# GiannisPikoulis/dsml-thesis

Hardware: AMD Instinct MI355X
Metric: DDIM denoise steps/sec (64×64×4 latent, 256² face) at 1/2/4/8 GPUs (higher is better)
Workload: dtype f32; 1 GPU; face_reenactment emotion-conditioned LDM (AffectNet config), DDIM-200 schedule, 16 samples/GPU, 64x64x4 latent, CFG off, eta 0, random-init weights; batch_per_gpu=16, global_batch=16, ddim_steps=200, hipgraph=True

## Files before the change

dsml_thesis_amd/csrc/igemm.hip:

```cpp
#include "ldmk_common.h"
#include "ldmk_split.h"
#include "ldmk_epilogue.h"
#include <stdlib.h>

#if defined(LDMK_IG_STAMPS) && (LDMK_IG_STAMPS == 1 || LDMK_IG_STAMPS == 3)
#define IG_T(i) do { const unsigned long long t_ = __builtin_amdgcn_s_memtime(); ig_acc[i] += t_ - ig_last; ig_last = t_; } while (0)
#elif defined(LDMK_IG_STAMPS)
#define IG_T(i) do { (void)ig_acc; (void)ig_last; } while (0)
#else
#define IG_T(i) do { } while (0)
#endif

namespace ldmk {

template <int TM, int TN, int LEAN>
__device__ __forceinline__ void ig_lean_epilogue(const ldmk_igemm_args& p, f32x16 (&acc)[TM][TN], const int rowbase, const int colbase, const int bz,
                                                 const int l31, const int half) {
  float* __restrict__ outp = p.out + (long long)bz * p.out_bstride;
  const float* __restrict__ resp = (LEAN == 2 || LEAN == 4) ? p.residual + (long long)bz * p.out_bstride : nullptr;
  const float alpha = p.alpha;
#pragma unroll
  for (int j = 0; j < TN; ++j) {
    const int col = colbase + j * 32 + l31;
    const float bv = p.bias ? p.bias[col] : 0.f;
// ... 1058 lines not shown
      const long long w = blocks * sk;
      const long long rounds = (w + 511) / 512;
      const float occ = (float)w / (float)(rounds * 512);
      const float kpen = (float)(iters / sk) / (float)(iters / sk + 2);
      const float score = kCfg[c].eff * col_use * row_use * occ * kpen * (sk > 1 ? 0.93f : 1.f);
      if (score > best) { best = score; best_cfg = c; best_sk = sk; }
    }
  }
  *cfg_out = best_cfg + 1;
  *splitk_out = best_sk;
}

template <int TM, int TN, int WM, int WN, int KS, bool BT, int BF, bool ASP, bool FG_RT>
static int launch_wk1(const ldmk_igemm_args& a, int splitk, float* ws, hipStream_t st) {
  if constexpr (FG_RT) return launch_cfg<TM, TN, WM, WN, 1, KS, false, BT, BF>(a, splitk, ws, st);
  else return launch_cfg_g<TM, TN, WM, WN, 1, KS, false, BT, BF, true, ASP>(a, splitk, ws, st);
}
template <bool BT, int BF, bool ASP, bool FG_RT>
static int dispatch_wk1(const ldmk_igemm_args& a, int cfg, int splitk, float* ws, hipStream_t st) {
  const bool geglu = a.epi == LDMK_EPI_GEGLU;
  if (cfg == 3) cfg = 4;
  if (cfg == 6) cfg = geglu ? 2 : 5;
  if (geglu && !kCfg[cfg - 1].even_tn) cfg = 1;
  switch (cfg) {
    case 1: return launch_wk1<2, 2, 2, 2, 1, BT, BF, ASP, FG_RT>(a, splitk, ws, st);
    case 2: return launch_wk1<1, 2, 2, 2, 2, BT, BF, ASP, FG_RT>(a, splitk, ws, st);
    case 4: return launch_wk1<1, 1, 2, 2, 2, BT, BF, ASP, FG_RT>(a, splitk, ws, st);
    default: return launch_wk1<1, 5, 4, 1, 1, BT, BF, ASP, FG_RT>(a, splitk, ws, st);
  }
}

template <bool BT>
static int dispatch(const ldmk_igemm_args& a, int cfg, int splitk, float* ws, hipStream_t st) {
  if (a.compute == LDMK_COMPUTE_BF16 && a.w_split && !BT && igemm_fast_gather_ok(a)) return dispatch_wk1<false, 2, false, false>(a, cfg, splitk, ws, st);
  if (a.compute == LDMK_COMPUTE_BF16) return dispatch_wk1<BT, 1, false, true>(a, cfg, splitk, ws, st);
  if (a.compute == LDMK_COMPUTE_BF16X3)
    return a.a_split ? dispatch_wk1<false, 3, true, false>(a, cfg, splitk, ws, st) : dispatch_wk1<false, 3, false, false>(a, cfg, splitk, ws, st);
  if (a.compute == LDMK_COMPUTE_F16X2) return dispatch_wk1<false, 4, false, false>(a, cfg, splitk, ws, st);
  if (a.epi == LDMK_EPI_GEGLU && !kCfg[cfg - 1].even_tn) cfg = 3;
  switch (cfg) {
    case 1: return launch_cfg<2, 2, 2, 2, 1, 1, false, BT>(a, splitk, ws, st);
    case 2: return launch_cfg<1, 2, 2, 2, 1, 2, false, BT>(a, splitk, ws, st);
    case 3: return launch_cfg<2, 2, 1, 1, 4, 1, false, BT>(a, splitk, ws, st);
    case 4: return launch_cfg<1, 1, 2, 2, 1, 2, false, BT>(a, splitk, ws, st);
    case 5: return launch_cfg<1, 5, 4, 1, 1, 1, false, BT>(a, splitk, ws, st);
    default: return launch_cfg<1, 5, 2, 1, 2, 1, false, BT>(a, splitk, ws, st);
  }
}

template <bool BT, bool FG>
static void set_all_attrs() {
  cfg_set_attr<2, 2, 2, 2, 1, 1, false, BT, false, FG>();
  cfg_set_attr<1, 2, 2, 2, 1, 2, false, BT, false, FG>();
  cfg_set_attr<2, 2, 1, 1, 4, 1, false, BT, false, FG>();
  cfg_set_attr<1, 1, 2, 2, 1, 2, false, BT, false, FG>();
  cfg_set_attr<1, 5, 4, 1, 1, 1, false, BT, false, FG>();
  cfg_set_attr<1, 5, 2, 1, 2, 1, false, BT, false, FG>();
}
void igemm_init_attributes() {
  set_all_attrs<false, true>();
  set_all_attrs<true, true>();
  set_all_attrs<false, false>();
  set_all_attrs<true, false>();
}

const char* rgemm_unsupported(const ldmk_igemm_args& a, int rcfg);
int rgemm_dispatch(const ldmk_igemm_args& a, int rcfg, hipStream_t st);
constexpr int kNumRCfg = 6;
const char* sgemm_unsupported(const ldmk_igemm_args& a, int scfg, int splitk);
int sgemm_dispatch(const ldmk_igemm_args& a, int scfg, int splitk, float* ws, hipStream_t st);
constexpr int kNumSCfg = 8;
const char* igemm_ws_unsupported(const ldmk_igemm_args& a, int wcfg, int splitk);
int igemm_ws_dispatch(const ldmk_igemm_args& a, int wcfg, int splitk, float* ws, hipStream_t st);
constexpr int kNumWCfg = 2;
const char* igemm_ps_unsupported(const ldmk_igemm_args& a, int pcfg, int splitk);
int igemm_ps_dispatch(const ldmk_igemm_args& a, int pcfg, int splitk, float* ws, hipStream_t st);
constexpr int kNumPCfg = 11;

}

extern "C" int ldmk_pack_wsplit(const float* w, int K, int N, int ldb, int batch, long long w_bstride, void* out, int ld_out,
                                void* stream) {
  LDMK_ENTER();
  LDMK_REQUIRE(w && out && K > 0 && N > 0 && ldb >= N && batch >= 1, "ldmk_pack_wsplit: bad args");
  LDMK_REQUIRE(ld_out >= K && ld_out % 8 == 0, "ldmk_pack_wsplit: ld_out=%d must be >= K=%d and a multiple of 8", ld_out, K);
  hipLaunchKernelGGL(ldmk::pack_wsplit_kernel<3>, dim3((ld_out + 31) / 32, (N + 31) / 32, batch), dim3(256), 0, (hipStream_t)stream, w, K,
                     N, ldb, w_bstride, reinterpret_cast<__bf16*>(out), ld_out);
  return ldmk::check_launch("ldmk_pack_wsplit");
}

extern "C" int ldmk_pack_wsplit_h2(const float* w, int K, int N, int ldb, int batch, long long w_bstride, int scale_exp, void* out, int ld_out,
                                   void* stream) {
  LDMK_ENTER();
  LDMK_REQUIRE(w && out && K > 0 && N > 0 && ldb >= N && batch >= 1, "ldmk_pack_wsplit_h2: bad args");
  LDMK_REQUIRE(ld_out >= K && ld_out % 8 == 0, "ldmk_pack_wsplit_h2: ld_out=%d must be >= K=%d and a multiple of 8", ld_out, K);
  LDMK_REQUIRE(scale_exp >= -60 && scale_exp <= 60, "ldmk_pack_wsplit_h2: scale_exp=%d outside [-60, 60]", scale_exp);
  hipLaunchKernelGGL(ldmk::pack_wsplit_h2_kernel, dim3((ld_out + 31) / 32, (N + 31) / 32, batch), dim3(256), 0, (hipStream_t)stream, w, K, N, ldb,
                     w_bstride, ldexpf(1.f, scale_exp), reinterpret_cast<_Float16*>(out), ld_out);
  return ldmk::check_launch("ldmk_pack_wsplit_h2");
}

extern "C" int ldmk_pack_wbf16t(const float* w, int K, int N, int ldb, void* out, int ld_out, void* stream) {
  LDMK_ENTER();
  LDMK_REQUIRE(w && out && K > 0 && N > 0 && ldb >= N, "ldmk_pack_wbf16t: bad args");
  LDMK_REQUIRE(ld_out >= K && ld_out % 8 == 0, "ldmk_pack_wbf16t: ld_out=%d must be >= K=%d and a multiple of 8", ld_out, K);
  hipLaunchKernelGGL(ldmk::pack_wsplit_kernel<1>, dim3((ld_out + 31) / 32, (N + 31) / 32, 1), dim3(256), 0, (hipStream_t)stream, w, K, N,
                     ldb, 0LL, reinterpret_cast<__bf16*>(out), ld_out);
  return ldmk::check_launch("ldmk_pack_wbf16t");
}

static int g_force_cfg = 0;
extern "C" void ldmk_igemm_force_config(int cfg) { g_force_cfg = cfg; }

extern "C" int ldmk_igemm_plan(const ldmk_igemm_args* args, int* tile_cfg, int* splitk) {
  if (!args || !tile_cfg || !splitk) return LDMK_EINVAL;
  ldmk::plan(*args, tile_cfg, splitk, args->splitk_ws ? args->splitk_ws_elems : 0);
  return LDMK_OK;
}

extern "C" long long ldmk_igemm_workspace_elems(const ldmk_igemm_args* args) {
  using namespace ldmk;
  LDMK_REQUIRE(args != nullptr, "ldmk_igemm_workspace_elems: null args");
  const ldmk_igemm_args& a = *args;
  LDMK_REQUIRE(a.M > 0 && a.N > 0 && a.K > 0, "ldmk_igemm_workspace_elems: empty problem M=%d N=%d K=%d", a.M, a.N, a.K);
  LDMK_REQUIRE(a.splitk >= 0 && a.splitk <= 64, "ldmk_igemm_workspace_elems: splitk=%d outside [0,64]", a.splitk);
  int cfg = a.tile_cfg, sk = a.splitk;
  if (sk == 0) {
    int c2 = 0;
    plan(a, &c2, &sk, 1LL << 50);
    if (cfg == 0) cfg = c2;
  }
  if (cfg > kNumCfg + kNumRCfg + kNumSCfg)
    return sk <= 1 || a.epi == LDMK_EPI_GEGLU ? 0 : (long long)(a.batch > 1 ? a.batch : 1) * sk * (long long)a.M * a.N;
  if (cfg > kNumCfg + kNumRCfg) {
    if (sk <= 1 || (a.epi == LDMK_EPI_GEGLU && !a.raw_slabs)) return 0;
    return (long long)sk * (long long)a.M * a.N;
  }
  if (cfg > kNumCfg || a.epi == LDMK_EPI_GEGLU || sk <= 1) return 0;
  return (long long)(a.batch > 1 ? a.batch : 1) * sk * (long long)a.M * a.N;
}

static int igemm_entry(const ldmk_igemm_args* args, void* stream, bool launch);
extern "C" int ldmk_igemm(const ldmk_igemm_args* args, void* stream) { return igemm_entry(args, stream, true); }
extern "C" int ldmk_igemm_check(const ldmk_igemm_args* args) { return igemm_entry(args, nullptr, false); }

static int igemm_entry(const ldmk_igemm_args* args, void* stream, bool launch) {
  LDMK_ENTER();
  using namespace ldmk;
  LDMK_REQUIRE(args != nullptr, "ldmk_igemm: null args");
  ldmk_igemm_args a = *args;
  LDMK_REQUIRE(a.M > 0 && a.N > 0 && a.K > 0, "ldmk_igemm: empty problem M=%d N=%d K=%d", a.M, a.N, a.K);
  LDMK_REQUIRE(a.c0 > 0 && a.c0 % 32 == 0 && a.c1 % 32 == 0, "ldmk_igemm: channel counts must be multiples of 32 (c0=%d c1=%d)", a.c0, a.c1);
  LDMK_REQUIRE((a.c1 == 0) == (a.a1 == nullptr), "ldmk_igemm: a1/c1 mismatch");
  const int taps = a.a_mode == LDMK_A_CONV3X3 ? 9 : 1;
  const int skip_k = a.skip_a0 ? a.skip_c0 + a.skip_c1 : 0;
  LDMK_REQUIRE(a.K == taps * (a.c0 + a.c1) + skip_k, "ldmk_igemm: K=%d != taps*(c0+c1)+skip=%d", a.K, taps * (a.c0 + a.c1) + skip_k);
  LDMK_REQUIRE(!a.skip_a0 || (a.a_mode == LDMK_A_CONV3X3 && a.skip_c0 > 0 && a.skip_c0 % 8 == 0 && a.skip_c1 % 8 == 0 &&
                              (a.skip_c1 == 0) == (a.skip_a1 == nullptr) && (a.tile_cfg > kNumCfg + kNumRCfg || a.tile_cfg == 0)),
               "ldmk_igemm: the fused skip connection needs a 3x3 convolution on a slab-GEMM tile, skip channels in multiples of 8");
  LDMK_REQUIRE(a.N % 4 == 0 && a.ldb % 4 == 0, "ldmk_igemm: N and ldb must be multiples of 4");
  LDMK_REQUIRE(a.rows_per_sample > 0, "ldmk_igemm: rows_per_sample");
  LDMK_REQUIRE((long long)a.M * a.ldc < (1LL << 31) && a.ldc > 0, "ldmk_igemm: output exceeds 2^31 elements per batch item (32-bit epilogue offsets)");
  const long long samples = ((long long)a.M + a.rows_per_sample - 1) / a.rows_per_sample;
  if (a.a_mode == LDMK_A_CONV3X3) {
    LDMK_REQUIRE(a.in_h > 0 && a.in_w > 0 && a.out_h > 0 && a.out_w > 0 && a.stride >= 1, "ldmk_igemm: conv geometry");
    LDMK_REQUIRE(a.rows_per_sample == a.out_h * a.out_w, "ldmk_igemm: rows_per_sample != out_h*out_w");
    LDMK_REQUIRE(a.batch <= 1, "ldmk_igemm: batched conv unsupported");
    LDMK_REQUIRE(samples * a.in_h * a.in_w * (a.c0 > a.c1 ? a.c0 : a.c1) < (1LL << 31),
                 "ldmk_igemm: conv input exceeds 2^31 elements (32-bit gather indices)");
  } else {
    LDMK_REQUIRE((long long)a.M * (a.c0 > a.c1 ? a.c0 : a.c1) < (1LL << 31), "ldmk_igemm: A exceeds 2^31 elements per batch item");
  }
  if (a.a_tf == LDMK_TF_AFFINE || a.a_tf == LDMK_TF_AFFINE_SILU) LDMK_REQUIRE(a.tf_coef, "ldmk_igemm: tf_coef missing");
  if (a.a_tf == LDMK_TF_LAYERNORM) {
    LDMK_REQUIRE(a.row_stats && a.ln_gamma && a.ln_beta && a.a_mode == LDMK_A_ROWS, "ldmk_igemm: layernorm prologue args");
  }
  if (a.a_tf == LDMK_TF_LAYERNORM_FOLDED)
    LDMK_REQUIRE(a.row_stats && a.ln_colsum && a.a_mode == LDMK_A_ROWS && !a.stats_out && a.batch <= 1,
                 "ldmk_igemm: folded layernorm needs row_stats, ln_colsum (ldmk_fold_layernorm), rows mode, no stats_out, no batching");
  LDMK_REQUIRE(a.a_tf >= LDMK_TF_NONE && a.a_tf <= LDMK_TF_LAYERNORM_FOLDED, "ldmk_igemm: a_tf=%d", a.a_tf);
  if (a.epi == LDMK_EPI_GEGLU) LDMK_REQUIRE(a.N % 64 == 0 && !a.residual && !a.batch_vec, "ldmk_igemm: GEGLU needs N%%64==0 and no residual");
  if (a.stats_out)
    LDMK_REQUIRE(a.M % 32 == 0 && a.rows_per_sample % 32 == 0 && a.epi == LDMK_EPI_NONE && a.batch <= 1,
                 "ldmk_igemm: stats_out needs M%%32==0, rows_per_sample%%32==0, no GEGLU, no batching");
  LDMK_REQUIRE(a.tile_cfg >= 0 && a.tile_cfg <= kNumCfg + kNumRCfg + kNumSCfg + kNumWCfg + kNumPCfg, "ldmk_igemm: tile_cfg=%d outside [0,%d]",
               a.tile_cfg, kNumCfg + kNumRCfg + kNumSCfg + kNumWCfg + kNumPCfg);
  LDMK_REQUIRE(a.splitk >= 0 && a.splitk <= 64, "ldmk_igemm: splitk=%d outside [0,64]", a.splitk);
  LDMK_REQUIRE(a.compute == LDMK_COMPUTE_F32 || a.compute == LDMK_COMPUTE_BF16 || a.compute == LDMK_COMPUTE_BF16X3 || a.compute == LDMK_COMPUTE_F16X2,
               "ldmk_igemm: compute=%d", a.compute);
  const bool ps_tile = a.tile_cfg > kNumCfg + kNumRCfg + kNumSCfg + kNumWCfg;
  LDMK_REQUIRE(!a.a_ps1 || (ps_tile && a.a_ps), "ldmk_igemm: a_ps1 (second A source) is read by the pre-split tiles only, next to a_ps");
  if (a.compute == LDMK_COMPUTE_BF16X3 && !ps_tile) {
    LDMK_REQUIRE(a.w_split && !a.b_trans && a.w_split_ld >= a.K && a.w_split_ld % 8 == 0,
                 "ldmk_igemm: LDMK_COMPUTE_BF16X3 needs w_split (ldmk_pack_wsplit), b_trans = 0, w_split_ld >= K and a multiple of 8");
    LDMK_REQUIRE(3LL * a.N * a.w_split_ld * 2 < (1LL << 32), "ldmk_igemm: w_split exceeds 4 GB per batch entry");
    LDMK_REQUIRE(igemm_fast_gather_ok(a), "ldmk_igemm: LDMK_COMPUTE_BF16X3 needs the fast gather (no zero-insertion, two-source "
                 "upsampling or operands beyond 4 GB)");
  }
  if (a.compute == LDMK_COMPUTE_F16X2) {
    LDMK_REQUIRE(a.tile_cfg <= kNumCfg || ps_tile, "ldmk_igemm: LDMK_COMPUTE_F16X2 runs on the LDS-tiled shapes (tile_cfg 0..6) and the pre-split "
                 "tiles (23..28, 31..33), not tile_cfg=%d", a.tile_cfg);
    LDMK_REQUIRE(!a.a_split && a.w_scale_exp >= -60 && a.w_scale_exp <= 60, "ldmk_igemm: LDMK_COMPUTE_F16X2: a_split is not taken; w_scale_exp=%d", a.w_scale_exp);
    if (!ps_tile) {
      LDMK_REQUIRE(a.w_split && !a.b_trans && a.w_split_ld >= a.K && a.w_split_ld % 8 == 0 && 2LL * a.N * a.w_split_ld * 2 < (1LL << 32),
                   "ldmk_igemm: LDMK_COMPUTE_F16X2 needs w_split (ldmk_pack_wsplit_h2), b_trans = 0, w_split_ld >= K and a multiple of 8, below 4 GB");
      LDMK_REQUIRE(a.range_flag != nullptr, "ldmk_igemm: LDMK_COMPUTE_F16X2 needs range_flag");
      LDMK_REQUIRE(igemm_fast_gather_ok(a), "ldmk_igemm: LDMK_COMPUTE_F16X2 needs the fast gather (no zero-insertion, two-source upsampling or "
                   "operands beyond 4 GB)");
    }
  }
  if (a.compute == LDMK_COMPUTE_BF16 && a.w_split)
    LDMK_REQUIRE(!a.b_trans && a.w_split_ld >= a.K && a.w_split_ld % 8 == 0 && (long long)a.N * a.w_split_ld * 2 < (1LL << 32) && a.batch <= 1,
                 "ldmk_igemm: LDMK_COMPUTE_BF16 with w_split (ldmk_pack_wbf16t) needs b_trans = 0, w_split_ld >= K and a multiple of 8, "
                 "no batching");
  if (a.a_split) {
    LDMK_REQUIRE(a.compute == LDMK_COMPUTE_BF16X3 && a.a_mode == LDMK_A_ROWS && a.c1 == 0 && a.batch <= 1 &&
                 (a.a_tf == LDMK_TF_NONE || a.a_tf == LDMK_TF_LAYERNORM_FOLDED) && a.tile_cfg <= kNumCfg,
                 "ldmk_igemm: a_split (pre-split A) needs LDMK_COMPUTE_BF16X3 on an LDS-tiled shape (tile_cfg 0..6), rows mode, one "
                 "source, no staging prologue, no batching");
    LDMK_REQUIRE(a.a_split_ld >= a.K && a.a_split_ld % 8 == 0 && 3LL * a.M * a.a_split_ld * 2 < (1LL << 32),
                 "ldmk_igemm: a_split_ld=%d must be >= K, a multiple of 8, and the three images below 4 GB", a.a_split_ld);
  }
  LDMK_REQUIRE(a.compute == LDMK_COMPUTE_F32 || a.tile_cfg <= kNumCfg || a.tile_cfg > kNumCfg + kNumRCfg + kNumSCfg,
               "ldmk_igemm: the row / slab GEMM tiles are fp32 only");
  if (a.alpha == 0.f) a.alpha = 1.f;
  if (a.compute == LDMK_COMPUTE_F16X2) a.alpha *= ldexpf(1.f, -(LDMK_F16X2_A_EXP + a.w_scale_exp));
  int cfg = 0, sk = 1;
  plan(a, &cfg, &sk, a.splitk_ws ? a.splitk_ws_elems : 0);
  if (a.tile_cfg > 0) cfg = a.tile_cfg;
  if (g_force_cfg > 0 && (g_force_cfg <= kNumCfg || !rgemm_unsupported(a, g_force_cfg - kNumCfg - 1))) cfg = g_force_cfg;
  LDMK_REQUIRE(!a.skip_a0 || cfg > kNumCfg + kNumRCfg, "ldmk_igemm: the fused skip connection runs on the slab GEMM only (tile_cfg 13..20)");
  if (cfg > kNumCfg + kNumRCfg + kNumSCfg + kNumWCfg) {
    const int pcfg = cfg - kNumCfg - kNumRCfg - kNumSCfg - kNumWCfg - 1;
    int psk = a.splitk > 0 ? a.splitk : 1;
    const char* why = igemm_ps_unsupported(a, pcfg, psk);
    LDMK_REQUIRE(why == nullptr, "ldmk_igemm: tile_cfg=%d splitk=%d (pre-split bf16x3 tile) cannot run this problem: %s", cfg, psk, why ? why : "");
    LDMK_REQUIRE(!a.raw_slabs || psk >= 2, "ldmk_igemm: raw_slabs needs a split-K plan");
    if (psk > 1) {
      const long long b = a.batch > 1 ? a.batch : 1;
      LDMK_REQUIRE_MEM(a.splitk_ws && b * psk * (long long)a.M * a.N <= a.splitk_ws_elems,
                       "ldmk_igemm: splitk=%d needs a workspace of %lld floats (ldmk_igemm_workspace_elems), %lld given", psk,
                       b * psk * (long long)a.M * a.N, a.splitk_ws ? a.splitk_ws_elems : 0LL);
    }
    if (!launch) return LDMK_OK;
    return igemm_ps_dispatch(a, pcfg, psk, a.splitk_ws, (hipStream_t)stream);
  }
  if (cfg > kNumCfg + kNumRCfg + kNumSCfg) {
    const int wcfg = cfg - kNumCfg - kNumRCfg - kNumSCfg - 1;
    int wsk = a.splitk > 0 ? a.splitk : 1;
    const char* why = igemm_ws_unsupported(a, wcfg, wsk);
    LDMK_REQUIRE(why == nullptr, "ldmk_igemm: tile_cfg=%d splitk=%d (warp-specialised bf16x3 tile) cannot run this problem: %s", cfg, wsk,
                 why ? why : "");
    LDMK_REQUIRE(!a.raw_slabs || wsk >= 2, "ldmk_igemm: raw_slabs needs a split-K plan");
    if (wsk > 1) {
      const long long b = a.batch > 1 ? a.batch : 1;
      LDMK_REQUIRE_MEM(a.splitk_ws && b * wsk * (long long)a.M * a.N <= a.splitk_ws_elems,
                       "ldmk_igemm: splitk=%d needs a workspace of %lld floats (ldmk_igemm_workspace_elems), %lld given", wsk,
                       b * wsk * (long long)a.M * a.N, a.splitk_ws ? a.splitk_ws_elems : 0LL);
    }
    if (!launch) return LDMK_OK;
    return igemm_ws_dispatch(a, wcfg, wsk, a.splitk_ws, (hipStream_t)stream);
  }
  if (cfg > kNumCfg + kNumRCfg) {
    const int scfg = cfg - kNumCfg - kNumRCfg - 1;
    int ssk = a.splitk > 0 ? a.splitk : 1;
    const char* why = sgemm_unsupported(a, scfg, ssk);
    LDMK_REQUIRE(why == nullptr, "ldmk_igemm: tile_cfg=%d splitk=%d (slab GEMM) cannot run this problem: %s", cfg, ssk, why ? why : "");
    if (ssk > 1)
      LDMK_REQUIRE_MEM(a.splitk_ws && ssk * (long long)a.M * a.N <= a.splitk_ws_elems,
                       "ldmk_igemm: splitk=%d needs a workspace of %lld floats (ldmk_igemm_workspace_elems), %lld given", ssk,
                       ssk * (long long)a.M * a.N, a.splitk_ws ? a.splitk_ws_elems : 0LL);
    if (!launch) return LDMK_OK;
    return sgemm_dispatch(a, scfg, ssk, a.splitk_ws, (hipStream_t)stream);
  }
  if (cfg > kNumCfg) {
    const char* why = rgemm_unsupported(a, cfg - kNumCfg - 1);
    LDMK_REQUIRE(why == nullptr, "ldmk_igemm: tile_cfg=%d (row GEMM) cannot run this problem: %s", cfg, why ? why : "");
    if (!launch) return LDMK_OK;
    return rgemm_dispatch(a, cfg - kNumCfg - 1, (hipStream_t)stream);
  }
  if (a.splitk > 0) sk = a.splitk;
  if (a.epi == LDMK_EPI_GEGLU && !a.raw_slabs) sk = 1;
  LDMK_REQUIRE(!a.raw_slabs || (sk >= 2 && a.batch <= 1 && !a.splitk_counters && !a.stats_out),
               "ldmk_igemm: raw_slabs needs a split-K plan (splitk >= 2), no batching / in-launch combine / stats_out");
  if (sk > 1 && a.splitk_counters) {
    const long long tiles = (long long)(a.batch > 1 ? a.batch : 1) * ((a.M + 63) / 64) * ((a.N + 63) / 64);
    LDMK_REQUIRE_MEM(tiles <= a.splitk_counters_len, "ldmk_igemm: in-launch split-K combine needs %lld zeroed counters, %d given",
                     tiles, a.splitk_counters_len);
    LDMK_REQUIRE((long long)sk * a.M * a.N * 4 < (1LL << 31), "ldmk_igemm: in-launch split-K combine addresses the %d slabs of one "
                 "batch entry with 32-bit offsets (%lld bytes)", sk, (long long)sk * a.M * a.N * 4);
  }
  if (sk > 1) {
    const long long b = a.batch > 1 ? a.batch : 1;
    LDMK_REQUIRE_MEM(a.splitk_ws && b * sk * (long long)a.M * a.N <= a.splitk_ws_elems,
                     "ldmk_igemm: splitk=%d needs a workspace of %lld floats (ldmk_igemm_workspace_elems), %lld given", sk,
                     b * sk * (long long)a.M * a.N, a.splitk_ws ? a.splitk_ws_elems : 0LL);
  }
  if (!launch) return LDMK_OK;
  hipStream_t st = (hipStream_t)stream;
  return a.b_trans ? dispatch<true>(a, cfg, sk, a.splitk_ws, st) : dispatch<false>(a, cfg, sk, a.splitk_ws, st);
}
```

dsml_thesis_amd/csrc/igemm_ps.hip:

```cpp
#include "ldmk_common.h"
#include "ldmk_split.h"
#include "ldmk_epilogue.h"
#include <stdlib.h>

namespace ldmk {

#ifdef LDMK_PS_PROBES
constexpr bool PS_PROBES = true;
#else
constexpr bool PS_PROBES = false;
#endif
static int ps_probe_bits() {
  if (!PS_PROBES) return 0;
  static const int dbg = [] {
    const char* d = getenv("LDMK_PS_DEBUG");
    const char* s = getenv("LDMK_PS_STAGGER");
    return (d ? atoi(d) : 0) | ((s ? atoi(s) : 0) << 8);
  }();
  return dbg;
}

constexpr unsigned PS_OOB = 0x80000000u;

__device__ __forceinline__ void ps_dma3(unsigned voff, const u32x4& rs, unsigned lds_dst) {
// ... 781 lines not shown
  const u32x4 rs_a = buffer_rsrc(p.a_ps, Mb_in * (unsigned)Kb_in * (unsigned)UB);
  const u32x4 rs_b = buffer_rsrc(p.w_ps, (unsigned)Nb * (unsigned)Kb_w * (unsigned)UB);

  unsigned toff[AI][9];
#pragma unroll
  for (int i = 0; i < AI; ++i) {
    const int u = wave + NW * i;
    const int row = m0 + 32 * u + l31;
    const bool rok = u < FA && row < p.M;
    const int rr = rok ? row : 0;
    const int n = rr / p.rows_per_sample, rem = rr - n * p.rows_per_sample;
    const int oy = rem / p.out_w, ox = rem - oy * p.out_w;
#pragma unroll
    for (int t = 0; t < 9; ++t) {
      const int iy = oy * p.stride + t / 3 - p.pad_lo, ix = ox * p.stride + t % 3 - p.pad_lo;
      const bool ok = rok && iy >= 0 && iy < p.in_h && ix >= 0 && ix < p.in_w;
      const unsigned q = (unsigned)((n * p.in_h + iy) * p.in_w + ix);
      toff[i][t] = ok ? (q >> 5) * (unsigned)Kb_in * (unsigned)UB + ((unsigned)half * 32u + (q & 31u)) * 16u : PS_OOB;
    }
  }
  unsigned ubase[UHI];
#pragma unroll
  for (int i = 0; i < UHI; ++i) {
    const int u = wave + NW * i;
    const int blk = n0 / 32 + (u - FA);
    ubase[i] = (u >= FA && u < U && blk < Nb) ? (unsigned)blk * (unsigned)Kb_w * (unsigned)UB + (unsigned)(18 * c_begin) * (unsigned)UB : PS_OOB;
  }
  const unsigned lane16 = lane * 16;
  const unsigned lds0 = (unsigned)(size_t)smem_ps;
  const bool hi_wave = wave + NW * (UHI - 1) < U;

  f32x16 acc[TM][TN];
#pragma unroll
  for (int i = 0; i < TM; ++i)
#pragma unroll
    for (int j = 0; j < TN; ++j)
#pragma unroll
      for (int r = 0; r < 16; ++r) acc[i][j][r] = 0.f;

  auto issue = [&](const int c, const int j, const int buf, const unsigned sB) {
    const bool live = c < c_end;
    const unsigned cs = (unsigned)(2 * c + (j & 1)) * (unsigned)UB;
    const unsigned bdst = lds0 + (unsigned)buf * STAGE;
#pragma unroll
    for (int i = 0; i < UHI; ++i) {
      const int u = wave + NW * i;
      if (u < U) {
        if (i < AI && u < FA) {
          const unsigned t = toff[i < AI ? i : 0][j >> 1];
          ps_dma<PL>((live && t != PS_OOB) ? t + cs : PS_OOB, rs_a, bdst + (unsigned)u * (unsigned)UB);
        } else {
          ps_dma<PL>((live && ubase[i] != PS_OOB) ? lane16 + ubase[i] + sB * (unsigned)UB : PS_OOB, rs_b, bdst + (unsigned)u * (unsigned)UB);
        }
      }
    }
  };

  unsigned sB = 0;
  issue(c_begin, 0, 0, 0);
  issue(c_begin, 1, 1, 1);
  for (int c = c_begin; c < c_end; ++c) {
#pragma unroll
    for (int j = 0; j < 18; ++j) {
      if (hi_wave) wait_vm<PL * UHI * (NS - 2)>(); else wait_vm<PL * ULO * (NS - 2)>();
      asm volatile("s_barrier" ::: "memory");
      issue(j + 2 < 18 ? c : c + 1, (j + 2) % 18, (j + 2) % NS, sB + 2);
      ++sB;
      const unsigned char* sb = smem_ps + (j % NS) * STAGE + lane16;
      f16x8 a8[PL][TM];
#pragma unroll
      for (int g = 0; g < PL; ++g)
#pragma unroll
        for (int i = 0; i < TM; ++i) a8[g][i] = *reinterpret_cast<const f16x8*>(sb + ((wm * TM + i) * PL + g) * 1024);
#pragma unroll
      for (int jn = 0; jn < TN; ++jn) {
        f16x8 b8[PL];
#pragma unroll
        for (int g = 0; g < PL; ++g) b8[g] = *reinterpret_cast<const f16x8*>(sb + ((FA + wn * TN + jn) * PL + g) * 1024);
#pragma unroll
        for (int i = 0; i < TM; ++i) {
          if constexpr (TR) {
            acc[i][jn] = __builtin_amdgcn_mfma_f32_32x32x16_f16(b8[0], a8[1][i], acc[i][jn], 0, 0, 0);
            acc[i][jn] = __builtin_amdgcn_mfma_f32_32x32x16_f16(b8[1], a8[0][i], acc[i][jn], 0, 0, 0);
            acc[i][jn] = __builtin_amdgcn_mfma_f32_32x32x16_f16(b8[0], a8[0][i], acc[i][jn], 0, 0, 0);
          } else {
            acc[i][jn] = __builtin_amdgcn_mfma_f32_32x32x16_f16(a8[1][i], b8[0], acc[i][jn], 0, 0, 0);
            acc[i][jn] = __builtin_amdgcn_mfma_f32_32x32x16_f16(a8[0][i], b8[1], acc[i][jn], 0, 0, 0);
            acc[i][jn] = __builtin_amdgcn_mfma_f32_32x32x16_f16(a8[0][i], b8[0], acc[i][jn], 0, 0, 0);
          }
        }
      }
    }
  }
  wait_vm<0>();
  const int lean = ps_lean_form<TR>(p, splitk, (nfast & 2) != 0, m0 + (wm + 1) * 32 * TM, n0 + (wn + 1) * 32 * TN);
  if (lean == 1) ps_epilogue<TM, TN, TR, PL, false, 1>(p, acc, m0 + wm * 32 * TM, n0 + wn * 32 * TN, splitk, ks, 0, ws, lane);
  else if (lean == 2) ps_epilogue<TM, TN, TR, PL, false, 2>(p, acc, m0 + wm * 32 * TM, n0 + wn * 32 * TN, splitk, ks, 0, ws, lane);
  else if (lean == 3) ps_epilogue<TM, TN, TR, PL, false, 3>(p, acc, m0 + wm * 32 * TM, n0 + wn * 32 * TN, splitk, ks, 0, ws, lane);
  else if (lean == 4) ps_epilogue<TM, TN, TR, PL, false, 4>(p, acc, m0 + wm * 32 * TM, n0 + wn * 32 * TN, splitk, ks, 0, ws, lane);
  else ps_epilogue<TM, TN, TR, PL>(p, acc, m0 + wm * 32 * TM, n0 + wn * 32 * TN, splitk, ks, 0, ws, lane);
}

__global__ __launch_bounds__(256) void gn_apply_ps_h2_kernel(const float* __restrict__ x0, int c0, const float* __restrict__ x1, int c1,
                                                             const float* __restrict__ coef, unsigned char* __restrict__ dst, long long rows,
                                                             int hw, int silu, int* __restrict__ range_flag) {
  const int rb = blockIdx.x, kc = blockIdx.y;
  const int r = threadIdx.x >> 3, o = threadIdx.x & 7;
  const long long row = (long long)rb * 32 + r;
  const int C = c0 + c1;
  const int k0 = kc * 64 + o * 8;
  if (k0 >= C) return;
  float4 v0 = make_float4(0.f, 0.f, 0.f, 0.f), v1 = v0;
  if (row < rows) {
    const float* src = k0 < c0 ? x0 + row * c0 + k0 : x1 + row * c1 + (k0 - c0);
    const float4 a = *reinterpret_cast<const float4*>(src), b = *reinterpret_cast<const float4*>(src + 4);
    const float* cf = coef + ((row / hw) * 2) * C + k0;
    const float4 s0 = *reinterpret_cast<const float4*>(cf), s1 = *reinterpret_cast<const float4*>(cf + 4);
    const float4 h0 = *reinterpret_cast<const float4*>(cf + C), h1 = *reinterpret_cast<const float4*>(cf + C + 4);
    v0 = make_float4(fmaf(a.x, s0.x, h0.x), fmaf(a.y, s0.y, h0.y), fmaf(a.z, s0.z, h0.z), fmaf(a.w, s0.w, h0.w));
    v1 = make_float4(fmaf(b.x, s1.x, h1.x), fmaf(b.y, s1.y, h1.y), fmaf(b.z, s1.z, h1.z), fmaf(b.w, s1.w, h1.w));
    if (silu) {
      v0 = make_float4(silu_f(v0.x), silu_f(v0.y), silu_f(v0.z), silu_f(v0.w));
      v1 = make_float4(silu_f(v1.x), silu_f(v1.y), silu_f(v1.z), silu_f(v1.w));
    }
    if (h2_out_of_range(v0) || h2_out_of_range(v1)) *range_flag = 1;
  }
  unsigned char* d = dst + ((long long)rb * (C / 16) + (k0 >> 4)) * 2048 + ((o & 1) * 32 + r) * 16;
  f16x4 a0, l0, a1, l1;
  split2h(scaled_sat(v0), a0, l0);
  split2h(scaled_sat(v1), a1, l1);
  *reinterpret_cast<f16x8*>(d) = f16x8{a0[0], a0[1], a0[2], a0[3], a1[0], a1[1], a1[2], a1[3]};
  *reinterpret_cast<f16x8*>(d + 1024) = f16x8{l0[0], l0[1], l0[2], l0[3], l1[0], l1[1], l1[2], l1[3]};
}

template <int NWM, int NWN, int TM, int TN, bool TR>
static int psc_launch(const ldmk_igemm_args& a, int splitk, float* ws, hipStream_t st) {
  constexpr int BM = 32 * TM * NWM, BN = 32 * TN * NWN;
  constexpr size_t lds = (size_t)3 * (BM / 32 + BN / 32) * 2048;
  static_assert(lds <= 160 * 1024, "LDS ring exceeds 160 KiB");
  static bool attr = false;
  if (!attr) {
    (void)hipFuncSetAttribute(reinterpret_cast<const void*>(igemm_psc_kernel<NWM, NWN, TM, TN, TR>), hipFuncAttributeMaxDynamicSharedMemorySize, (int)lds);
    attr = true;
  }
  const int tiles = ((a.M + BM - 1) / BM) * ((a.N + BN - 1) / BN);
  const int nfast_env = switch_value(SW_PS_NFAST);
  const int lean_env = switch_value(SW_PS_LEAN);
  const int nfast = (nfast_env && (a.N + BN - 1) / BN > 1 && (a.M + BM - 1) / BM >= 8 ? 1 : 0) | (lean_env ? 0 : 2);
  hipLaunchKernelGGL((igemm_psc_kernel<NWM, NWN, TM, TN, TR>), dim3(tiles, splitk, 1), dim3(64 * NWM * NWN), lds, st, a, splitk, ws, nfast);
  if (splitk > 1 && !a.raw_slabs) return launch_splitk_reduce(a, splitk, ws, st);
  return check_launch("ldmk_igemm(ps, conv)");
}

const char* igemm_ps_unsupported(const ldmk_igemm_args& a, int pcfg, int splitk) {
  if (a.compute != LDMK_COMPUTE_BF16X3 && a.compute != LDMK_COMPUTE_F16X2) return "the pre-split tiles run the bf16x3 and the f16x2 arithmetic (compute)";
  const int pl = a.compute == LDMK_COMPUTE_F16X2 ? 2 : 3;
  if (pl == 2 && (pcfg == 6 || pcfg == 7)) return "the warp-specialised pre-split tiles (29 / 30) exist in the bf16x3 arithmetic only";
  if (pl == 2 && a.out_ps && !a.range_flag) return "out_ps in the f16x2 arithmetic needs range_flag";
  if (!a.a_ps || !a.w_ps) return "a_ps / w_ps (operands in the PS layout: ldmk_pack_ps, ldmk_ln_stats_ps, out_ps of a producer GEMM)";
  if (a.a_mode == LDMK_A_CONV3X3) {
    if (pl != 2) return "the conv-mode pre-split tile runs the f16x2 arithmetic only";
    if (pcfg != 0 && pcfg != 1 && pcfg != 3 && pcfg != 4) return "conv mode: tile_cfg 23 / 24 / 26 / 27";
    if (a.c1 || a.a1 || a.upsample || a.a_tf != LDMK_TF_NONE || a.out_ps || a.batch > 1 || a.epi != LDMK_EPI_NONE || a.attn_kv_out)
      return "conv mode: one pre-normalised source (ldmk_gn_apply_ps_h2), no upsampling / prologue / out_ps / batching / GEGLU";
    if (a.c0 % 32) return "conv mode: C_in must be a multiple of 32";
    if ((a.c0 / 32) % splitk) return "conv mode: splitk must divide C_in / 32 (K is split on 32-channel chunk boundaries)";
    const long long smp = ((long long)a.M + a.rows_per_sample - 1) / a.rows_per_sample;
    if (((smp * a.in_h * a.in_w + 31) / 32) * (a.c0 / 16) * 2048 >= (1LL << 31)) return "conv mode: input of 2 GiB or more";
  } else if (a.a_mode != LDMK_A_ROWS) {
    return "rows mode or 3x3 convolution";
  }
  if (a.b_trans || a.upsample || a.skip_a0 || (a.splitk_counters && !(ps_probe_bits() & 8))) return "b_trans / upsample / fused skip / in-launch combine";
  if (a.a_tf != LDMK_TF_NONE && a.a_tf != LDMK_TF_LAYERNORM_FOLDED) return "no staging prologue: a_ps is what gets multiplied";
  if (a.K % 32 || a.N % 32) return "K and N must be multiples of 32";
  if (a.a_ps1) {
    if (a.a_mode != LDMK_A_ROWS || pcfg == 6 || pcfg == 7) return "a_ps1: rows mode on tile_cfg 23..28 / 31..33 (not the conv-mode or warp-specialised tiles)";
    if (a.batch > 1 || a.attn_kv_out || a.a_tf != LDMK_TF_NONE || a.epi == LDMK_EPI_GEGLU)
      return "a_ps1: no batching, no fused QKV tiles, no folded LayerNorm, no GEGLU";
    if (a.a_ps_k0 <= 0 || a.a_ps_k0 >= a.K || a.a_ps_k0 % 32) return "a_ps1: a_ps_k0 and K - a_ps_k0 must be positive multiples of 32";
  }
  const long long kb = a.K / 16;
  if ((a.a_mode == LDMK_A_ROWS && (long long)((a.M + 31) / 32) * kb * pl * 1024 >= (1LL << 31)) || (long long)(a.N / 32) * kb * pl * 1024 >= (1LL << 31))
    return "an operand of 2 GiB or more";
  if (a.epi == LDMK_EPI_GEGLU && (!kPsCfg[pcfg].even_tn || splitk > 1)) return "GEGLU needs a tile of (value, gate) pairs (256x256, 128x256) and no split-K";
  if (splitk > a.K / 32) return "more K slices than 32-deep chunks";
  if (a.out_ps) {
    if (splitk > 1 || a.batch > 1 || a.stats_out) return "out_ps: no split-K, no batching, no GroupNorm records (transposed epilogue)";
    if (a.ldc % 16) return "out_ps: ldc (the PS output's column count) must be a multiple of 16";
  } else if (!a.out && splitk <= 1) {
    return "no output";
  }
  if (a.stats_out && !a.out) return "stats_out needs out";
  if (a.attn_kv_out) {
    if (pl != 2 || (pcfg != 0 && pcfg != 4)) return "attn_kv_out: the F16X2 arithmetic on tile_cfg 23 / 27";
    if (a.stats_out || splitk > 1 || a.batch > 1 || a.epi != LDMK_EPI_NONE || a.out_ps || !a.out || !a.range_flag)
      return "attn_kv_out: the fused QKV projection (no split-K / batching / GEGLU / records / out_ps; out and range_flag required)";
    if (a.attn_heads <= 0 || a.N != 3 * 32 * a.attn_heads) return "attn_kv_out: N must be 3 x 32 x attn_heads ([q | k | v] of d_head 32)";
    if (a.attn_tokens <= 0 || a.attn_tokens % 64 || a.M % a.attn_tokens) return "attn_kv_out: attn_tokens a multiple of 64 that divides M";
  }
  return nullptr;
}

int igemm_ps_dispatch(const ldmk_igemm_args& a, int pcfg, int splitk, float* ws, hipStream_t st) {
  const bool tr = !a.stats_out;
  if (a.a_mode == LDMK_A_CONV3X3) {
    switch (pcfg) {
      case 0: return tr ? psc_launch<8, 1, 1, 5, true>(a, splitk, ws, st) : psc_launch<8, 1, 1, 5, false>(a, splitk, ws, st);
      case 1: return tr ? psc_launch<4, 2, 2, 5, true>(a, splitk, ws, st) : psc_launch<4, 2, 2, 5, false>(a, splitk, ws, st);
      case 3: return tr ? psc_launch<4, 2, 1, 5, true>(a, splitk, ws, st) : psc_launch<4, 2, 1, 5, false>(a, splitk, ws, st);
      default: return tr ? psc_launch<4, 1, 1, 5, true>(a, splitk, ws, st) : psc_launch<4, 1, 1, 5, false>(a, splitk, ws, st);
    }
  }
  if (a.compute == LDMK_COMPUTE_F16X2 && a.attn_kv_out)
    return pcfg == 0 ? ps_launch<8, 1, 1, 5, 3, true, 2, true>(a, splitk, ws, st) : ps_launch<4, 1, 1, 5, 3, true, 2, true>(a, splitk, ws, st);
  if (a.compute == LDMK_COMPUTE_F16X2) {
    switch (pcfg) {
      case 0: return tr ? ps_launch<8, 1, 1, 5, 3, true, 2>(a, splitk, ws, st) : ps_launch<8, 1, 1, 5, 3, false, 2>(a, splitk, ws, st);
      case 1: return tr ? ps_launch<4, 2, 2, 5, 3, true, 2>(a, splitk, ws, st) : ps_launch<4, 2, 2, 5, 3, false, 2>(a, splitk, ws, st);
      case 2: return tr ? ps_launch<4, 2, 2, 4, 3, true, 2>(a, splitk, ws, st) : ps_launch<4, 2, 2, 4, 3, false, 2>(a, splitk, ws, st);
      case 3: return tr ? ps_launch<4, 2, 1, 5, 3, true, 2>(a, splitk, ws, st) : ps_launch<4, 2, 1, 5, 3, false, 2>(a, splitk, ws, st);
      case 4: return tr ? ps_launch<4, 1, 1, 5, 3, true, 2>(a, splitk, ws, st) : ps_launch<4, 1, 1, 5, 3, false, 2>(a, splitk, ws, st);
      case 8: return tr ? ps_launch<4, 1, 2, 5, 3, true, 2>(a, splitk, ws, st) : ps_launch<4, 1, 2, 5, 3, false, 2>(a, splitk, ws, st);
      case 9: return tr ? ps_launch<4, 1, 2, 4, 3, true, 2>(a, splitk, ws, st) : ps_launch<4, 1, 2, 4, 3, false, 2>(a, splitk, ws, st);
      case 10: return tr ? ps_launch<2, 2, 2, 4, 3, true, 2>(a, splitk, ws, st) : ps_launch<2, 2, 2, 4, 3, false, 2>(a, splitk, ws, st);
      default: return tr ? ps_launch<4, 2, 1, 4, 3, true, 2>(a, splitk, ws, st) : ps_launch<4, 2, 1, 4, 3, false, 2>(a, splitk, ws, st);
    }
  }
  switch (pcfg) {
    case 0: return tr ? ps_launch<8, 1, 1, 5, 3, true>(a, splitk, ws, st) : ps_launch<8, 1, 1, 5, 3, false>(a, splitk, ws, st);
    case 1: return tr ? ps_launch<4, 2, 2, 5, 2, true>(a, splitk, ws, st) : ps_launch<4, 2, 2, 5, 2, false>(a, splitk, ws, st);
    case 2: return tr ? ps_launch<4, 2, 2, 4, 3, true>(a, splitk, ws, st) : ps_launch<4, 2, 2, 4, 3, false>(a, splitk, ws, st);
    case 3: return tr ? ps_launch<4, 2, 1, 5, 3, true>(a, splitk, ws, st) : ps_launch<4, 2, 1, 5, 3, false>(a, splitk, ws, st);
    case 4: return tr ? ps_launch<4, 1, 1, 5, 2, true>(a, splitk, ws, st) : ps_launch<4, 1, 1, 5, 2, false>(a, splitk, ws, st);
    case 6: return tr ? pw_launch<2, 5, 4, true>(a, splitk, ws, st) : pw_launch<2, 5, 4, false>(a, splitk, ws, st);
    case 7: return tr ? pw_launch<2, 4, 4, true>(a, splitk, ws, st) : pw_launch<2, 4, 4, false>(a, splitk, ws, st);
    case 8: return tr ? ps_launch<4, 1, 2, 5, 2, true>(a, splitk, ws, st) : ps_launch<4, 1, 2, 5, 2, false>(a, splitk, ws, st);
    case 9: return tr ? ps_launch<4, 1, 2, 4, 2, true>(a, splitk, ws, st) : ps_launch<4, 1, 2, 4, 2, false>(a, splitk, ws, st);
    case 10: return tr ? ps_launch<2, 2, 2, 4, 2, true>(a, splitk, ws, st) : ps_launch<2, 2, 2, 4, 2, false>(a, splitk, ws, st);
    default: return tr ? ps_launch<4, 2, 1, 4, 3, true>(a, splitk, ws, st) : ps_launch<4, 2, 1, 4, 3, false>(a, splitk, ws, st);
  }
}

}

extern "C" long long ldmk_ps_bytes(int rows, int k) {
  if (rows <= 0 || k <= 0 || k % 16) return -1;
  return (long long)((rows + 31) / 32) * (k / 16) * 3072;
}

extern "C" long long ldmk_ps_bytes_h2(int rows, int k) {
  if (rows <= 0 || k <= 0 || k % 16) return -1;
  return (long long)((rows + 31) / 32) * (k / 16) * 2048;
}

extern "C" int ldmk_pack_ps(const float* src, int rows, int k, long long row_stride, long long k_stride, int batch, long long src_bstride,
                            void* dst, void* stream) {
  LDMK_ENTER();
  using namespace ldmk;
  LDMK_REQUIRE(src && dst && rows > 0 && k > 0 && batch >= 1, "ldmk_pack_ps: bad args");
  LDMK_REQUIRE(k % 16 == 0, "ldmk_pack_ps: k=%d must be a multiple of 16", k);
  LDMK_REQUIRE(k_stride != 1 || (row_stride % 4 == 0 && (reinterpret_cast<uintptr_t>(src) & 15) == 0 && src_bstride % 4 == 0),
               "ldmk_pack_ps: row-major sources are read as float4 (16-byte aligned rows)");
  const long long bytes = ldmk_ps_bytes(rows, k);
  hipLaunchKernelGGL(pack_ps_kernel<3>, dim3((rows + 31) / 32, (k + 63) / 64, batch), dim3(256), 0, (hipStream_t)stream, src, rows, k, row_stride,
                     k_stride, src_bstride, reinterpret_cast<unsigned char*>(dst), bytes, 1.0f, (int*)nullptr);
  return check_launch("ldmk_pack_ps");
}

extern "C" int ldmk_pack_ps_h2(const float* src, int rows, int k, long long row_stride, long long k_stride, int batch, long long src_bstride,
                               int scale_exp, int* range_flag, void* dst, void* stream) {
  LDMK_ENTER();
  using namespace ldmk;
  LDMK_REQUIRE(src && dst && rows > 0 && k > 0 && batch >= 1, "ldmk_pack_ps_h2: bad args");
  LDMK_REQUIRE(k % 16 == 0, "ldmk_pack_ps_h2: k=%d must be a multiple of 16", k);
  LDMK_REQUIRE(k_stride != 1 || (row_stride % 4 == 0 && (reinterpret_cast<uintptr_t>(src) & 15) == 0 && src_bstride % 4 == 0),
               "ldmk_pack_ps_h2: row-major sources are read as float4 (16-byte aligned rows)");
  LDMK_REQUIRE(scale_exp >= -60 && scale_exp <= 60, "ldmk_pack_ps_h2: scale_exp=%d outside [-60, 60]", scale_exp);
  LDMK_REQUIRE(!range_flag || scale_exp == LDMK_F16X2_A_EXP, "ldmk_pack_ps_h2: range_flag is the activations' check: scale_exp must be %d", LDMK_F16X2_A_EXP);
  const long long bytes = ldmk_ps_bytes_h2(rows, k);
  hipLaunchKernelGGL(pack_ps_kernel<2>, dim3((rows + 31) / 32, (k + 63) / 64, batch), dim3(256), 0, (hipStream_t)stream, src, rows, k, row_stride,
                     k_stride, src_bstride, reinterpret_cast<unsigned char*>(dst), bytes, ldexpf(1.f, scale_exp), range_flag);
  return check_launch("ldmk_pack_ps_h2");
}

extern "C" int ldmk_ln_stats_ps(const float* x, int rows, int c, float eps, float* stats, void* dst, float guard, int* flag, void* stream) {
  LDMK_ENTER();
  using namespace ldmk;
  LDMK_REQUIRE(x && stats && dst && rows > 0 && c > 0, "ldmk_ln_stats_ps: bad args");
  LDMK_REQUIRE(c % 16 == 0 && c <= 1280, "ldmk_ln_stats_ps: C=%d must be a multiple of 16, at most 1280", c);
  LDMK_REQUIRE(!flag || guard > 0.f, "ldmk_ln_stats_ps: guard=%g must be positive", (double)guard);
  const dim3 grid((rows + 31) / 32);
  unsigned char* d = reinterpret_cast<unsigned char*>(dst);
  hipStream_t st = (hipStream_t)stream;
  int* nf = nullptr;
  if (c <= 192) hipLaunchKernelGGL(ln_stats_ps_kernel<3>, grid, dim3(256), 0, st, x, rows, c, eps, stats, d, guard, flag, nf);
  else if (c <= 320) hipLaunchKernelGGL(ln_stats_ps_kernel<5>, grid, dim3(256), 0, st, x, rows, c, eps, stats, d, guard, flag, nf);
  else if (c <= 640) hipLaunchKernelGGL(ln_stats_ps_kernel<10>, grid, dim3(256), 0, st, x, rows, c, eps, stats, d, guard, flag, nf);
  else hipLaunchKernelGGL(ln_stats_ps_kernel<20>, grid, dim3(256), 0, st, x, rows, c, eps, stats, d, guard, flag, nf);
  return check_launch("ldmk_ln_stats_ps");
}

extern "C" int ldmk_ln_stats_ps_h2(const float* x, int rows, int c, float eps, float* stats, void* dst, float guard, int* flag, int* range_flag,
                                   void* stream) {
  LDMK_ENTER();
  using namespace ldmk;
  LDMK_REQUIRE(x && stats && dst && range_flag && rows > 0 && c > 0, "ldmk_ln_stats_ps_h2: bad args");
  LDMK_REQUIRE(c % 16 == 0 && c <= 1280, "ldmk_ln_stats_ps_h2: C=%d must be a multiple of 16, at most 1280", c);
  LDMK_REQUIRE(!flag || guard > 0.f, "ldmk_ln_stats_ps_h2: guard=%g must be positive", (double)guard);
  const dim3 grid((rows + 31) / 32);
  unsigned char* d = reinterpret_cast<unsigned char*>(dst);
  hipStream_t st = (hipStream_t)stream;
  if (c <= 192) hipLaunchKernelGGL((ln_stats_ps_kernel<3, 2>), grid, dim3(256), 0, st, x, rows, c, eps, stats, d, guard, flag, range_flag);
  else if (c <= 320) hipLaunchKernelGGL((ln_stats_ps_kernel<5, 2>), grid, dim3(256), 0, st, x, rows, c, eps, stats, d, guard, flag, range_flag);
  else if (c <= 640) hipLaunchKernelGGL((ln_stats_ps_kernel<10, 2>), grid, dim3(256), 0, st, x, rows, c, eps, stats, d, guard, flag, range_flag);
  else hipLaunchKernelGGL((ln_stats_ps_kernel<20, 2>), grid, dim3(256), 0, st, x, rows, c, eps, stats, d, guard, flag, range_flag);
  return check_launch("ldmk_ln_stats_ps_h2");
}

extern "C" int ldmk_gn_apply_ps_h2(const float* x0, int c0, const float* x1, int c1, const float* coef, void* y_ps, int n, int hw, int silu,
                                   int* range_flag, void* stream) {
  LDMK_ENTER();
  using namespace ldmk;
  LDMK_REQUIRE(x0 && coef && y_ps && range_flag && n > 0 && hw > 0 && c0 > 0, "ldmk_gn_apply_ps_h2: bad args");
  LDMK_REQUIRE((c1 == 0) == (x1 == nullptr), "ldmk_gn_apply_ps_h2: x1/c1 mismatch");
  LDMK_REQUIRE(c0 % 8 == 0 && c1 % 8 == 0 && (c0 + c1) % 16 == 0, "ldmk_gn_apply_ps_h2: c0 = %d, c1 = %d must be multiples of 8, their sum of 16", c0, c1);
  const long long rows = (long long)n * hw;
  LDMK_REQUIRE(ldmk_ps_bytes_h2((int)rows, c0 + c1) < (1LL << 31) && rows < (1LL << 31), "ldmk_gn_apply_ps_h2: output of 2 GiB or more");
  hipLaunchKernelGGL(gn_apply_ps_h2_kernel, dim3((unsigned)((rows + 31) / 32), (c0 + c1 + 63) / 64), dim3(256), 0, (hipStream_t)stream, x0, c0, x1, c1,
                     coef, reinterpret_cast<unsigned char*>(y_ps), rows, hw, silu, range_flag);
  return check_launch("ldmk_gn_apply_ps_h2");
}
```

dsml_thesis_amd/csrc/ldmk_epilogue.h:

```cpp
#pragma once
#include "ldmk_common.h"

namespace ldmk {

__device__ __forceinline__ float lnf_bias(float acc, float mean, float cs, float rstd, float bias) {
#pragma clang fp contract(off)
  const float t = __builtin_fmaf(-mean, cs, acc) * rstd;
  return t + bias;
}
__device__ __forceinline__ float bias_res(float acc_alpha, float bias, float vec, float res) {
#pragma clang fp contract(off)
  float t = acc_alpha + bias;
  t = t + vec;
  return t + res;
}
__device__ __forceinline__ float col_finish(float acc_alpha, float bias) {
#pragma clang fp contract(off)
  return acc_alpha + bias;
}
__device__ __forceinline__ float col_finish(float acc_alpha, float bias, float extra) {
#pragma clang fp contract(off)
  const float t = acc_alpha + bias;
  return t + extra;
}
// ... 21 lines not shown
  sm += __shfl_xor(sm, 32, 64);
  sq += __shfl_xor(sq, 32, 64);
  if (half == 0) {
    float* d = stats_out + ((long long)tile_row * N + col) * 3;
    d[0] = shift; d[1] = sm; d[2] = sq;
  }
}

template <int TM, int TN>
__device__ __forceinline__ void col_slab_store(const ldmk_igemm_args& p, const f32x16 (&acc)[TM][TN], const int rowbase, const int colbase,
                                               const int bz, const int l31, const int half, const int splitk, const int ks,
                                               float* __restrict__ ws) {
  float* slab = ws + ((long long)bz * splitk + ks) * p.M * p.N;
#pragma unroll
  for (int j = 0; j < TN; ++j) {
    const int col = colbase + j * 32 + l31;
    if (col >= p.N) continue;
#pragma unroll
    for (int i = 0; i < TM; ++i)
#pragma unroll
      for (int r = 0; r < 16; ++r) {
        const int row = rowbase + i * 32 + (r & 3) + 8 * (r >> 2) + 4 * half;
        if (row < p.M) slab[(long long)row * p.N + col] = acc[i][j][r];
      }
  }
}

template <int TM, int TN>
__device__ __forceinline__ void col_geglu(const ldmk_igemm_args& p, const f32x16 (&acc)[TM][TN], const int rowbase, const int colbase,
                                          const int bz, const int l31, const int half, const bool lnf) {
  float* __restrict__ outp = p.out + (long long)bz * p.out_bstride;
  const float alpha = p.alpha;
  const float2* __restrict__ stats2 = reinterpret_cast<const float2*>(p.row_stats);
  if constexpr (TN % 2 == 0) {
#pragma unroll
    for (int j = 0; j < TN; j += 2) {
      const int cv = colbase + j * 32 + l31;
      const int cg = cv + 32;
      if (cv >= p.N) continue;
      const int oc = ((colbase + j * 32) >> 1) + l31;
      const float bv = p.bias ? p.bias[cv] : 0.f, bg = p.bias ? p.bias[cg] : 0.f;
      const float csv = lnf ? p.ln_colsum[cv] : 0.f, csg = lnf ? p.ln_colsum[cg] : 0.f;
#pragma unroll
      for (int i = 0; i < TM; ++i) {
        float2 st[16];
        if (lnf) {
#pragma unroll
          for (int r = 0; r < 16; ++r) st[r] = stats2[min(rowbase + i * 32 + (r & 3) + 8 * (r >> 2) + 4 * half, p.M - 1)];
        }
#pragma unroll
        for (int r = 0; r < 16; ++r) {
          const int row = rowbase + i * 32 + (r & 3) + 8 * (r >> 2) + 4 * half;
          if (row < p.M) {
            float v = acc[i][j][r] * alpha, g = acc[i][j + 1][r] * alpha;
            if (lnf) {
              v = fmaf(-st[r].x, csv, v) * st[r].y;
              g = fmaf(-st[r].x, csg, g) * st[r].y;
            }
            v += bv;
            g += bg;
            const float ge = gelu_erf_f(g);
            outp[(long long)row * p.ldc + oc] = v * ge;
          }
        }
      }
    }
  }
}

template <int TM, int TN>
__device__ __forceinline__ void col_general(const ldmk_igemm_args& p, f32x16 (&acc)[TM][TN], const int rowbase, const int colbase,
                                            const int bz, const int l31, const int half, const bool lnf) {
  float* __restrict__ outp = p.out + (long long)bz * p.out_bstride;
  const float* resp = p.residual ? p.residual + (long long)bz * p.out_bstride : nullptr;
  const float alpha = p.alpha;
  const float2* __restrict__ stats2 = reinterpret_cast<const float2*>(p.row_stats);
  const bool tile_in_sample = p.rows_per_sample % 32 == 0;
  int smp[TM];
#pragma unroll
  for (int i = 0; i < TM; ++i) smp[i] = p.batch_vec ? min(rowbase + i * 32, p.M - 1) / p.rows_per_sample : 0;
#pragma unroll
  for (int j = 0; j < TN; ++j) {
    const int col = colbase + j * 32 + l31;
    if (col >= p.N) continue;
    const float bv = p.bias ? p.bias[col] : 0.f;
    const float cs = lnf ? p.ln_colsum[col] : 0.f;
#pragma unroll
    for (int i = 0; i < TM; ++i) {
      float vals[16];
      const int r0 = rowbase + i * 32 + 4 * half;
      if (lnf) {
        float2 st[16];
#pragma unroll
        for (int r = 0; r < 16; ++r) st[r] = stats2[min(r0 + (r & 3) + 8 * (r >> 2), p.M - 1)];
#pragma unroll
        for (int r = 0; r < 16; ++r) acc[i][j][r] = fmaf(-st[r].x, cs, acc[i][j][r] * alpha) * st[r].y;
      }
      const unsigned obase = (unsigned)r0 * (unsigned)p.ldc + (unsigned)col;
      const float vec = (p.batch_vec && tile_in_sample) ? p.batch_vec[(long long)smp[i] * p.batch_vec_ld + col] : 0.f;
#pragma unroll
      for (int r = 0; r < 16; ++r) {
        const int dr = (r & 3) + 8 * (r >> 2);
        float v = 0.f;
        if (r0 + dr < p.M) {
          v = (lnf ? acc[i][j][r] : acc[i][j][r] * alpha) + bv;
          if (p.batch_vec) v += tile_in_sample ? vec : p.batch_vec[(long long)((r0 + dr) / p.rows_per_sample) * p.batch_vec_ld + col];
          const unsigned o = obase + (unsigned)(dr * p.ldc);
          if (resp) v += resp[o];
          outp[o] = v;
        }
        vals[r] = v;
      }
      if (p.stats_out && rowbase + i * 32 < p.M) gn_tile_record(vals, p.stats_out, (rowbase + i * 32) >> 5, p.N, col, l31, half);
    }
  }
}

template <int TM, int TN, int LEAN>
__device__ __forceinline__ void col_lean(const ldmk_igemm_args& p, const f32x16 (&acc)[TM][TN], const int rowbase, const int colbase,
                                         const int bz, const int l31, const int half) {
  static_assert(LEAN >= 1 && LEAN <= 4, "operand set 1..4");
  float* __restrict__ outp = p.out + (long long)bz * p.out_bstride;
  const float* __restrict__ resp = (LEAN == 2 || LEAN == 4) ? p.residual + (long long)bz * p.out_bstride : nullptr;
  const float alpha = p.alpha;
#pragma unroll
  for (int j = 0; j < TN; ++j) {
    const int col = colbase + j * 32 + l31;
    const float bv = p.bias ? p.bias[col] : 0.f;
#pragma unroll
    for (int i = 0; i < TM; ++i) {
      const int r0 = rowbase + i * 32 + 4 * half;
      const unsigned obase = (unsigned)r0 * (unsigned)p.ldc + (unsigned)col;
      float extra[16], vec = 0.f;
      if constexpr (LEAN == 1 || LEAN == 4) vec = p.batch_vec[(long long)((rowbase + i * 32) / p.rows_per_sample) * p.batch_vec_ld + col];
      if constexpr (LEAN == 2 || LEAN == 4) {
#pragma unroll
        for (int r = 0; r < 16; ++r) extra[r] = resp[obase + (unsigned)(((r & 3) + 8 * (r >> 2)) * p.ldc)];
      }
      float vals[16];
#pragma unroll
      for (int r = 0; r < 16; ++r) {
        const float t = acc[i][j][r] * alpha;
        if constexpr (LEAN == 3) vals[r] = col_finish(t, bv);
        else if constexpr (LEAN == 1) vals[r] = col_finish(t, bv, vec);
        else if constexpr (LEAN == 2) vals[r] = col_finish(t, bv, extra[r]);
        else vals[r] = col_finish(t, bv, vec, extra[r]);
        outp[obase + (unsigned)(((r & 3) + 8 * (r >> 2)) * p.ldc)] = vals[r];
      }
      if (p.stats_out) gn_tile_record(vals, p.stats_out, (rowbase + i * 32) >> 5, p.N, col, l31, half);
    }
  }
}

__device__ __forceinline__ int col_lean_form(const ldmk_igemm_args& p, const int splitk, const bool off, const int row_end, const int col_end) {
  if (off || splitk != 1 || row_end > p.M || col_end > p.N) return 0;
  if (p.batch_vec && p.rows_per_sample % 32 != 0) return 0;
  if (p.a_tf == LDMK_TF_LAYERNORM_FOLDED || p.epi == LDMK_EPI_GEGLU) return 0;
  return p.batch_vec ? (p.residual ? 4 : 1) : (p.residual ? 2 : 3);
}

}
```

dsml_thesis_amd/engine.py:

```python
import ctypes as C
import math
import os
from collections import namedtuple

import torch

from . import lib as L
from . import ops as _ops
from . import switches


def plan_key(a, m):
    key = f"{m},{a.N},{a.K},{a.a_mode},{a.a_tf},{a.epi},{max(1, a.batch)}"
    if a.b_trans:
        key += ",bt"
    if a.a_mode == L.A_CONV3X3 and (a.stride != 1 or a.upsample):
        key += f",s{a.stride}u{a.upsample}"
    return key


_SECTIONS = {"f32": "LDMK_PLAN_TABLE", "bf16x3": "LDMK_X3_TABLE", "f16x2": "LDMK_H2_TABLE", "ps_bf16x3": "LDMK_PS_TABLE",
             "ps_f16x2": "LDMK_PS_H2_TABLE"}
_TABLES = {}
_PLAN_FILE = os.path.join(os.path.dirname(os.path.abspath(__file__)), "igemm_plans.json")
# ... 322 lines not shown
            args.raw_slabs = 1
            args.splitk_ws, args.splitk_ws_elems = slabs.data_ptr(), args.splitk * args.M * args.N
        else:
            args.raw_slabs = 0
            args.out = slabs.data_ptr()
        args._own_slabs = slabs
        self.calls.append((self.lib.ldmk_igemm, (C.byref(args),), args, "ldmk_igemm"))

    def post(self, pargs, keep=None):
        need = self.lib.ldmk_post_scratch_elems(C.byref(pargs))
        if need > 0:
            if self._gnws is None or self._gnws.numel() < need:
                self._gnws = torch.empty(int(need), device=self.device, dtype=torch.float32)
                self._all.append(self._gnws)
                for _, _, k, name in self.calls:
                    if name == "ldmk_post" and k[0].gn_scratch:
                        k[0].gn_scratch, k[0].gn_scratch_elems = self._gnws.data_ptr(), self._gnws.numel()
            pargs.gn_scratch, pargs.gn_scratch_elems = self._gnws.data_ptr(), self._gnws.numel()
        self.calls.append((self.lib.ldmk_post, (C.byref(pargs),), (pargs, keep), "ldmk_post"))

    def run(self, stream=None):
        st = torch.cuda.current_stream().cuda_stream if stream is None else stream
        for fn, args, _, name in self.calls:
            rc = fn(*args, st)
            if rc != 0:
                L.check(rc, name)


class NetBuilder:

    def __init__(self, pg, n, pin=None, sites=None):
        self.pg, self.n, self.pin, self.ops = pg, n, pin, _ops
        self._stats = {}
        self.sites = sites
        self.h2_flag = pg.h2_flag

    def site(self, name):
        import contextlib

        @contextlib.contextmanager
        def ctx():
            if self.sites is None:
                yield self.h2_flag
                return
            old = (self.h2_flag, self.pg.h2_flag)
            self.h2_flag = self.pg.h2_flag = self.sites.flag(name)
            try:
                yield self.h2_flag
            finally:
                self.h2_flag, self.pg.h2_flag = old
        return ctx()

    @staticmethod
    def ptr(t):
        return 0 if t is None else (t if isinstance(t, int) else t.data_ptr())

    def stats_buffer(self, rows, c):
        return self.pg.alloc(rows // 32, c, 3)

    def release(self, *tensors):
        for t in tensors:
            if t is not None:
                self.drop_stats(t)
        self.pg.release(*tensors)

    def attach_stats(self, t, partial):
        self._stats[t.data_ptr()] = partial

    def drop_stats(self, t):
        p = self._stats.pop(t.data_ptr(), None)
        if p is not None:
            self.pg.release(p)

    def _partial(self, x, hw):
        p = self._stats.get(x.data_ptr())
        if p is None:
            c = x.shape[-1]
            p = self.pg.alloc(self.n * self.pg.lib.ldmk_gn_chunks(hw), c, 3)
            self.pg.add("ldmk_gn_partial", self.ptr(x), c, self.n, hw, self.ptr(p))
            self._stats[x.data_ptr()] = p
        return p

    def gn(self, x0, x1, hw, gamma, beta, eps, film=None):
        pg, p_ = self.pg, self.ptr
        c0 = x0.shape[-1]
        c1 = 0 if x1 is None else x1.shape[-1]
        pa = self._partial(x0, hw)
        pb = None if x1 is None else self._partial(x1, hw)
        coef = pg.alloc(self.n, 2, c0 + c1)
        pg.add("ldmk_gn_finalize", p_(pa), c0, p_(pb), c1, self.n, hw, 32, eps, p_(gamma), p_(beta), p_(coef))
        if film is not None:
            pg.add("ldmk_gn_coef_film", p_(coef), film[0], film[1], self.n, c0 + c1)
        return coef

    def gn_act(self, x0, x1, hw, gamma, beta, eps, silu=True, film=None):
        pg, p_ = self.pg, self.ptr
        c0 = x0.shape[-1]
        c1 = 0 if x1 is None else x1.shape[-1]
        coef = self.gn(x0, x1, hw, gamma, beta, eps, film)
        y = pg.alloc(self.n * hw, c0 + c1)
        pg.add("ldmk_gn_apply", p_(x0), c0, p_(x1), c1, p_(coef), p_(y), self.n, hw, 1 if silu else 0)
        self.release(coef)
        return y

    def conv(self, x0, x1, wp, bias, h, w, coef=None, stride=1, pad_lo=1, upsample=False, batch_vec=None, bv_ld=0,
             residual=None, out=None, stats=False, wf=None):
        pg, n, ops = self.pg, self.n, self.ops
        c0 = x0.shape[-1]
        c1 = 0 if x1 is None else x1.shape[-1]
        cout = wp.shape[1]
        if upsample:
            oh, ow = 2 * h, 2 * w
        elif pad_lo == 1:
            oh, ow = (h - 1) // stride + 1, (w - 1) // stride + 1
        else:
            oh, ow = (h + 1 - 3) // stride + 1, (w + 1 - 3) // stride + 1
        if out is None:
            out = pg.alloc(n, oh, ow, cout)
        a = ops.make_igemm_args(n * oh * ow, cout, 9 * (c0 + c1), x0, c0, wp, out, cout, oh * ow, a1=x1, c1=c1,
                                conv=(h, w, oh, ow, stride, pad_lo, 1 if upsample else 0),
                                tf=L.TF_NONE if coef is None else L.TF_AFFINE_SILU, tf_coef=coef, bias=bias,
                                residual=residual, w_frag=wf)
        if batch_vec is not None:
            a.batch_vec, a.batch_vec_ld = self.ptr(batch_vec), bv_ld
        self._maybe_stats(a, out.view(-1, cout), oh * ow, stats)
        pg.igemm(a, self.pin)
        return out

    WINO_MIN_TILES = int(switches.get("LDMK_WINO_MIN_TILES", "256"))
    UP_MIN_PIXELS = 1024
    WINO_MIN_CIN = int(switches.get("LDMK_WINO_MIN_CIN", "320"))

    def winograd_ok(self, cin, h, w):
        if switches.get("LDMK_NO_WINOGRAD"):
            return False
        pol_n = self.pin[0] if self.pin else self.n
        return (cin >= self.WINO_MIN_CIN and pol_n * (h // 2) * (w // 2) >= self.WINO_MIN_TILES and h % 2 == 0
                and w in (8, 16, 32, 64, 128) and (h * w) % 32 == 0 and (w >= 16 or (h // 2) % 2 == 0))

    def ps_query_conv(self, M, N, K, stride=1):
        if not ps_enabled() or self.h2_flag is None or switches.get("LDMK_PSC", "1") == "0":
            return None
        forced = switches.get("LDMK_PSC_FORCE")
        if forced:
            cfg, sk = (int(v) for v in forced.split(","))
            cin32 = K // (9 * 32)
            while cin32 % sk:
                sk -= 1
            return cfg, sk
        m = M
        if self.pin is not None and self.pin[0] != self.pin[1]:
            m = max(1, M * self.pin[0] // self.pin[1])
        return ps_plan(f"{N},{K},{L.A_CONV3X3},0,0,1" + ("" if stride == 1 else f",s{stride}u0"), m, h2=True, max_ratio=2.0)

    def gn_conv(self, x0, x1, h, w, gamma, beta, eps, wp, u, bias, batch_vec=None, bv_ld=0, residual=None, out=None,
                stats=False, wf=None, u_ps=None, wp_ps=None, film=None):
        pg, n, ops, p_ = self.pg, self.n, self.ops, self.ptr
        c0 = x0.shape[-1]
        c1 = 0 if x1 is None else x1.shape[-1]
        cin = c0 + c1
        cout_ = wp.shape[1]
        plan_c = (self.ps_query_conv(n * h * w, cout_, 9 * cin)
                  if (wp_ps is not None and cin % 32 == 0 and cout_ % 32 == 0 and c0 % 8 == 0 and c1 % 8 == 0) else None)
        if plan_c is not None:
            hf = self.h2_flag
            coef = self.gn(x0, x1, h * w, gamma, beta, eps, film)
            y_ps = pg.alloc_ps(n * h * w, cin)
            pg.add("ldmk_gn_apply_ps_h2", p_(x0), c0, p_(x1), c1, p_(coef), p_(y_ps), n, h * w, 1, p_(hf))
            self.release(coef)
            if out is None:
                out = pg.alloc(n, h, w, cout_)
            a = ops.make_igemm_args(n * h * w, cout_, 9 * cin, None, cin, wp, out, cout_, h * w, conv=(h, w, h, w, 1, 1, 0), bias=bias,
                                    residual=residual, a_ps=y_ps, w_ps=wp_ps, range_flag=hf)
            if batch_vec is not None:
                a.batch_vec, a.batch_vec_ld = self.ptr(batch_vec), bv_ld
            a._algo_flops = 2.0 * (n * h * w) * cout_ * (9 * cin)
            self._maybe_stats(a, out.view(-1, cout_), h * w, stats)
            pg.igemm_ps(a, *plan_c)
            pg.release(y_ps)
            return out
        if u is None or not self.winograd_ok(cin, h, w):
            y = self.gn_act(x0, x1, h * w, gamma, beta, eps, film=film)
            res = self.conv(y.view(n, h, w, cin), None, wp, bias, h, w, batch_vec=batch_vec, bv_ld=bv_ld, residual=residual,
                            out=out, stats=stats, wf=wf)
            self.release(y)
            return res
        cout = u.shape[2]
        tiles = n * (h // 2) * (w // 2)
        coef = self.gn(x0, x1, h * w, gamma, beta, eps, film)
        Mb = pg.alloc(16, tiles, cout)
        if out is None:
            out = pg.alloc(n, h, w, cout)
        plan = self.ps_query(tiles, cout, cin, batch=16) if (u_ps is not None and c0 % 16 == 0 and c1 % 16 == 0) else None
        if plan is not None:
            V = pg.alloc_ps(tiles, cin, batch=16)
            hf = pg.h2_flag
            if hf is not None:
                pg.add("ldmk_winograd_input_ps_h2", p_(x0), c0, p_(x1), c1, p_(coef), 1, n, h, w, p_(V), p_(hf))
            else:
                pg.add("ldmk_winograd_input_ps", p_(x0), c0, p_(x1), c1, p_(coef), 1, n, h, w, p_(V))
            a = ops.make_igemm_args(tiles, cout, cin, None, cin, u, Mb, cout, tiles, batch=16, w_bstride=cin * cout,
                                    out_bstride=tiles * cout, a_ps=V.view(16, -1), w_ps=u_ps, range_flag=hf)
        else:
            V = pg.alloc(16, tiles, cin)
            pg.add("ldmk_winograd_input", p_(x0), c0, p_(x1), c1, p_(coef), 1, n, h, w, p_(V))
            a = ops.make_igemm_args(tiles, cout, cin, V, cin, u, Mb, cout, tiles, batch=16, a_bstride=tiles * cin,
                                    w_bstride=cin * cout, out_bstride=tiles * cout)
        a._winograd = True
        a._algo_flops = 2.0 * (4 * tiles) * cout * (9 * cin)
        if plan is not None:
            pg.igemm_ps(a, *plan)
        else:
            pg.igemm(a, self.pin, batch_is_samples=False)
        part = None
        out2d = out.view(-1, cout)
        if stats:
            self.drop_stats(out2d)
            part = self.stats_buffer(n * h * w, cout)
        pg.add("ldmk_winograd_output", p_(Mb), p_(bias), p_(batch_vec), bv_ld, p_(residual), p_(out), p_(part), n, h, w, cout)
        if stats:
            self.attach_stats(out2d, part)
        self.release(coef)
        pg.release(V, Mb)
        return out

    def up_conv(self, x, h, w, wp, w4, bias, stats=False, w4_ps=None):
        pg, n, ops, p_ = self.pg, self.n, self.ops, self.ptr
        c = x.shape[-1]
        pol_n = self.pin[0] if self.pin else n
        if (w4 is None or switches.get("LDMK_NO_WINOGRAD") or c < self.WINO_MIN_CIN or pol_n * h * w < self.UP_MIN_PIXELS
                or w not in (8, 16, 32, 64)):
            return self.conv(x, None, wp, bias, h, w, upsample=True, stats=stats)
        cout = w4.shape[2]
        pix = n * h * w
        Pm = pg.alloc(4, pix, cout)
        out = pg.alloc(n, 2 * h, 2 * w, cout)
        plan = self.ps_query(pix, cout, 4 * c, batch=4) if (w4_ps is not None and c % 16 == 0) else None
        if plan is not None:
            A = pg.alloc_ps(pix, 4 * c, batch=4)
            hf = pg.h2_flag
            if hf is not None:
                pg.add("ldmk_upconv_gather_ps_h2", p_(x), c, n, h, w, p_(A), p_(hf))
            else:
                pg.add("ldmk_upconv_gather_ps", p_(x), c, n, h, w, p_(A))
            a = ops.make_igemm_args(pix, cout, 4 * c, None, 4 * c, w4, Pm, cout, pix, batch=4, w_bstride=4 * c * cout,
                                    out_bstride=pix * cout, a_ps=A.view(4, -1), w_ps=w4_ps, range_flag=hf)
        else:
            A = pg.alloc(4, pix, 4 * c)
            pg.add("ldmk_upconv_gather", p_(x), c, n, h, w, p_(A))
            a = ops.make_igemm_args(pix, cout, 4 * c, A, 4 * c, w4, Pm, cout, pix, batch=4, a_bstride=pix * 4 * c,
                                    w_bstride=4 * c * cout, out_bstride=pix * cout)
        a._winograd = True
        a._algo_flops = 2.0 * (4 * pix) * cout * (9 * c)
        if plan is not None:
            pg.igemm_ps(a, *plan)
        else:
            pg.igemm(a, self.pin, batch_is_samples=False)
        part = None
        out2d = out.view(-1, cout)
        if stats:
            self.drop_stats(out2d)
            part = self.stats_buffer(4 * pix, cout)
        pg.add("ldmk_upconv_scatter", p_(Pm), p_(bias), p_(out), p_(part), n, h, w, cout)
        if stats:
            self.attach_stats(out2d, part)
        pg.release(A, Pm)
        return out

    def _maybe_stats(self, a, out2d, rows_per_sample, stats):
        if stats and a.M % 32 == 0 and rows_per_sample % 32 == 0:
            self.drop_stats(out2d)
            part = self.stats_buffer(a.M, a.N)
            a.stats_out = part.data_ptr()
            self.attach_stats(out2d, part)

    def ps_query(self, M, N, K, tf=L.TF_NONE, epi=L.EPI_NONE, batch=1, per_sample=True):
        if not ps_enabled():
            return None
        m = M
        if self.pin is not None and self.pin[0] != self.pin[1] and per_sample:
            m = max(1, M * self.pin[0] // self.pin[1])
        return ps_plan(f"{N},{K},{L.A_ROWS},{tf},{epi},{max(1, batch)}", m, h2=self.pg.h2_flag is not None,
                       far=self.pg.far_plans)

    def lin_ps(self, plan, M, K, a_ps, wp, w_ps, bias, rows_per_sample, out=None, out_ps=None, geglu=False, stats=False, **kw):
        pg, ops = self.pg, self.ops
        N = wp.shape[1]
        ncol = N // 2 if geglu else N
        if out is None and out_ps is None:
            out = pg.alloc(M, ncol)
        a = ops.make_igemm_args(M, N, K, None, K, wp, out, ncol, rows_per_sample, bias=bias,
                                epi=L.EPI_GEGLU if geglu else L.EPI_NONE, a_ps=a_ps, w_ps=w_ps, out_ps=out_ps,
                                range_flag=pg.h2_flag, **kw)
        if out is not None:
            self._maybe_stats(a, out, rows_per_sample, stats)
        pg.igemm_ps(a, *plan)
        return out

    def lin(self, x0, wp, bias, rows_per_sample, x1=None, out=None, geglu=False, stats=False, wf=None, **kw):
        pg, ops = self.pg, self.ops
        M, c0 = x0.shape[0], x0.shape[-1]
        c1 = 0 if x1 is None else x1.shape[-1]
        N = wp.shape[1]
        ncol = N // 2 if geglu else N
        if out is None:
            out = pg.alloc(M, ncol)
        a = ops.make_igemm_args(M, N, c0 + c1, x0, c0, wp, out, ncol, rows_per_sample, a1=x1, c1=c1, bias=bias,
                                epi=L.EPI_GEGLU if geglu else L.EPI_NONE, w_frag=wf, **kw)
        self._maybe_stats(a, out, rows_per_sample, stats)
        pg.igemm(a, self.pin)
        return out


class GraphedProgram:

    def __init__(self, fn, warmup=2):
        self.fn = fn
        rng = torch.cuda.get_rng_state()
        side = torch.cuda.Stream()
        side.wait_stream(torch.cuda.current_stream())
        with torch.cuda.stream(side):
            for _ in range(warmup):
                fn()
        torch.cuda.current_stream().wait_stream(side)
        torch.cuda.synchronize()
        self.graph = torch.cuda.CUDAGraph()
        with torch.cuda.graph(self.graph):
            fn()
        torch.cuda.set_rng_state(rng)

    def replay(self):
        self.graph.replay()
```

dsml_thesis_amd/lib.py:

```python
import ctypes as C
import os

from . import switches

_HERE = os.path.dirname(os.path.abspath(__file__))
LIB_PATH = switches.get("LDMK_LIBRARY") or os.path.join(_HERE, "libldmk.so")

A_ROWS, A_CONV3X3 = 0, 1
TF_NONE, TF_AFFINE, TF_AFFINE_SILU, TF_LAYERNORM, TF_LAYERNORM_FOLDED = 0, 1, 2, 3, 4
EPI_NONE, EPI_GEGLU = 0, 1
COMPUTE_F32, COMPUTE_BF16, COMPUTE_BF16X3, COMPUTE_F16X2 = 0, 1, 2, 3
POST_NONE, POST_GROUPNORM, POST_LAYERNORM = 0, 1, 2
PLMS_MULTISTEP, PLMS_PREDICTOR, PLMS_CORRECTOR = 0, 1, 2

_fp = C.c_void_p


class IgemmArgs(C.Structure):
    _fields_ = [
        ("M", C.c_int), ("N", C.c_int), ("K", C.c_int),
        ("a0", _fp), ("a1", _fp), ("c0", C.c_int), ("c1", C.c_int),
        ("a_mode", C.c_int), ("in_h", C.c_int), ("in_w", C.c_int), ("out_h", C.c_int), ("out_w", C.c_int),
        ("stride", C.c_int), ("pad_lo", C.c_int), ("upsample", C.c_int),
        ("a_tf", C.c_int), ("tf_coef", _fp), ("row_stats", _fp), ("ln_gamma", _fp), ("ln_beta", _fp),
        ("rows_per_sample", C.c_int),
        ("w", _fp), ("b_trans", C.c_int), ("ldb", C.c_int),
        ("bias", _fp), ("batch_vec", _fp), ("batch_vec_ld", C.c_int),
        ("residual", _fp), ("epi", C.c_int),
        ("out", _fp), ("ldc", C.c_int), ("batch", C.c_int),
        ("a_bstride", C.c_longlong), ("w_bstride", C.c_longlong), ("out_bstride", C.c_longlong),
        ("alpha", C.c_float), ("tile_cfg", C.c_int), ("splitk", C.c_int),
        ("splitk_ws", _fp), ("splitk_ws_elems", C.c_longlong), ("stats_out", _fp), ("compute", C.c_int), ("splitk_counters", _fp), ("splitk_counters_len", C.c_int),
        ("w_frag", _fp),
        ("ln_colsum", _fp),
        ("raw_slabs", C.c_int),
        ("skip_a0", _fp), ("skip_a1", _fp), ("skip_c0", C.c_int), ("skip_c1", C.c_int),
        ("w_split", _fp), ("w_split_ld", C.c_int), ("w_split_bstride", C.c_longlong),
        ("a_split", _fp), ("a_split_ld", C.c_int),
        ("a_ps", _fp), ("a_ps_bstride", C.c_longlong), ("w_ps", _fp), ("w_ps_bstride", C.c_longlong), ("out_ps", _fp),
        ("w_scale_exp", C.c_int), ("range_flag", _fp),
        ("attn_kv_out", _fp), ("attn_tokens", C.c_int), ("attn_heads", C.c_int),
        ("a_ps1", _fp), ("a_ps_k0", C.c_int),
    ]


class PostArgs(C.Structure):
    _fields_ = [
        ("src", _fp), ("nslab", C.c_int), ("slab_stride", C.c_longlong), ("M", C.c_int), ("N", C.c_int),
        ("rows_per_sample", C.c_int), ("alpha", C.c_float), ("bias", _fp), ("batch_vec", _fp), ("batch_vec_ld", C.c_int),
        ("residual", _fp), ("ldr", C.c_int), ("geglu", C.c_int), ("raw_out", _fp), ("ld_raw", C.c_int), ("norm", C.c_int),
        ("x1", _fp), ("c1", C.c_int), ("groups", C.c_int), ("eps", C.c_float), ("gamma", _fp), ("beta", _fp),
        ("silu", C.c_int), ("norm_out", _fp), ("ld_norm", C.c_int), ("gn_cache_floats", C.c_int),
        ("gn_scratch", _fp), ("gn_scratch_elems", C.c_longlong),
    ]


class WgradArgs(C.Structure):
    _fields_ = [
        ("R", C.c_int), ("Kw", C.c_int), ("N", C.c_int), ("a", _fp), ("c", C.c_int), ("lda", C.c_int),
        ("a_mode", C.c_int), ("in_h", C.c_int), ("in_w", C.c_int), ("out_h", C.c_int), ("out_w", C.c_int),
        ("stride", C.c_int), ("pad_lo", C.c_int), ("upsample", C.c_int),
        ("dy", _fp), ("ldy", C.c_int), ("dw", _fp), ("ldw", C.c_int), ("accumulate", C.c_int), ("alpha", C.c_float),
        ("batch", C.c_int), ("a_bstride", C.c_longlong), ("dy_bstride", C.c_longlong), ("dw_bstride", C.c_longlong),
        ("splitr", C.c_int), ("ws", _fp), ("ws_elems", C.c_longlong), ("dbias", _fp), ("compute", C.c_int),
    ]


_SIGS = {
    "ldmk_version": (C.c_int, []),
    "ldmk_last_error": (C.c_char_p, []),
    "ldmk_init": (C.c_int, [C.c_int]),
    "ldmk_switch_value": (C.c_int, [C.c_char_p]),
    "ldmk_switch_override": (C.c_int, [C.c_char_p, C.c_int]),
    "ldmk_igemm": (C.c_int, [C.POINTER(IgemmArgs), _fp]),
    "ldmk_igemm_workspace_elems": (C.c_longlong, [C.POINTER(IgemmArgs)]),
    "ldmk_igemm_check": (C.c_int, [C.POINTER(IgemmArgs)]),
    "ldmk_igemm_plan": (C.c_int, [C.POINTER(IgemmArgs), C.POINTER(C.c_int), C.POINTER(C.c_int)]),
    "ldmk_igemm_force_config": (None, [C.c_int]),
    "ldmk_wfrag_elems": (C.c_longlong, [C.c_int, C.c_int]),
    "ldmk_pack_wfrag": (C.c_int, [_fp, C.c_int, C.c_int, C.c_int, _fp, _fp]),
    "ldmk_pack_wsplit": (C.c_int, [_fp, C.c_int, C.c_int, C.c_int, C.c_int, C.c_longlong, _fp, C.c_int, _fp]),
    "ldmk_pack_wsplit_h2": (C.c_int, [_fp, C.c_int, C.c_int, C.c_int, C.c_int, C.c_longlong, C.c_int, _fp, C.c_int, _fp]),
    "ldmk_pack_wbf16t": (C.c_int, [_fp, C.c_int, C.c_int, C.c_int, _fp, C.c_int, _fp]),
    "ldmk_winograd_tiles": (C.c_longlong, [C.c_int, C.c_int, C.c_int]),
    "ldmk_winograd_input": (C.c_int, [_fp, C.c_int, _fp, C.c_int, _fp, C.c_int, C.c_int, C.c_int, C.c_int, _fp, _fp]),
    "ldmk_winograd_input_ps": (C.c_int, [_fp, C.c_int, _fp, C.c_int, _fp, C.c_int, C.c_int, C.c_int, C.c_int, _fp, _fp]),
    "ldmk_winograd_output": (C.c_int, [_fp, _fp, _fp, C.c_int, _fp, _fp, _fp, C.c_int, C.c_int, C.c_int, C.c_int, _fp]),
    "ldmk_upconv_gather": (C.c_int, [_fp, C.c_int, C.c_int, C.c_int, C.c_int, _fp, _fp]),
    "ldmk_upconv_gather_ps": (C.c_int, [_fp, C.c_int, C.c_int, C.c_int, C.c_int, _fp, _fp]),
    "ldmk_upconv_gather_ps_h2": (C.c_int, [_fp, C.c_int, C.c_int, C.c_int, C.c_int, _fp, _fp, _fp]),
    "ldmk_winograd_input_ps_h2": (C.c_int, [_fp, C.c_int, _fp, C.c_int, _fp, C.c_int, C.c_int, C.c_int, C.c_int, _fp, _fp, _fp]),
    "ldmk_winograd_input_ps_v1": (C.c_int, [_fp, C.c_int, _fp, C.c_int, _fp, C.c_int, C.c_int, C.c_int, C.c_int, _fp, _fp]),
    "ldmk_winograd_input_ps_h2_v1": (C.c_int, [_fp, C.c_int, _fp, C.c_int, _fp, C.c_int, C.c_int, C.c_int, C.c_int, _fp, _fp, _fp]),
    "ldmk_winograd_output_v1": (C.c_int, [_fp, _fp, _fp, C.c_int, _fp, _fp, _fp, C.c_int, C.c_int, C.c_int, C.c_int, _fp]),
    "ldmk_winograd_input_ps_route": (C.c_int, [C.c_int, C.c_int, C.c_int, C.c_int, C.c_int]),
    "ldmk_winograd_output_route": (C.c_int, [C.c_int, C.c_int, C.c_int, C.c_int, C.c_int]),
    "ldmk_upconv_scatter": (C.c_int, [_fp, _fp, _fp, _fp, C.c_int, C.c_int, C.c_int, C.c_int, _fp]),
    "ldmk_fold_layernorm": (C.c_int, [_fp, C.c_int, C.c_int, C.c_int, _fp, _fp, _fp, _fp, _fp, _fp, _fp]),
    "ldmk_attn_force_qt": (None, [C.c_int]),
    "ldmk_gn_chunks": (C.c_int, [C.c_int]),
    "ldmk_gn_partial": (C.c_int, [_fp, C.c_int, C.c_int, C.c_int, _fp, _fp]),
    "ldmk_gn_finalize": (C.c_int, [_fp, C.c_int, _fp, C.c_int, C.c_int, C.c_int, C.c_int, C.c_float, _fp, _fp, _fp, _fp]),
    "ldmk_gn_coef": (C.c_int, [_fp, C.c_int, _fp, C.c_int, C.c_int, C.c_int, C.c_int, C.c_float, _fp, _fp, _fp, _fp, _fp]),
    "ldmk_ln_stats": (C.c_int, [_fp, C.c_int, C.c_int, C.c_float, _fp, _fp]),
    "ldmk_ln_stats_guard": (C.c_int, [_fp, C.c_int, C.c_int, C.c_float, _fp, C.c_float, _fp, _fp]),
    "ldmk_ps_bytes": (C.c_longlong, [C.c_int, C.c_int]),
    "ldmk_pack_ps": (C.c_int, [_fp, C.c_int, C.c_int, C.c_longlong, C.c_longlong, C.c_int, C.c_longlong, _fp, _fp]),
    "ldmk_ps_bytes_h2": (C.c_longlong, [C.c_int, C.c_int]),
    "ldmk_pack_ps_h2": (C.c_int, [_fp, C.c_int, C.c_int, C.c_longlong, C.c_longlong, C.c_int, C.c_longlong, C.c_int, _fp, _fp, _fp]),
    "ldmk_ln_stats_ps_h2": (C.c_int, [_fp, C.c_int, C.c_int, C.c_float, _fp, _fp, C.c_float, _fp, _fp, _fp]),
    "ldmk_ln_stats_ps": (C.c_int, [_fp, C.c_int, C.c_int, C.c_float, _fp, _fp, C.c_float, _fp, _fp]),
    "ldmk_ln_stats_split": (C.c_int, [_fp, C.c_int, C.c_int, C.c_float, _fp, _fp, C.c_int, _fp]),
    "ldmk_gn_apply": (C.c_int, [_fp, C.c_int, _fp, C.c_int, _fp, _fp, C.c_int, C.c_int, C.c_int, _fp]),
    "ldmk_gn_coef_film": (C.c_int, [_fp, _fp, C.c_int, C.c_int, C.c_int, _fp]),
    "ldmk_gn_apply_ps_h2": (C.c_int, [_fp, C.c_int, _fp, C.c_int, _fp, _fp, C.c_int, C.c_int, C.c_int, _fp, _fp]),
    "ldmk_post": (C.c_int, [C.POINTER(PostArgs), _fp]),
    "ldmk_post_scratch_elems": (C.c_longlong, [C.POINTER(PostArgs)]),
    "ldmk_attn_self": (C.c_int, [_fp, _fp, C.c_int, C.c_int, C.c_int, C.c_float, _fp]),
    "ldmk_attn_self_x3": (C.c_int, [_fp, _fp, C.c_int, C.c_int, C.c_int, C.c_float, _fp]),
    "ldmk_attn_kv_split_bytes": (C.c_longlong, [C.c_int, C.c_int, C.c_int]),
    "ldmk_attn_self_x3p": (C.c_int, [_fp, _fp, _fp, C.c_int, C.c_int, C.c_int, C.c_float, _fp]),
    "ldmk_attn_self_x3p_ps": (C.c_int, [_fp, _fp, _fp, _fp, C.c_int, C.c_int, C.c_int, C.c_float, _fp]),
    "ldmk_attn_kv_split_h2_bytes": (C.c_longlong, [C.c_int, C.c_int, C.c_int]),
    "ldmk_attn_self_h2": (C.c_int, [_fp, _fp, _fp, _fp, C.c_int, C.c_int, C.c_int, C.c_float, _fp]),
    "ldmk_attn_self_h2_ps": (C.c_int, [_fp, _fp, _fp, _fp, _fp, C.c_int, C.c_int, C.c_int, C.c_float, _fp]),
    "ldmk_attn_self_h2_tiles": (C.c_int, [_fp, _fp, _fp, _fp, _fp, C.c_int, C.c_int, C.c_int, C.c_float, _fp]),
    "ldmk_attn_self_small": (C.c_int, [_fp, C.c_int, C.c_longlong, _fp, C.c_int, C.c_int, C.c_int, C.c_float, _fp]),
    "ldmk_attn_cross": (C.c_int, [_fp, C.c_int, _fp, _fp, C.c_int, _fp, C.c_int, C.c_int, C.c_int, C.c_int, C.c_int,
                                  C.c_float, _fp]),
    "ldmk_attn_cross_d": (C.c_int, [_fp, C.c_int, _fp, _fp, C.c_int, _fp, C.c_int, C.c_int, C.c_int, C.c_int, C.c_int, C.c_int, C.c_float, _fp]),
    "ldmk_heads_gather": (C.c_int, [_fp, C.c_int, C.c_int, _fp, C.c_int, C.c_int, C.c_int, C.c_int, C.c_int, _fp]),
    "ldmk_heads_scatter": (C.c_int, [_fp, _fp, C.c_int, C.c_int, C.c_int, C.c_int, C.c_int, C.c_int, _fp]),
    "ldmk_softmax_rows": (C.c_int, [_fp, C.c_longlong, C.c_int, C.c_float, _fp]),
    "ldmk_dense_small": (C.c_int, [_fp, C.c_int, _fp, _fp, _fp, C.c_int, C.c_int, C.c_int, C.c_int, C.c_int, _fp]),
    "ldmk_timestep_embedding": (C.c_int, [_fp, _fp, _fp, C.c_int, C.c_int, _fp]),
    "ldmk_timestep_embedding_f32": (C.c_int, [_fp, _fp, _fp, C.c_int, C.c_int, _fp]),
    "ldmk_conv3x3_in": (C.c_int, [_fp, C.c_int, _fp, C.c_int, _fp, _fp, _fp, C.c_int, C.c_int, C.c_int, C.c_int, _fp]),
    "ldmk_conv3x3_out": (C.c_int, [_fp, _fp, _fp, _fp, _fp, C.c_int, C.c_int, C.c_int, C.c_int, C.c_int, _fp]),
    "ldmk_conv3x3_out_small": (C.c_int, [_fp, _fp, _fp, _fp, _fp, C.c_int, C.c_int, C.c_int, C.c_int, C.c_int, _fp]),
    "ldmk_conv1x1_nchw": (C.c_int, [_fp, _fp, _fp, _fp, C.c_int, C.c_int, C.c_int, C.c_int, _fp]),
    "ldmk_ddim_step": (C.c_int, [_fp, _fp, _fp, _fp, _fp, C.c_float, C.c_int, _fp, _fp, C.c_longlong, C.c_int, _fp, _fp,
                                 C.c_int, C.c_int, C.c_int, _fp]),
    "ldmk_plms_step": (C.c_int, [_fp, _fp, _fp, _fp, _fp, C.c_float, C.c_int, C.c_int, _fp, _fp, _fp, _fp, C.c_longlong, C.c_int,
                                 _fp, _fp, C.c_int, C.c_int, C.c_int, _fp]),
    "ldmk_dpm_step": (C.c_int, [_fp, _fp, _fp, _fp, C.c_float, C.c_int, _fp, _fp, _fp, C.c_longlong, C.c_int, _fp, C.c_int, C.c_int,
                                C.c_int, C.c_int, _fp]),
    "ldmk_advance_timestep": (C.c_int, [_fp, _fp, _fp, C.c_int, C.c_int, C.c_int, _fp]),
    "ldmk_ddpm_step": (C.c_int, [_fp, _fp, _fp, _fp, _fp, _fp, _fp, C.c_longlong, C.c_int, _fp]),
    "ldmk_patch_unfold": (C.c_int, [_fp, _fp] + [C.c_int] * 10 + [_fp]),
    "ldmk_patch_fold": (C.c_int, [_fp, _fp, _fp, _fp] + [C.c_int] * 10 + [_fp]),
    "ldmk_conv3x3_moments": (C.c_int, [_fp] * 7 + [C.c_int] * 6 + [_fp]),
    "ldmk_gauss_posterior": (C.c_int, [_fp, _fp, C.c_float, _fp, _fp, _fp, _fp, C.c_int, C.c_int, C.c_int, _fp]),
    "ldmk_vq_nearest": (C.c_int, [_fp, _fp, _fp, _fp, C.c_int, C.c_int, C.c_int, C.c_int, _fp]),
    "ldmk_permute3": (C.c_int, [_fp, _fp, C.c_int, C.c_int, C.c_int, C.c_int, C.c_int, C.c_int, _fp]),
    "ldmk_audio_attention": (C.c_int, [_fp, C.c_int, C.c_int, C.c_int, _fp, _fp, _fp, _fp, _fp, _fp]),
    "ldmk_mask_rows": (C.c_int, [_fp, _fp, C.c_int, C.c_int, C.c_int, C.c_int, C.c_float, _fp]),
    "ldmk_pack_conv3x3": (C.c_int, [_fp, _fp, C.c_int, C.c_int, _fp]),
    "ldmk_postprocess_frames": (C.c_int, [_fp, _fp, C.c_int, C.c_int, C.c_int, _fp]),
    "ldmk_add_rowvec": (C.c_int, [_fp, _fp, C.c_int, C.c_longlong, C.c_int, C.c_int, _fp]),
    "ldmk_wgrad": (C.c_int, [C.POINTER(WgradArgs), _fp]),
    "ldmk_wgrad_workspace_elems": (C.c_longlong, [C.POINTER(WgradArgs)]),
# ... 109 lines not shown
```

dsml_thesis_amd/ops.py:

```python
import ctypes as C
import math
import weakref
from typing import NamedTuple

import torch

from . import lib as L


def _ptr(t):
    return 0 if t is None else (t if isinstance(t, int) else t.data_ptr())


def stream():
    return torch.cuda.current_stream().cuda_stream


def _chk(t, name):
    if t is None:
        return
    if not (t.is_cuda and t.dtype == torch.float32 and t.is_contiguous()):
        raise L.LdmkError(f"{name}: expected a contiguous float32 CUDA tensor, got {t.dtype} {t.device} "
                          f"contiguous={t.is_contiguous()}")


def pack_conv3x3(w):
    _chk(w, "pack_conv3x3")
    o, i, kh, kw = w.shape
    assert kh == 3 and kw == 3
    out = torch.empty(9 * i, o, device=w.device, dtype=torch.float32)
    L.call("ldmk_pack_conv3x3", _ptr(w), _ptr(out), o, i, stream())
    return out


def pack_conv3x3_narrow(w):
    _chk(w, "pack_conv3x3")
    o, i, kh, kw = w.shape
    assert kh == 3 and kw == 3
    out = torch.empty(9 * i, o, device=w.device, dtype=torch.float32)
    L.call("ldmk_permute3", _ptr(w), _ptr(out), o, i, 9, 2, 1, 0, stream())
    return out


def pack_linear(w):
    _chk(w, "pack_linear")
    n, k = w.shape[0], w.shape[1]
    out = torch.empty(k, n, device=w.device, dtype=torch.float32)
    L.call("ldmk_permute3", _ptr(w), _ptr(out), n, k, 1, 1, 0, 2, stream())
    return out


def permute3(x, perm):
    _chk(x, "permute3")
    d0, d1, d2 = x.shape
    out = torch.empty(x.shape[perm[0]], x.shape[perm[1]], x.shape[perm[2]], device=x.device, dtype=torch.float32)
    L.call("ldmk_permute3", _ptr(x), _ptr(out), d0, d1, d2, perm[0], perm[1], perm[2], stream())
    return out


def pack_wfrag(wp):
    _chk(wp, "pack_wfrag")
    k, n = wp.shape
    if L.load().ldmk_wfrag_elems(k, n) < 0:
        return None
    out = torch.empty(k * n, device=wp.device, dtype=torch.float32)
    L.call("ldmk_pack_wfrag", _ptr(wp), n, k, n, _ptr(out), stream())
    return out


def pack_geglu(w, b):
    two_inner, k = w.shape
    inner = two_inner // 2
    assert inner % 32 == 0
    wt = pack_linear(w)
    val = wt[:, :inner].reshape(k, inner // 32, 1, 32)
    gate = wt[:, inner:].reshape(k, inner // 32, 1, 32)
    wp = torch.cat([val, gate], dim=2).reshape(k, two_inner).contiguous()
    bp = torch.cat([b[:inner].reshape(-1, 1, 32), b[inner:].reshape(-1, 1, 32)], dim=1).reshape(-1).contiguous()
    return wp, bp


def gn_coef(x0, x1, n, hw, gamma, beta, eps, groups=32, partial=None, coef=None):
    c0 = x0.shape[-1]
    c1 = 0 if x1 is None else x1.shape[-1]
    C_ = c0 + c1
    chunks = L.load().ldmk_gn_chunks(hw)
    if partial is None:
        partial = torch.empty(n * chunks * C_ * 3, device=x0.device, dtype=torch.float32)
    if coef is None:
        coef = torch.empty(n, 2, C_, device=x0.device, dtype=torch.float32)
    L.call("ldmk_gn_coef", _ptr(x0), c0, _ptr(x1), c1, n, hw, groups, float(eps), _ptr(gamma), _ptr(beta),
           _ptr(partial), _ptr(coef), stream())
    return coef


def gn_apply(x0, x1, coef, n, hw, silu=True, out=None):
    c0 = x0.shape[-1]
    c1 = 0 if x1 is None else x1.shape[-1]
    if out is None:
        out = torch.empty(n * hw, c0 + c1, device=x0.device, dtype=torch.float32)
    L.call("ldmk_gn_apply", _ptr(x0), c0, _ptr(x1), c1, _ptr(coef), _ptr(out), n, hw, 1 if silu else 0, stream())
    return out


def gn_apply_ps(x0, x1, coef, n, hw, h2_flag, silu=True, out=None):
    c0 = x0.shape[-1]
    c1 = 0 if x1 is None else x1.shape[-1]
    if out is None:
        out = ps_empty(n * hw, c0 + c1, 1, x0.device, h2=True)
    L.call("ldmk_gn_apply_ps_h2", _ptr(x0), c0, _ptr(x1), c1, _ptr(coef), _ptr(out), n, hw, 1 if silu else 0, _ptr(h2_flag), stream())
    return out


def conv3x3_ps(y_ps, n, h, w_, cin, wp, wps, range_flag, bias=None, stride=1, pad_lo=1, batch_vec=None, residual=None, out=None,
               tile_cfg=27, splitk=1, splitk_ws=None, stats_out=None):
    cout = wp.shape[1]
    oh = (h + 2 * pad_lo - 3) // stride + 1 if pad_lo == 1 else (h + 1 - 3) // stride + 1
    ow = (w_ + 2 * pad_lo - 3) // stride + 1 if pad_lo == 1 else (w_ + 1 - 3) // stride + 1
    if out is None:
        out = torch.empty(n, oh, ow, cout, device=wp.device, dtype=torch.float32)
    a = make_igemm_args(n * oh * ow, cout, 9 * cin, None, cin, wp, out, cout, oh * ow, conv=(h, w_, oh, ow, stride, pad_lo, 0), bias=bias,
                        batch_vec=batch_vec, batch_vec_ld=0 if batch_vec is None else batch_vec.stride(0), residual=residual,
                        tile_cfg=tile_cfg, splitk=splitk, splitk_ws=splitk_ws, a_ps=y_ps, w_ps=wps, range_flag=range_flag)
    if stats_out is not None:
        a.stats_out = stats_out.data_ptr()
        a._keep = a._keep + (stats_out,)
    igemm(a)
    return out


def ln_stats(x2d, eps=1e-5, out=None, split=None):
    rows, c = x2d.shape
    if out is None:
        out = torch.empty(rows, 2, device=x2d.device, dtype=torch.float32)
    if split is not None:
        L.call("ldmk_ln_stats_split", _ptr(x2d), rows, c, float(eps), _ptr(out), _ptr(split), split.shape[-1], stream())
    else:
        L.call("ldmk_ln_stats", _ptr(x2d), rows, c, float(eps), _ptr(out), stream())
    return out


PS_TILE0 = 23


def ps_empty(rows, k, batch=1, device="cuda", h2=False):
    nb = (L.load().ldmk_ps_bytes_h2 if h2 else L.load().ldmk_ps_bytes)(int(rows), int(k))
    assert nb > 0, (rows, k)
    return torch.empty(batch, nb, device=device, dtype=torch.uint8)


F16X2_A_EXP = 6


def pack_ps(x, out=None, h2_flag=None):
    batch = x.shape[0] if x.dim() == 3 else 1
    rows, k = x.shape[-2], x.shape[-1]
    assert x.is_contiguous()
    if out is None:
        out = ps_empty(rows, k, batch, x.device, h2=h2_flag is not None)
    if h2_flag is not None:
        L.call("ldmk_pack_ps_h2", _ptr(x), rows, k, k, 1, batch, rows * k, F16X2_A_EXP, _ptr(h2_flag), _ptr(out), stream())
    else:
        L.call("ldmk_pack_ps", _ptr(x), rows, k, k, 1, batch, rows * k, _ptr(out), stream())
    return out


_WPS_H2_EXP = {}


def h2_scale_exp(w):
    mx = float(w.abs().max().item())
    e = 13 - math.floor(math.log2(mx)) if mx > 0.0 and math.isfinite(mx) else 0
    return max(-60, min(60, e))


def pack_wps(w, batch=1, h2=False):
    assert w.is_contiguous() and ((w.dim() == 3 and w.shape[0] == batch) if batch > 1 else w.dim() == 2)
    K, N = w.shape[-2:]
    out = ps_empty(N, K, batch, w.device, h2=h2)
    if h2:
        e = h2_scale_exp(w)
        L.call("ldmk_pack_ps_h2", _ptr(w), N, K, 1, N, batch, K * N, e, 0, _ptr(out), stream())
        ptr = out.data_ptr()
        _WPS_H2_EXP[ptr] = (weakref.ref(out), e)
        weakref.finalize(out, _WPS_H2_EXP.pop, ptr, None)
    else:
        L.call("ldmk_pack_ps", _ptr(w), N, K, 1, N, batch, K * N, _ptr(out), stream())
    return out


def fold_pout(w2, b2, wpo, bpo, dtype=torch.float32):
    w2d, wpod = w2.double(), wpo.reshape(wpo.shape[0], wpo.shape[1]).double()
    w = torch.cat([w2d.t() @ wpod.t(), wpod.t()], 0)
    b = b2.double() @ wpod.t() + bpo.double()
    return w.to(dtype).contiguous(), b.to(dtype).contiguous()


FOLD_POUT_H2_MIN_RATIO = 2.0 ** -16


def fold_pout_h2_ok(w, k0):
    top, bot = float(w[:k0].abs().max().item()), float(w[k0:].abs().max().item())
    return min(top, bot) >= FOLD_POUT_H2_MIN_RATIO * max(top, bot) > 0.0


def ln_stats_ps(x2d, eps=1e-5, out=None, ps=None, guard=0.0, flag=None, h2_flag=None):
    rows, c = x2d.shape
    if out is None:
        out = torch.empty(rows, 2, device=x2d.device, dtype=torch.float32)
    if ps is None:
        ps = ps_empty(rows, c, 1, x2d.device, h2=h2_flag is not None)
    if h2_flag is not None:
        L.call("ldmk_ln_stats_ps_h2", _ptr(x2d), rows, c, float(eps), _ptr(out), _ptr(ps), float(guard), _ptr(flag), _ptr(h2_flag), stream())
    else:
        L.call("ldmk_ln_stats_ps", _ptr(x2d), rows, c, float(eps), _ptr(out), _ptr(ps), float(guard), _ptr(flag), stream())
    return out, ps


def unpack_ps_h2(ps, rows, k):
    nb = (rows + 31) // 32
    t = ps.reshape(-1).view(torch.float16).reshape(nb, k // 16, 2, 2, 32, 8)
    t = t.permute(2, 0, 4, 1, 3, 5).reshape(2, nb * 32, k)[:, :rows]
    return t[0].float(), t[1].float()


def unpack_ps(ps, rows, k):
    nb = (rows + 31) // 32
    t = ps.reshape(-1).view(torch.bfloat16).reshape(nb, k // 16, 3, 2, 32, 8)
    t = t.permute(2, 0, 4, 1, 3, 5).reshape(3, nb * 32, k)[:, :rows]
    return t[0].float(), t[1].float(), t[2].float()


def make_post_args(src, M, N, rows_per_sample, nslab=1, slab_stride=None, bias=None, batch_vec=None, batch_vec_ld=0,
                   residual=None, ldr=None, geglu=False, raw_out=None, ld_raw=None, norm=L.POST_NONE, x1=None, c1=0,
                   gamma=None, beta=None, eps=1e-5, silu=False, norm_out=None, ld_norm=None, groups=32, alpha=1.0):
    a = L.PostArgs()
    a.src, a.nslab, a.slab_stride = _ptr(src), nslab, (M * N if slab_stride is None else slab_stride)
    a.M, a.N, a.rows_per_sample, a.alpha = M, N, rows_per_sample, alpha
    a.bias, a.batch_vec, a.batch_vec_ld = _ptr(bias), _ptr(batch_vec), batch_vec_ld
    a.residual, a.ldr = _ptr(residual), (N if ldr is None else ldr)
    a.geglu = 1 if geglu else 0
    a.raw_out, a.ld_raw = _ptr(raw_out), ((N // 2 if geglu else N) if ld_raw is None else ld_raw)
    a.norm, a.x1, a.c1, a.groups, a.eps = norm, _ptr(x1), c1, groups, float(eps)
    a.gamma, a.beta, a.silu = _ptr(gamma), _ptr(beta), 1 if silu else 0
    a.norm_out, a.ld_norm = _ptr(norm_out), ((N + c1) if ld_norm is None else ld_norm)
    return a


def post(args, device=None):
    need = L.load().ldmk_post_scratch_elems(C.byref(args))
    if need > 0 and not args.gn_scratch:
        scratch = torch.empty(need, device=device if device is not None else torch.device("cuda", torch.cuda.current_device()),
                              dtype=torch.float32)
        args.gn_scratch, args.gn_scratch_elems = scratch.data_ptr(), need
        args._scratch = scratch
    L.call("ldmk_post", C.byref(args), stream())


def make_igemm_args(M, N, K, a0, c0, w, out, ldc, rows_per_sample, a1=None, c1=0, conv=None, tf=L.TF_NONE,
                    tf_coef=None, row_stats=None, ln_gamma=None, ln_beta=None, b_trans=False, ldb=None, bias=None,
                    batch_vec=None, batch_vec_ld=0, residual=None, epi=L.EPI_NONE, batch=1, a_bstride=0, w_bstride=0,
                    out_bstride=0, alpha=1.0, splitk=0, splitk_ws=None, w_frag=None, tile_cfg=0, compute=0, ln_colsum=None,
                    splitk_counters=None, raw_slabs=False, a_split=None, w_bf16t=None, a_ps=None, w_ps=None, out_ps=None,
                    range_flag=None, attn_kv=None, a_ps1=None, a_ps_k0=0):
    a = L.IgemmArgs()
    a._keep = (a0, a1, w, out, tf_coef, row_stats, ln_gamma, ln_beta, bias, batch_vec, residual, splitk_ws, w_frag, ln_colsum,
               splitk_counters, a_split, w_bf16t, a_ps, w_ps, out_ps)
    a.M, a.N, a.K = M, N, K
    a.a0, a.a1, a.c0, a.c1 = _ptr(a0), _ptr(a1), c0, c1
    if conv is not None:
        a.a_mode = L.A_CONV3X3
        a.in_h, a.in_w, a.out_h, a.out_w, a.stride, a.pad_lo, a.upsample = conv
    else:
        a.a_mode = L.A_ROWS
    a.a_tf = tf
    a.tf_coef, a.row_stats, a.ln_gamma, a.ln_beta = _ptr(tf_coef), _ptr(row_stats), _ptr(ln_gamma), _ptr(ln_beta)
    a.rows_per_sample = rows_per_sample
    a.w, a.b_trans = _ptr(w), 1 if b_trans else 0
    a.ldb = ldb if ldb is not None else (K if b_trans else N)
# ... 454 lines not shown
```

dsml_thesis_amd/switches.py:

```python
import os

SWITCHES = {
    "LDMK_SPLIT_BF16": ("1", "arithmetic", "0: every GEMM and the attention on the f32 matrix-core form (v_mfma_f32_32x32x2_f32); the "
                        "f32_mfma_form leg of bench.py", "tolerance"),
    "LDMK_F16X2": ("1", "arithmetic", "0: split products from the exact bf16x3 split (six bf16 MFMAs, operands bit-exact) instead of "
                   "F16X2 (three fp16 MFMAs, range-checked per site); the bf16x3_form leg of bench.py", "tolerance"),
    "LDMK_LN_UNFOLDED": (None, "arithmetic", "set: LayerNorm applied in the GEMM prologue instead of folded through the product (what "
                         "the folded-LayerNorm guard switches a model to by itself)", "tolerance"),
    "LDMK_LN_GUARD_RATIO": ("4.0", "arithmetic", "|mean| / std of a token row above which the folded LayerNorm raises its guard", None),
    "LDMK_ATTN_H2_MIN_TOKENS": ("512", "arithmetic", "self attention runs in F16X2 from this many tokens per sample, bf16x3 below", None),
    "LDMK_H2_CONV_RULE": ("1", "arithmetic", "0: untabled long-K convolutions (K >= 1440) do not take the F16X2 rule (they stay on the f32 matrix-core form of their plan: other bits, same tolerance)", "tolerance"),
    "LDMK_PS": ("1", "route", "0: no pre-split (PS layout, LDS-DMA) GEMM tiles: every GEMM back on the LDS-tiled plan of its shape (that plan's "
                "tile and K split), no conv-mode tile, no folded proj_out -- other bits, same tolerance (tile for tile, at equal split-K, "
                "a pre-split kernel gives the LDS-tiled kernel's bits: tests/test_ps_gpu.py)", "tolerance"),
    "LDMK_PSC": ("1", "route", "0: no conv-mode pre-split tile for 3x3 convolutions: the listed shapes return to their other route (Winograd for "
                 "the wide ones, the in-register split on that route's plan) -- other bits, same tolerance (at equal split-K the tile gives "
                 "the LDS-tiled F16X2 convolution's bits: tests/test_ps_conv_gpu.py)", "tolerance"),
    "LDMK_PSC_FORCE": (None, "route", "'cfg,splitk': force the conv-mode pre-split tile for every eligible convolution (A/B runs)", None),
    "LDMK_POUT_PS": ("0", "route", "1: SpatialTransformer.proj_out on a pre-split tile instead of the row GEMM (measured slower; another arithmetic: other bits, same tolerance)", "tolerance"),
    "LDMK_FOLD_POUT": ("1", "route", "0: the last block's ff.net.2 and proj_out stay two GEMMs instead of one pre-split GEMM on two A "
                       "sources with the composed weight (other bits, same tolerance)", "tolerance"),
    "LDMK_ATTN_PS": ("1", "route", "0: attn1.to_out does not read the attention result in the PS layout (its GEMM leaves the pre-split tile: other bits, same tolerance)", "tolerance"),
    "LDMK_ATTN_PRESPLIT": ("1", "route", "0: K / V are split inside the attention kernel instead of once by their producer; same bits", "bits"),
    "LDMK_ATTN_PRESPLIT_MIN_TOKENS": ("2048", "route", "tokens per sample from which K / V are pre-split", None),
    "LDMK_QKV_TILES": ("1", "route", "0: the fused QKV projection does not write the attention's K / V tiles from its epilogue (the attention's own pre-pass splits them; same bits)", "bits"),
    "LDMK_NO_WINOGRAD": (None, "route", "set: no Winograd F(2x2,3x3) convolutions and no phase-split upsampling convolutions (direct "
                         "implicit GEMM everywhere; other bits, same tolerance)", "tolerance"),
    "LDMK_WINO_MIN_TILES": ("256", "route", "Winograd from this many 2x2 output tiles at the plan-policy batch", None),
    "LDMK_WINO_MIN_CIN": ("320", "route", "Winograd / phase-split upsampling from this many input channels", None),
    "LDMK_NO_SMALL_ROUTE": (None, "route", "set: batch 1-2 jobs run the batched launch program instead of the small-batch route (other kernels: other bits, same tolerance)", "tolerance"),
    "LDMK_SMALL_ROWS": ("4096", "route", "rows (batch x pixels at the policy batch) up to which the small-batch route is taken", None),
    "LDMK_SPLITK_IN_LAUNCH": (None, "route", "set: split-K slabs combined by each tile's last workgroup instead of a reduce launch "
                              "(measured slower; the same output bits per GEMM, but its GroupNorm records are summed in another order: other bits, same tolerance)", "tolerance"),
    "LDMK_TRAIN_NO_PACKED_W": (None, "route", "set: the training step's bf16 GEMMs read fp32 weights instead of the packed bf16 copies (rounded to bf16 in the kernel as the packing does; same bits)", "bits"),
    "LDMK_ATTN_QT": (None, "route", "1 | 2: query tiles per wave of the staged f32 attention kernel (A/B hook; other bits, same tolerance)", "tolerance"),
    "LDMK_NO_PLAN_TABLE": (None, "plan", "set: ignore igemm_plans.json (the library's built-in tile heuristic plans every GEMM)", None),
    "LDMK_PLAN_MAX_RATIO": ("0", "plan", "> 0: a tuned plan is used only within this ratio of its tuned row count (0: nearest at any "
                            "distance)", None),
    "LDMK_PLAN_TABLE": (None, "plan", "a file that replaces the `f32` section of igemm_plans.json (a flat {key: [cfg, splitk]} file as "
                        "the tuning tools write it, or another merged file whose section is taken)", None),
    "LDMK_X3_TABLE": (None, "plan", "the same for the `bf16x3` section", None),
    "LDMK_H2_TABLE": (None, "plan", "the same for the `f16x2` section", None),
    "LDMK_PS_TABLE": (None, "plan", "the same for the `ps_bf16x3` section (pre-split tiles)", None),
    "LDMK_PS_H2_TABLE": (None, "plan", "the same for the `ps_f16x2` section (pre-split tiles, F16X2)", None),
    "LDMK_LIBRARY": (None, "runtime", "path of the libldmk.so to load instead of the in-tree one", None),
    "LDMK_FORCE_COLLECTIVE": (None, "runtime", "set: parallel.all_gather_items issues the real all-gather at world size 1 too (RCCL "
                              "rehearsal; bench.py sets it under LDMK_BENCH_FORCE_DIST)", None),
    "LDMK_LIB_OUT": (None, "build", "output path of the build (an A/B build next to the shipped library)", None),
    "LDMK_HIPCC_FLAGS": ("", "build", "extra hipcc flags, part of the build digest (-DLDMK_PS_PROBES, -DLDMK_IG_STAMPS: probe builds "
                         "for tools/; the shipped library carries neither)", None),
    "LDMK_ATTN_QB": (None, "library", "1 | 2: 32-query blocks per wave of the pre-split attention kernels (default by token count); "
                     "same bits -- but two blocks per wave at a multiple of 256 tokens bring the F16X2 kernel's pipelined loop with them: "
                     "the same bits under LDMK_ATTN_PIPE=1 | 0, other bits within the same tolerance under its default 2", "bits"),
    "LDMK_ATTN_XCD": ("1", "library", "0: F16X2 attention workgroups in launch order instead of re-dealt over the XCDs; same bits", "bits"),
    "LDMK_ATTN_PIPE": ("2", "library", "F16X2 attention key loop: 2 pipelined + lazy running maximum, 1 pipelined with the exact "
                       "maximum, 0 phase-separated (1 and 0: same bits)", "bits"),
    "LDMK_IG_NFAST": ("1", "library", "0: LDS-tiled igemm workgroups in row-major tile order instead of column tiles adjacent; same bits", "bits"),
    "LDMK_IG_LEAN": ("1", "library", "0: the general igemm epilogue everywhere instead of the operand-set specialised copies; same bits", "bits"),
    "LDMK_PS_NFAST": ("1", "library", "as LDMK_IG_NFAST, pre-split tiles; same bits", "bits"),
    "LDMK_PS_LEAN": ("1", "library", "as LDMK_IG_LEAN, pre-split tiles; same bits", "bits"),
    "LDMK_WINO_STAGED": ("1", "library", "0: the Winograd input / output transforms on their first kernels (a thread loads its own 4x4 "
                         "window / walks a band's tiles) instead of the LDS-staged / vectorised ones; same bits", "bits"),
    "LDMK_WGRAD_TR": ("1", "library", "0: bf16 weight-gradient GEMM with the strided gather instead of transposed LDS reads (A/B); dW the same bits, the fused "
                      "bias gradient's fp32 column sums in another order (other bits, same tolerance)", "tolerance"),
    "LDMK_BENCH_BACKEND": ("nccl", "bench", "'gloo': rehearse the N > 1 path of bench.py on a one-GPU box", None),
    "LDMK_BENCH_FORCE_DIST": (None, "bench", "set: create the process group and issue the clip leg's collective with a single rank", None),
}

PROBE_ONLY = ("LDMK_PS_DEBUG", "LDMK_PS_STAGGER")


def get(name, default=None):
    if name not in SWITCHES:
        raise KeyError(f"{name} is not a registered switch (dsml_thesis_amd/switches.py)")
    return os.environ.get(name, default)


def table_markdown():
    rows = ["| switch | default | scope | contract | effect |", "|---|---|---|---|---|"]
    for name, (default, scope, doc, contract) in SWITCHES.items():
        shown = "unset" if default is None else ("`" + (default or "''") + "`")
        rows.append(f"| `{name}` | {shown} | {scope} | {contract or '-'} | {doc} |")
    return "\n".join(rows)


if __name__ == "__main__":
    print(table_markdown())
```

dsml_thesis_amd/unet.py:

```python
import math
import os

import torch
import torch.nn as nn

from . import lib as L
from . import switches
from . import ops
from .engine import ArithSites, NetBuilder, Program, far_from_tuned, split_enabled as engine_split_enabled, ps_enabled as engine_ps_enabled, f16x2_enabled

LN_GUARD_RATIO = float(switches.get("LDMK_LN_GUARD_RATIO", "4.0"))


ATTN_PRESPLIT_MIN_TOKENS = int(switches.get("LDMK_ATTN_PRESPLIT_MIN_TOKENS", "2048"))
ATTN_H2_MIN_TOKENS = int(switches.get("LDMK_ATTN_H2_MIN_TOKENS", "512"))


def ln_unfolded_default():
    return bool(switches.get("LDMK_LN_UNFOLDED"))


class _Params(nn.Module):
    def __init__(self, **shapes):
        super().__init__()
# ... 61 lines not shown

def _seq(*mods):
    s = nn.Module()
    for i, m in enumerate(mods):
        s.add_module(str(i), m)
    s.layers = list(mods)
    return s


def pack_spatial_transformer(P, sd, prefix, m):
    P[prefix + "pin"] = ops.pack_linear(sd[prefix + "proj_in.weight"])
    P[prefix + "pout"] = ops.pack_linear(sd[prefix + "proj_out.weight"])
    for d in range(m.depth):
        q = f"{prefix}transformer_blocks.{d}."
        wqkv = torch.cat([sd[q + "attn1.to_q.weight"], sd[q + "attn1.to_k.weight"], sd[q + "attn1.to_v.weight"]], 0)
        P[q + "qkv"] = ops.pack_linear(wqkv.contiguous())
        P[q + "o1"] = ops.pack_linear(sd[q + "attn1.to_out.0.weight"])
        P[q + "q2"] = ops.pack_linear(sd[q + "attn2.to_q.weight"])
        P[q + "k2"] = ops.pack_linear(sd[q + "attn2.to_k.weight"])
        P[q + "v2"] = ops.pack_linear(sd[q + "attn2.to_v.weight"])
        P[q + "o2"] = ops.pack_linear(sd[q + "attn2.to_out.0.weight"])
        P[q + "ff1"], P[q + "ff1b"] = ops.pack_geglu(sd[q + "ff.net.0.proj.weight"], sd[q + "ff.net.0.proj.bias"])
        P[q + "ff2"] = ops.pack_linear(sd[q + "ff.net.2.weight"])
        for k, nrm, b in (("qkv", "norm1", None), ("q2", "norm2", None), ("ff1", "norm3", P[q + "ff1b"])):
            P[q + k + "_ln"], P[q + k + "_ln#cs"], P[q + k + "_ln#b"] = ops.fold_layernorm(
                P[q + k], sd[q + nrm + ".weight"], sd[q + nrm + ".bias"], b)
    if engine_ps_enabled():
        q = f"{prefix}transformer_blocks.{m.depth - 1}."
        if all(d % 32 == 0 for k in (q + "ff2", prefix + "pout") for d in P[k].shape):
            P[prefix + "ffpo"], P[prefix + "ffpo#b"] = ops.fold_pout(sd[q + "ff.net.2.weight"], sd[q + "ff.net.2.bias"],
                                                                     sd[prefix + "proj_out.weight"], sd[prefix + "proj_out.bias"])


def attention_presplit(hw):
    return engine_split_enabled() and hw >= ATTN_PRESPLIT_MIN_TOKENS and switches.get("LDMK_ATTN_PRESPLIT", "1") != "0"


def emit_self_attention(nb_, qkv, att, hw, heads, d_head, att_ps=None, kv_tiles=None):
    pg, n = nb_.pg, nb_.n
    scale = d_head ** -0.5
    h2_flag = nb_.h2_flag
    if d_head != 32:
        assert att_ps is None and kv_tiles is None
        ops, C_ = nb_.ops, heads * d_head
        dp = -(-d_head // 32) * 32
        if hw % 32:
            raise NotImplementedError(f"attention heads of width {d_head} need a token count that is a multiple of 32 (got {hw})")
        q, k, v = (pg.alloc(n * heads, hw, dp) for _ in range(3))
        for i, t in enumerate((q, k, v)):
            pg.add("ldmk_heads_gather", qkv.data_ptr(), 3 * C_, i * C_, t.data_ptr(), n, hw, heads, d_head, dp)
        sc = pg.alloc(n * heads, hw, hw)
        a = ops.make_igemm_args(hw, hw, dp, q, dp, k, sc, hw, hw, b_trans=True, batch=n * heads, a_bstride=hw * dp, w_bstride=hw * dp,
                                out_bstride=hw * hw)
        pg.igemm(a, nb_.pin, per_sample=True)
        pg.add("ldmk_softmax_rows", sc.data_ptr(), n * heads * hw, hw, float(scale))
        o = pg.alloc(n * heads, hw, dp)
        a = ops.make_igemm_args(hw, dp, hw, sc, hw, v, o, dp, hw, batch=n * heads, a_bstride=hw * hw, w_bstride=hw * dp, out_bstride=hw * dp)
        pg.igemm(a, nb_.pin, per_sample=True)
        pg.add("ldmk_heads_scatter", o.data_ptr(), att.data_ptr(), C_, n, hw, heads, d_head, dp)
        nb_.release(q, k, v, sc, o)
        return
    if h2_flag is not None and kv_tiles is not None:
        pg.add("ldmk_attn_self_h2_tiles", qkv.data_ptr(), kv_tiles.data_ptr(), 0 if att is None else att.data_ptr(),
               0 if att_ps is None else att_ps.data_ptr(), h2_flag.data_ptr(), n, hw, heads, scale)
    elif h2_flag is not None and hw >= ATTN_H2_MIN_TOKENS:
        kvs = pg.alloc(pg.lib.ldmk_attn_kv_split_h2_bytes(n, hw, heads), dtype=torch.uint8)
        if att_ps is not None:
            pg.add("ldmk_attn_self_h2_ps", qkv.data_ptr(), kvs.data_ptr(), 0 if att is None else att.data_ptr(), att_ps.data_ptr(),
                   h2_flag.data_ptr(), n, hw, heads, scale)
        else:
            pg.add("ldmk_attn_self_h2", qkv.data_ptr(), kvs.data_ptr(), att.data_ptr(), h2_flag.data_ptr(), n, hw, heads, scale)
        nb_.release(kvs)
    elif attention_presplit(hw):
        kvs = pg.alloc(pg.lib.ldmk_attn_kv_split_bytes(n, hw, heads), dtype=torch.uint8)
        if att_ps is not None:
            pg.add("ldmk_attn_self_x3p_ps", qkv.data_ptr(), kvs.data_ptr(), 0 if att is None else att.data_ptr(), att_ps.data_ptr(), n, hw,
                   heads, scale)
        else:
            pg.add("ldmk_attn_self_x3p", qkv.data_ptr(), kvs.data_ptr(), att.data_ptr(), n, hw, heads, scale)
        nb_.release(kvs)
    else:
        assert att_ps is None
        pg.add("ldmk_attn_self_x3" if engine_split_enabled() else "ldmk_attn_self", qkv.data_ptr(), att.data_ptr(), n, hw, heads, scale)


def pack_attention_block(P, sd, prefix, m):
    ch, heads = m.ch, m.heads
    d = ch // heads
    if getattr(m, "new_order", False):
        w, bq = sd[prefix + "qkv.weight"].reshape(3 * ch, ch).contiguous(), sd[prefix + "qkv.bias"].contiguous()
    else:
        w = sd[prefix + "qkv.weight"].reshape(heads, 3, d, ch).permute(1, 0, 2, 3).reshape(3 * ch, ch).contiguous()
        bq = sd[prefix + "qkv.bias"].reshape(heads, 3, d).permute(1, 0, 2).reshape(3 * ch).contiguous()
    P[prefix + "aqkv"] = ops.pack_linear(w)
    P[prefix + "aqkv#b"] = bq
    P[prefix + "apout"] = ops.pack_linear(sd[prefix + "proj_out.weight"].reshape(ch, ch).contiguous())


def emit_attention_block(nb_, P, sd, prefix, m, x, h, w):
    pg, n = nb_.pg, nb_.n
    p_ = lambda t: 0 if t is None else t.data_ptr()
    hw = h * w
    rows = n * hw
    xr = x.reshape(rows, m.ch)
    coef = nb_.gn(x, None, hw, sd[prefix + "norm.weight"], sd[prefix + "norm.bias"], 1e-5)
    with nb_.site(prefix + "attn"):
        qkv = nb_.lin(xr, P[prefix + "aqkv"], P[prefix + "aqkv#b"], hw, tf=L.TF_AFFINE, tf_coef=coef, wf=P.get(prefix + "aqkv#f"))
        nb_.release(coef)
        att = pg.alloc(rows, m.ch)
        emit_self_attention(nb_, qkv, att, hw, m.heads, m.d_head)
        nb_.release(qkv)
    with nb_.site(prefix + "proj_out"):
        out = nb_.lin(att, P[prefix + "apout"], sd[prefix + "proj_out.bias"], hw, residual=xr, stats=True, wf=P.get(prefix + "apout#f"))
    nb_.release(att)
    return out.view(n, h, w, m.ch)


def pack_gemm_copies(P, unfolded=False):
    for k in [k for k in P if k.rsplit(".", 1)[-1] in ("pin", "pout", "qkv_ln", "o1", "q2_ln", "o2", "ff1_ln", "ff2", "skip",
                                                        "c1", "c2", "aqkv", "apout")
              or (unfolded and k.rsplit(".", 1)[-1] in ("qkv", "ff1", "q2"))]:
        wf = ops.pack_wfrag(P[k])
        if wf is not None:
            P[k + "#f"] = wf
    if engine_split_enabled():
        for k in list(P):
            tail = k.rsplit(".", 1)[-1]
            if tail in ("pin", "pout", "qkv_ln", "o1", "ff1_ln", "ff2", "skip", "c1", "c2", "w", "aqkv", "apout") or (unfolded and tail in ("qkv", "ff1")):
                if P[k].dim() == 2:
                    P[k + "#s"] = ops.pack_wsplit(P[k])
                    if f16x2_enabled():
                        P[k + "#h"] = ops.pack_wsplit_h2(P[k])
            elif tail in ("c1#wg", "c2#wg", "w#up"):
                P[k + "#s"] = ops.pack_wsplit(P[k], batch=P[k].shape[0])
                if f16x2_enabled():
                    P[k + "#h"] = ops.pack_wsplit_h2(P[k], batch=P[k].shape[0])
    if engine_ps_enabled():
        for k in list(P):
            tail = k.rsplit(".", 1)[-1]
            if tail in ("qkv_ln", "ff1_ln", "ff2", "o1", "pout", "ffpo") and P[k].dim() == 2 and P[k].shape[0] % 32 == 0 and P[k].shape[1] % 32 == 0:
                P[k + "#p"] = ops.pack_wps(P[k])
            elif tail in ("c1#wg", "c2#wg", "w#up") and P[k].shape[1] % 32 == 0 and P[k].shape[2] % 32 == 0:
                P[k + "#p"] = ops.pack_wps(P[k], batch=P[k].shape[0])
        if f16x2_enabled():
            for k in list(P):
                tail = k.rsplit(".", 1)[-1]
                if tail in ("qkv_ln", "ff1_ln", "ff2", "o1", "pout") and P[k].dim() == 2 and P[k].shape[0] % 32 == 0 and P[k].shape[1] % 32 == 0:
                    P[k + "#p2"] = ops.pack_wps(P[k], h2=True)
                elif tail == "ffpo" and ops.fold_pout_h2_ok(P[k], P[k].shape[0] - P[k].shape[0] // 5):
                    P[k + "#p2"] = ops.pack_wps(P[k], h2=True)
                elif tail in ("c1#wg", "c2#wg", "w#up") and P[k].shape[1] % 32 == 0 and P[k].shape[2] % 32 == 0:
                    P[k + "#p2"] = ops.pack_wps(P[k], batch=P[k].shape[0], h2=True)
                elif tail in ("c1", "c2") and P[k].dim() == 2 and P[k].shape[0] % (9 * 32) == 0 and P[k].shape[1] % 32 == 0:
                    P[k + "#pc2"] = ops.pack_wps(P[k], h2=True)


def emit_spatial_transformer(nb_, ctx_pg, P, sd, prefix, m, x, h, w, L_ctx, ctx_in, context_dim, unfolded=False, ln_flag=None):
    pg, n = nb_.pg, nb_.n
    gn, lin = nb_.gn, nb_.lin
    p_ = lambda t: 0 if t is None else t.data_ptr()
    hw = h * w
    C_ = m.heads * m.d_head
    rows = n * hw
    xr = x.reshape(rows, m.ch)
    coef = gn(x, None, hw, sd[prefix + "norm.weight"], sd[prefix + "norm.bias"], 1e-6)
    with nb_.site(prefix + "proj_in"):
        hcur = lin(xr, P[prefix + "pin"], sd[prefix + "proj_in.bias"], hw, tf=L.TF_AFFINE, tf_coef=coef, wf=P.get(prefix + "pin#f"))
    nb_.release(coef)
    stats = pg.alloc(rows, 2)

    hf = lambda: nb_.h2_flag
    psfx = lambda: "#p2" if hf() is not None else "#p"

    kv_state = {"tiles": None}

    def ln_lin(x2d, wkey, geglu, out_ps=None, attn_kv=None, keep_xs=False):
        wp = P[wkey]
        N_ = wp.shape[1]
        h2_flag = hf()
        plan = nb_.ps_query(rows, N_, C_, tf=L.TF_LAYERNORM_FOLDED, epi=L.EPI_GEGLU if geglu else L.EPI_NONE) if wkey + psfx() in P else None
        if plan is not None:
            xs = pg.alloc_ps(rows, C_)
            if h2_flag is not None:
                pg.add("ldmk_ln_stats_ps_h2", p_(x2d), rows, C_, 1e-5, p_(stats), p_(xs), LN_GUARD_RATIO, p_(ln_flag), p_(h2_flag))
            else:
                pg.add("ldmk_ln_stats_ps", p_(x2d), rows, C_, 1e-5, p_(stats), p_(xs), LN_GUARD_RATIO, p_(ln_flag))
            kw = {}
            if attn_kv is not None and h2_flag is not None and int(plan[0]) in (23, 27) and int(plan[1]) <= 1:
                kw["attn_kv"] = attn_kv
                kv_state["tiles"] = attn_kv[0]
            y = nb_.lin_ps(plan, rows, C_, xs, wp, P[wkey + psfx()], P[wkey + "#b"], hw, geglu=geglu, out_ps=out_ps,
                           tf=L.TF_LAYERNORM_FOLDED, row_stats=stats, ln_colsum=P[wkey + "#cs"], **kw)
            if keep_xs:
                return xs
            nb_.release(xs)
            return y
        assert out_ps is None
        pg.add("ldmk_ln_stats_guard", p_(x2d), rows, C_, 1e-5, p_(stats), LN_GUARD_RATIO, p_(ln_flag))
        return lin(x2d, wp, P[wkey + "#b"], hw, geglu=geglu, tf=L.TF_LAYERNORM_FOLDED, row_stats=stats,
                   ln_colsum=P[wkey + "#cs"], wf=P.get(wkey + "#f"))

    hc_ps = plan_p = None
    ff_site = None

    def attn1_section(q, hcur):
        h2_flag = hf()
        if unfolded:
            pg.add("ldmk_ln_stats", p_(hcur), rows, C_, 1e-5, p_(stats))
            qkv = lin(hcur, P[q + "qkv"], None, hw, tf=L.TF_LAYERNORM, row_stats=stats,
                      ln_gamma=sd[q + "norm1.weight"], ln_beta=sd[q + "norm1.bias"], wf=P.get(q + "qkv#f"))
        else:
            kv_state["tiles"] = None
            kvt = None
            if (h2_flag is not None and hw >= ATTN_H2_MIN_TOKENS and hw % 64 == 0 and m.d_head == 32
                    and switches.get("LDMK_QKV_TILES", "1") != "0"):
                kvt = pg.alloc(pg.lib.ldmk_attn_kv_split_h2_bytes(n, hw, m.heads), dtype=torch.uint8)
            qkv = ln_lin(hcur, q + "qkv_ln", False, attn_kv=None if kvt is None else (kvt, hw, m.heads))
            if kvt is not None and kv_state["tiles"] is None:
                nb_.release(kvt)
                kvt = None
        plan_o = (nb_.ps_query(rows, C_, C_) if (q + "o1" + psfx() in P and L_ctx == 1 and hw % 32 == 0 and switches.get("LDMK_ATTN_PS", "1") != "0"
                                                 and m.d_head == 32
                                                 and (hw >= ATTN_H2_MIN_TOKENS if h2_flag is not None else attention_presplit(hw))) else None)
        att = None if plan_o is not None else pg.alloc(rows, C_)
        att_ps = pg.alloc_ps(rows, C_) if plan_o is not None else None
        kv_tiles = None if unfolded else kv_state["tiles"]
        emit_self_attention(nb_, qkv, att, hw, m.heads, m.d_head, att_ps=att_ps, kv_tiles=kv_tiles)
        nb_.release(qkv)
        if kv_tiles is not None:
            nb_.release(kv_tiles)
        if L_ctx != 1:
            return lin(att, P[q + "o1"], sd[q + "attn1.to_out.0.bias"], hw, residual=hcur, out=hcur, wf=P.get(q + "o1#f")), att
        v = ctx_pg.alloc(n, C_)
        ctx_pg.add("ldmk_dense_small", p_(ctx_in), context_dim, p_(P[q + "v2"]), 0, p_(v), C_, n,
                   context_dim, C_, 0)
        cvec = ctx_pg.alloc(n, C_)
        ctx_pg.add("ldmk_dense_small", p_(v), C_, p_(P[q + "o2"]), p_(sd[q + "attn2.to_out.0.bias"]), p_(cvec),
                   C_, n, C_, C_, 0)
        if plan_o is not None:
            h1 = nb_.lin_ps(plan_o, rows, C_, att_ps, P[q + "o1"], P[q + "o1" + psfx()], sd[q + "attn1.to_out.0.bias"], hw, out=hcur,
                            residual=hcur, batch_vec=cvec, batch_vec_ld=C_)
            nb_.release(att_ps)
        else:
            h1 = lin(att, P[q + "o1"], sd[q + "attn1.to_out.0.bias"], hw, residual=hcur, out=hcur,
                     batch_vec=cvec, batch_vec_ld=C_, wf=P.get(q + "o1#f"))
            nb_.release(att)
        return h1, None

    def attn2_section(q, h1, att):
        kk = ctx_pg.alloc(n * L_ctx, C_)
        vv = ctx_pg.alloc(n * L_ctx, C_)
        ctx_pg.add("ldmk_dense_small", p_(ctx_in), context_dim, p_(P[q + "k2"]), 0, p_(kk), C_,
                   n * L_ctx, context_dim, C_, 0)
        ctx_pg.add("ldmk_dense_small", p_(ctx_in), context_dim, p_(P[q + "v2"]), 0, p_(vv), C_,
                   n * L_ctx, context_dim, C_, 0)
        if unfolded:
            pg.add("ldmk_ln_stats", p_(h1), rows, C_, 1e-5, p_(stats))
            q2 = lin(h1, P[q + "q2"], None, hw, tf=L.TF_LAYERNORM, row_stats=stats, ln_gamma=sd[q + "norm2.weight"],
                     ln_beta=sd[q + "norm2.bias"], out=att, wf=P.get(q + "q2#f"))
        else:
            pg.add("ldmk_ln_stats_guard", p_(h1), rows, C_, 1e-5, p_(stats), LN_GUARD_RATIO, p_(ln_flag))
            q2 = lin(h1, P[q + "q2_ln"], P[q + "q2_ln#b"], hw, tf=L.TF_LAYERNORM_FOLDED, row_stats=stats,
                     ln_colsum=P[q + "q2_ln#cs"], out=att, wf=P.get(q + "q2_ln#f"))
        a2 = pg.alloc(rows, C_)
        if m.d_head == 32:
            pg.add("ldmk_attn_cross", p_(q2), C_, p_(kk), p_(vv), C_, p_(a2), C_, n, hw, L_ctx, m.heads, m.d_head ** -0.5)
        elif m.d_head in (40, 64, 80):
            pg.add("ldmk_attn_cross_d", p_(q2), C_, p_(kk), p_(vv), C_, p_(a2), C_, n, hw, L_ctx, m.heads, m.d_head, m.d_head ** -0.5)
        else:
            raise NotImplementedError(f"cross attention over a context of {L_ctx} tokens with heads of width {m.d_head} (built: 32, 40, 64, 80)")
        h2 = lin(a2, P[q + "o2"], sd[q + "attn2.to_out.0.bias"], hw, residual=h1, out=h1, wf=P.get(q + "o2#f"))
        nb_.release(att, a2)
        return h2

    def ff_section(q, h2, last):
        Nf = P[q + "ff2"].shape[0]
        plan_g = plan_f = None
        if not unfolded and q + "ff1_ln" + psfx() in P and q + "ff2" + psfx() in P:
            plan_g = nb_.ps_query(rows, 2 * Nf, C_, tf=L.TF_LAYERNORM_FOLDED, epi=L.EPI_GEGLU)
            plan_f = nb_.ps_query(rows, C_, Nf)
        if plan_g is not None and plan_f is not None:
            f_ps = pg.alloc_ps(rows, Nf)
            plan_fp = (nb_.ps_query(rows, m.ch, Nf + C_) if (last and prefix + "ffpo" + psfx() in P
                                                            and switches.get("LDMK_FOLD_POUT", "1") != "0") else None)
            if plan_fp is not None:
                xs = ln_lin(h2, q + "ff1_ln", True, out_ps=f_ps, keep_xs=True)
                out = nb_.lin_ps(plan_fp, rows, Nf + C_, f_ps, P[prefix + "ffpo"], P[prefix + "ffpo" + psfx()], P[prefix + "ffpo#b"], hw,
                                 residual=xr, stats=True, a_ps1=xs, a_ps_k0=Nf)
                nb_.release(f_ps, xs, h2)
                return None, None, None, out
            ln_lin(h2, q + "ff1_ln", True, out_ps=f_ps)
            plan_p = (nb_.ps_query(rows, m.ch, C_) if (last and prefix + "pout" + psfx() in P and plan_f[1] <= 1
                                                       and switches.get("LDMK_POUT_PS", "0") == "1") else None)
            hc_ps = pg.alloc_ps(rows, C_) if plan_p is not None else None
            hcur = nb_.lin_ps(plan_f, rows, Nf, f_ps, P[q + "ff2"], P[q + "ff2" + psfx()], sd[q + "ff.net.2.bias"], hw, out=h2, residual=h2,
                              out_ps=hc_ps)
            nb_.release(f_ps)
            return hcur, hc_ps, plan_p, None
        if unfolded:
            pg.add("ldmk_ln_stats", p_(h2), rows, C_, 1e-5, p_(stats))
            f = lin(h2, P[q + "ff1"], P[q + "ff1b"], hw, geglu=True, tf=L.TF_LAYERNORM, row_stats=stats,
                    ln_gamma=sd[q + "norm3.weight"], ln_beta=sd[q + "norm3.bias"], wf=P.get(q + "ff1#f"))
        else:
            f = ln_lin(h2, q + "ff1_ln", True)
        hcur = lin(f, P[q + "ff2"], sd[q + "ff.net.2.bias"], hw, residual=h2, out=h2, wf=P.get(q + "ff2#f"))
        nb_.release(f)
# ... 258 lines not shown
        P["freqs"] = ops.timestep_freqs(self.model_channels, device=dev)
        pack_gemm_copies(P, self.ln_unfolded)
        self._ln_flag = torch.zeros(1, device=dev, dtype=torch.int32)
        if self._sites is None or self._sites.flags.device != dev:
            denied = set(self._denied0) if self._sites is None else self._sites.denied
            self._sites = ArithSites(dev)
            self._sites.denied = denied
        self.generation += 1
        self._sd = sd
        self._packed = P
        self._pack_sig = self._signature()
        self._programs = {}
        self._ctx_sig = None
        self._weight_token = None

    def adopt_weights(self, token):
        sets = self.__dict__.setdefault("_weight_sets", {})
        cur = getattr(self, "_weight_token", None)
        if cur is not None and self._packed is not None and cur != token:
            sets[cur] = (self._packed, self._sd, self._programs, self._emb_off, self._emb_total, self._ln_flag, self.ln_unfolded)
        hit = sets.pop(token, None)
        if hit is not None and hit[6] == self.ln_unfolded:
            self._packed, self._sd, self._programs, self._emb_off, self._emb_total, self._ln_flag, _ = hit
            self._ctx_sig = None
        else:
            self.pack_weights()
        self._pack_sig = self._signature()
        self._weight_token = token
        while len(sets) > 1:
            sets.pop(next(iter(sets)))

    def _walk(self):
        for i, blk in enumerate(self.input_blocks):
            for j, m in enumerate(blk.layers):
                yield f"input_blocks.{i}.{j}.", m
        for j, m in enumerate(self.middle_block.layers):
            yield f"middle_block.{j}.", m
        for i, blk in enumerate(self.output_blocks):
            for j, m in enumerate(blk.layers):
                yield f"output_blocks.{i}.{j}.", m

    def _build(self, n, H, W_, L_ctx, c_concat, policy_n, float_time=False):
        P, sd = self._packed, self._sd
        dev = next(self.parameters()).device
        if self.resblock_updown and (H % (1 << (len(self.channel_mult) - 1)) or W_ % (1 << (len(self.channel_mult) - 1))):
            raise L.LdmkError(f"UNetModel(resblock_updown): {H}x{W_} input -- avg_pool2d(2, 2) of an odd grid drops its last row / column "
                              "in the reference and the skip shapes stop matching on the way up; use even sizes at every level")
        pg = Program(dev)
        pg.h2_flag = None
        pg.far_plans = far_from_tuned(policy_n)
        mc = self.model_channels
        emb_ch = 4 * mc
        cx = self.in_channels - c_concat
        x_in = pg.alloc(n, cx, H, W_)
        cc_in = pg.alloc(n, c_concat, H, W_) if c_concat else None
        t_in = pg.alloc(n, dtype=torch.float32 if float_time else torch.int64)
        ctx_in = pg.alloc(n * L_ctx, self.context_dim) if L_ctx else None
        y_emb = pg.alloc(n, emb_ch) if self.num_classes is not None else None
        pg.inputs = {"x": x_in, "c_concat": cc_in, "t_f32" if float_time else "t": t_in, "context": ctx_in, "y_emb": y_emb}
        ctx_pg = Program(dev)
        ctx_pg._all = pg._all
        p_ = lambda t: 0 if t is None else t.data_ptr()
        pin = (policy_n, n)

        temb = pg.alloc(n, mc)
        pg.add("ldmk_timestep_embedding_f32" if float_time else "ldmk_timestep_embedding", p_(t_in), p_(P["freqs"]), p_(temb), n, mc)
        e1 = pg.alloc(n, emb_ch)
        pg.add("ldmk_dense_small", p_(temb), mc, p_(P["te0"]), p_(sd["time_embed.0.bias"]), p_(e1), emb_ch, n, mc, emb_ch, 0)
        emb = pg.alloc(n, emb_ch)
        pg.add("ldmk_dense_small", p_(e1), emb_ch, p_(P["te2"]), p_(sd["time_embed.2.bias"]), p_(emb), emb_ch, n, emb_ch, emb_ch, 1)
        if y_emb is not None:
            pg.add("ldmk_axpy", p_(emb), p_(y_emb), 1.0, n * emb_ch)
        emb_all = pg.alloc(n, self._emb_total)
        pg.add("ldmk_dense_small", p_(emb), emb_ch, p_(P["emb_all"]), p_(P["emb_all_b"]), p_(emb_all), self._emb_total, n,
               emb_ch, self._emb_total, 1)

        nb_ = NetBuilder(pg, n, pin, sites=self._sites if self.f16x2 else None)
        psfx = lambda: "#p2" if nb_.h2_flag is not None else "#p"
        gn, conv, lin = nb_.gn, nb_.conv, nb_.lin

        def res_block(prefix, m, x0, x1, h, w):
            hw = h * w
            bv = emb_all.data_ptr() + 4 * self._emb_off[prefix]
            film = (bv, self._emb_total) if m.scale_shift else None
            if m.updown:
                return res_block_updown(prefix, m, x0, h, w, bv, film)
            with nb_.site(prefix + "in_layers"):
                h1 = nb_.gn_conv(x0, x1, h, w, sd[prefix + "in_layers.0.weight"], sd[prefix + "in_layers.0.bias"], 1e-5,
                                 P[prefix + "c1"], P.get(prefix + "c1#wg"), sd[prefix + "in_layers.2.bias"],
                                 batch_vec=None if film else bv,
                                 bv_ld=self._emb_total, stats=True, wf=P.get(prefix + "c1#f"), u_ps=P.get(prefix + "c1#wg" + psfx()),
                                 wp_ps=P.get(prefix + "c1#pc2"))
            g2, b2 = sd[prefix + "out_layers.0.weight"], sd[prefix + "out_layers.0.bias"]
            if m.cin != m.cout:
                x0r = x0.reshape(n * hw, -1)
                x1r = None if x1 is None else x1.reshape(n * hw, -1)
                with nb_.site(prefix + "skip_connection"):
                    skip = lin(x0r, P[prefix + "skip"], sd[prefix + "skip_connection.bias"], hw, x1=x1r, wf=P.get(prefix + "skip#f"))
                with nb_.site(prefix + "out_layers"):
                    out = nb_.gn_conv(h1, None, h, w, g2, b2, 1e-5, P[prefix + "c2"], P.get(prefix + "c2#wg"),
                                      sd[prefix + "out_layers.3.bias"], residual=skip, out=skip.view(n, h, w, m.cout), stats=True,
                                      wf=P.get(prefix + "c2#f"), u_ps=P.get(prefix + "c2#wg" + psfx()), wp_ps=P.get(prefix + "c2#pc2"), film=film)
            else:
                assert x1 is None
                with nb_.site(prefix + "out_layers"):
                    out = nb_.gn_conv(h1, None, h, w, g2, b2, 1e-5, P[prefix + "c2"], P.get(prefix + "c2#wg"),
                                      sd[prefix + "out_layers.3.bias"], residual=x0, stats=True, wf=P.get(prefix + "c2#f"),
                                      u_ps=P.get(prefix + "c2#wg" + psfx()), wp_ps=P.get(prefix + "c2#pc2"), film=film)
            nb_.release(h1)
            return out

        def res_block_updown(prefix, m, x, h, w, bv, film):
            up = m.updown == "up"
            assert m.cin == m.cout and (up or (h % 2 == 0 and w % 2 == 0))
            oh, ow = (2 * h, 2 * w) if up else (h // 2, w // 2)
            sh_, sw_ = (h, w) if up else (oh, ow)
            a = nb_.gn_act(x, None, h * w, sd[prefix + "in_layers.0.weight"], sd[prefix + "in_layers.0.bias"], 1e-5)
            a_r = pg.alloc(n, oh, ow, m.cin)
            pg.add("ldmk_resample2", p_(a), p_(a_r), n, sh_, sw_, m.cin, 1 if up else 0)
            nb_.release(a)
            x_r = pg.alloc(n, oh, ow, m.cin)
            pg.add("ldmk_resample2", p_(x), p_(x_r), n, sh_, sw_, m.cin, 1 if up else 0)
            with nb_.site(prefix + "in_layers"):
                h1 = conv(a_r, None, P[prefix + "c1"], sd[prefix + "in_layers.2.bias"], oh, ow, batch_vec=None if film else bv,
                          bv_ld=self._emb_total, stats=True, wf=P.get(prefix + "c1#f"))
            nb_.release(a_r)
            with nb_.site(prefix + "out_layers"):
                out = nb_.gn_conv(h1, None, oh, ow, sd[prefix + "out_layers.0.weight"], sd[prefix + "out_layers.0.bias"], 1e-5,
                                  P[prefix + "c2"], P.get(prefix + "c2#wg"), sd[prefix + "out_layers.3.bias"], residual=x_r,
                                  out=x_r, stats=True, wf=P.get(prefix + "c2#f"), u_ps=P.get(prefix + "c2#wg" + psfx()),
                                  wp_ps=P.get(prefix + "c2#pc2"), film=film)
            nb_.release(h1)
            return out

        def spatial_tf(prefix, m, x, h, w):
            return emit_spatial_transformer(nb_, ctx_pg, P, sd, prefix, m, x, h, w, L_ctx, ctx_in, self.context_dim,
                                            unfolded=self.ln_unfolded, ln_flag=self._ln_flag)

        def run_layers(prefix, layers, x0, x1, h, w, keep_input):
            cur0, cur1 = x0, x1
            owned = not keep_input
            for j, m in enumerate(layers):
                p = f"{prefix}{j}."
                if m.kind == "res":
                    out = res_block(p, m, cur0, cur1, h, w)
                    if m.updown:
                        h, w = (2 * h, 2 * w) if m.updown == "up" else (h // 2, w // 2)
                elif m.kind == "st":
                    out = spatial_tf(p, m, cur0, h, w)
                elif m.kind == "attn":
                    out = emit_attention_block(nb_, P, sd, p, m, cur0, h, w)
                elif m.kind == "down":
                    with nb_.site(p + "op"):
                        out = conv(cur0, None, P[p + "w"], sd[p + "op.bias"], h, w, stride=2, stats=True)
                    h, w = (h - 1) // 2 + 1, (w - 1) // 2 + 1
                elif m.kind == "up":
                    with nb_.site(p + "conv"):
                        out = nb_.up_conv(cur0, h, w, P[p + "w"], P.get(p + "w#up"), sd[p + "conv.bias"], stats=True, w4_ps=P.get(p + "w#up" + psfx()))
                    h, w = 2 * h, 2 * w
                else:
                    raise AssertionError(m.kind)
                if owned:
                    nb_.release(cur0)
                cur0, cur1, owned = out, None, True
            return cur0, h, w

        hs = []
        h0 = pg.alloc(n, H, W_, mc)
        pg.add("ldmk_conv3x3_in", p_(x_in), cx, p_(cc_in), c_concat, p_(P["input_blocks.0.0.w"]),
               p_(sd["input_blocks.0.0.bias"]), p_(h0), n, H, W_, mc)
        hcur, ch_, cw_ = h0, H, W_
        hs.append((hcur, ch_, cw_))
        for i in range(1, len(self.input_blocks)):
            hcur, ch_, cw_ = run_layers(f"input_blocks.{i}.", self.input_blocks[i].layers, hcur, None, ch_, cw_, True)
            hs.append((hcur, ch_, cw_))
        hcur, ch_, cw_ = run_layers("middle_block.", self.middle_block.layers, hcur, None, ch_, cw_, True)
        for i, blk in enumerate(self.output_blocks):
            skip, sh, sw = hs.pop()
            assert (sh, sw) == (ch_, cw_)
            new, ch_, cw_ = run_layers(f"output_blocks.{i}.", blk.layers, hcur, skip, ch_, cw_, True)
            nb_.release(hcur, skip)
            hcur = new
        coef = gn(hcur, None, ch_ * cw_, sd["out.0.weight"], sd["out.0.bias"], 1e-5)
        eps = pg.alloc(n, self.out_channels, H, W_)
        co_small = (policy_n * H * W_ < 256 * 256 and self._final_ch % 4 == 0
                    and 9 * self._final_ch * self.out_channels * 4 <= 60 * 1024)
        pg.add("ldmk_conv3x3_out_small" if co_small else "ldmk_conv3x3_out", p_(hcur), p_(coef), p_(P["out"]), p_(sd["out.2.bias"]),
               p_(eps), n, H, W_, self._final_ch, self.out_channels)
        pg.outputs = dict(eps=eps)
        pg.ctx_program = ctx_pg
        return pg

    H2_SITE_PASSES = 2

    def flags_tripped(self, check_layernorm=True):
        import warnings
        if self.f16x2 and self._sites is not None:
            raised = self._sites.raised()
            if raised:
                self._h2_passes += 1
                if self._h2_passes > self.H2_SITE_PASSES:
                    warnings.warn("UNetModel: operands keep leaving the range of the F16X2 arithmetic (|x| >= 1000) after "
                                  f"{self.H2_SITE_PASSES} rounds of per-site fall-back; switching the whole model to the bf16x3 "
                                  "arithmetic (LDMK_F16X2=0 starts there)", RuntimeWarning, stacklevel=3)
                    self.f16x2 = False
                else:
                    self._sites.denied.update(raised)
                    warnings.warn(f"UNetModel: an operand left the range of the F16X2 arithmetic (|x| >= 1000) at {len(raised)} of "
                                  f"{len(self._sites.index)} sites ({', '.join(raised[:4])}{', ...' if len(raised) > 4 else ''}); "
                                  "these run in the bf16x3 arithmetic from now on, the others stay in F16X2", RuntimeWarning, stacklevel=3)
                if self._ln_flag is not None:
                    self._ln_flag.zero_()
                self._programs.clear()
                for st_ in self.__dict__.get("_weight_sets", {}).values():
                    st_[2].clear()
                self.generation += 1
                return True
            self._h2_passes = 0
        if check_layernorm and not (self.ln_unfolded or self._ln_flag is None or int(self._ln_flag.item()) == 0):
            warnings.warn(f"UNetModel: token rows with |mean| > {LN_GUARD_RATIO:g} standard deviations reached a LayerNorm; the folded "
                          "form (LayerNorm through the product) loses accuracy on them -- switching this model to the unfolded "
                          "prologue (LDMK_LN_UNFOLDED=1 starts there)", RuntimeWarning, stacklevel=3)
            self.ln_unfolded = True
            tok = getattr(self, "_weight_token", None)
            self.__dict__.get("_weight_sets", {}).clear()
            self.pack_weights()
            self._weight_token = tok
            return True
        return False

    layernorm_guard_tripped = flags_tripped

    def deny_f16x2(self, names):
        names = set(names)
        self._denied0 |= names
        if self._sites is not None and not names <= self._sites.denied:
            self._sites.denied |= names
            self._programs.clear()
            for st_ in self.__dict__.get("_weight_sets", {}).values():
                st_[2].clear()
            self.generation += 1

    def arithmetic_status(self):
        up = [] if self._sites is None else self._sites.raised(clear=False)
        return {"f16x2": bool(self.f16x2), "sites": 0 if self._sites is None else len(self._sites.index),
                "denied": sorted(self._sites.denied) if self._sites is not None else [], "flags_up": up,
                "ln_flag_up": bool(self._ln_flag is not None and int(self._ln_flag.item()) != 0), "ln_unfolded": bool(self.ln_unfolded)}

    def program(self, n, H, W_, L_ctx, c_concat=0, float_time=False):
        if self._packed is None or (self.auto_repack and self._pack_sig != self._signature()):
            self.pack_weights()
        policy_n = self.policy_batch or n
        key = (n, H, W_, L_ctx, c_concat, policy_n) + (("float_time",) if float_time else ())
        pg = self._programs.get(key)
        if pg is None:
            from . import unet_small
            plain = self._heads32 and not self.use_scale_shift_norm and self.num_classes is None and not self.resblock_updown
            if plain and unet_small.wants_small_route(policy_n, H, W_, L_ctx):
                pg = unet_small.build_small(self, n, H, W_, L_ctx, c_concat, policy_n, float_time=float_time)
            else:
                pg = self._build(n, H, W_, L_ctx, c_concat, policy_n, float_time=float_time)
            self._programs[key] = pg
        return pg

    def convert_to_fp16(self):
        raise NotImplementedError("UNetModel.convert_to_fp16: fp32 only (reference precision; use_fp16 is refused the same way)")

    def convert_to_fp32(self):
        return None

    @torch.no_grad()
    def forward(self, x, timesteps=None, context=None, y=None, c_concat=None, **kwargs):
        assert (y is not None) == (self.num_classes is not None), "must specify y if and only if the model is class-conditional"
        if context is None and self.use_spatial_transformer:
            raise L.LdmkError("UNetModel.forward: context is required (the reference raises a shape error for "
                              "context=None when context_dim != inner dim, attention.py:174-175)")
        if context is not None and not self.use_spatial_transformer:
            raise L.LdmkError("UNetModel.forward: this UNet has no cross-attention (use_spatial_transformer=False): context must be None")
        if not x.is_cuda:
            raise L.LdmkError("UNetModel.forward: input must be a CUDA tensor (no CPU fallback)")
        n, cx, H, W_ = x.shape
        cc = 0 if c_concat is None else c_concat.shape[1]
        assert cx + cc == self.in_channels, f"got {cx}+{cc} input channels, model has {self.in_channels}"
        assert context is None or (context.shape[0] == n and context.shape[2] == self.context_dim)
        L_ctx = 0 if context is None else context.shape[1]
        float_time = timesteps.is_floating_point()
        for _ in range(MAX_ARITHMETIC_PASSES):
            pg = self.program(n, H, W_, L_ctx, cc, float_time=float_time)
            pg.inputs["x"].copy_(x)
            if cc:
                pg.inputs["c_concat"].copy_(c_concat)
            if float_time:
                pg.inputs["t_f32"].copy_(timesteps.to(torch.float32))
            else:
                pg.inputs["t"].copy_(timesteps.to(torch.int64))
            if L_ctx:
                pg.inputs["context"].copy_(context.reshape(n * L_ctx, self.context_dim))
            if y is not None:
                assert y.shape == (n,)
                pg.inputs["y_emb"].copy_(self.label_emb.weight.detach().float()[y.to(torch.int64)])
            pg.ctx_program.run()
            pg.run()
            if torch.cuda.is_current_stream_capturing():
                break
            first = not getattr(pg, "ln_checked", False)
            pg.ln_checked = True
            if not self.flags_tripped(check_layernorm=first):
# ... 3 lines not shown
```

include/ldmk.h:

```cpp
#ifndef LDMK_H
#define LDMK_H
#ifdef __cplusplus
extern "C" {
#endif

#define LDMK_OK 0
#define LDMK_EINVAL (-1)
#define LDMK_EHIP (-2)
#define LDMK_ENOMEM (-3)

int ldmk_version(void);
const char* ldmk_last_error(void);
int ldmk_init(int device);

int ldmk_switch_value(const char* name);
int ldmk_switch_override(const char* name, int value);

enum { LDMK_A_ROWS = 0, LDMK_A_CONV3X3 = 1 };
enum { LDMK_TF_NONE = 0, LDMK_TF_AFFINE = 1, LDMK_TF_AFFINE_SILU = 2, LDMK_TF_LAYERNORM = 3,
       LDMK_TF_LAYERNORM_FOLDED = 4 };
enum { LDMK_EPI_NONE = 0, LDMK_EPI_GEGLU = 1 };
enum { LDMK_COMPUTE_F32 = 0, LDMK_COMPUTE_BF16 = 1, LDMK_COMPUTE_BF16X3 = 2, LDMK_COMPUTE_F16X2 = 3 };
#define LDMK_F16X2_A_EXP 6
#define LDMK_F16X2_RANGE 1000.0f

typedef struct ldmk_igemm_args {
  int M, N, K;
  const float* a0;
  const float* a1;
  int c0, c1;
  int a_mode;
  int in_h, in_w;
  int out_h, out_w;
  int stride, pad_lo;
  int upsample;
  int a_tf;
  const float* tf_coef;
  const float* row_stats;
  const float* ln_gamma;
  const float* ln_beta;
  int rows_per_sample;
  const float* w;
  int b_trans, ldb;
  const float* bias;
  const float* batch_vec;
  int batch_vec_ld;
  const float* residual;
  int epi;
  float* out;
  int ldc;
  int batch;
  long long a_bstride, w_bstride, out_bstride;
  float alpha;
  int tile_cfg;
  int splitk;
  float* splitk_ws;
  long long splitk_ws_elems;
  float* stats_out;
  int compute;
  int* splitk_counters;
  int splitk_counters_len;
  const float* w_frag;
  const float* ln_colsum;
  int raw_slabs;
  const float* skip_a0;
  const float* skip_a1;
  int skip_c0, skip_c1;
  const void* w_split;
  int w_split_ld;
  long long w_split_bstride;
  const void* a_split;
  int a_split_ld;
  const void* a_ps;
  long long a_ps_bstride;
  const void* w_ps;
  long long w_ps_bstride;
  void* out_ps;
  int w_scale_exp;
  int* range_flag;
  void* attn_kv_out;
  int attn_tokens;
  int attn_heads;
  const void* a_ps1;
  int a_ps_k0;
} ldmk_igemm_args;

long long ldmk_ps_bytes(int rows, int k);
int ldmk_pack_ps(const float* src, int rows, int k, long long row_stride, long long k_stride, int batch, long long src_bstride,
                 void* dst, void* stream);
int ldmk_ln_stats_ps(const float* x, int rows, int c, float eps, float* stats, void* dst, float guard, int* flag, void* stream);

long long ldmk_ps_bytes_h2(int rows, int k);
int ldmk_pack_ps_h2(const float* src, int rows, int k, long long row_stride, long long k_stride, int batch, long long src_bstride,
                    int scale_exp, int* range_flag, void* dst, void* stream);
int ldmk_ln_stats_ps_h2(const float* x, int rows, int c, float eps, float* stats, void* dst, float guard, int* flag, int* range_flag,
                        void* stream);
int ldmk_gn_apply_ps_h2(const float* x0, int c0, const float* x1, int c1, const float* coef, void* y_ps, int n, int hw, int silu,
                        int* range_flag, void* stream);

int ldmk_pack_wsplit(const float* w, int K, int N, int ldb, int batch, long long w_bstride, void* out, int ld_out, void* stream);
int ldmk_pack_wsplit_h2(const float* w, int K, int N, int ldb, int batch, long long w_bstride, int scale_exp, void* out, int ld_out,
                        void* stream);
int ldmk_pack_wbf16t(const float* w, int K, int N, int ldb, void* out, int ld_out, void* stream);

int ldmk_igemm(const ldmk_igemm_args* args, void* stream);
long long ldmk_igemm_workspace_elems(const ldmk_igemm_args* args);
int ldmk_igemm_check(const ldmk_igemm_args* args);
long long ldmk_wfrag_elems(int K, int N);
int ldmk_pack_wfrag(const float* w, int ldb, int K, int N, float* wfrag, void* stream);
int ldmk_fold_layernorm(const float* w, int ldb, int K, int N, const float* gamma, const float* beta, const float* bias,
                        float* w_out, float* colsum, float* bias_out, void* stream);
int ldmk_igemm_plan(const ldmk_igemm_args* args, int* tile_cfg, int* splitk);

long long ldmk_winograd_tiles(int n, int h, int w);
int ldmk_winograd_input(const float* x0, int c0, const float* x1, int c1, const float* coef, int silu, int n, int h, int w,
                        float* v, void* stream);
int ldmk_winograd_input_ps(const float* x0, int c0, const float* x1, int c1, const float* coef, int silu, int n, int h, int w,
                           void* v_ps, void* stream);
int ldmk_winograd_input_ps_h2(const float* x0, int c0, const float* x1, int c1, const float* coef, int silu, int n, int h, int w,
                              void* v_ps, int* range_flag, void* stream);
int ldmk_winograd_output(const float* m, const float* bias, const float* batch_vec, int batch_vec_ld, const float* residual,
                         float* out, float* stats_out, int n, int h, int w, int cout, void* stream);
int ldmk_winograd_input_ps_route(int n, int h, int w, int c0, int c1);
int ldmk_winograd_output_route(int n, int h, int w, int cout, int with_stats);
int ldmk_winograd_input_ps_v1(const float* x0, int c0, const float* x1, int c1, const float* coef, int silu, int n, int h, int w,
                              void* v_ps, void* stream);
int ldmk_winograd_input_ps_h2_v1(const float* x0, int c0, const float* x1, int c1, const float* coef, int silu, int n, int h, int w,
                                 void* v_ps, int* range_flag, void* stream);
int ldmk_winograd_output_v1(const float* m, const float* bias, const float* batch_vec, int batch_vec_ld, const float* residual,
                            float* out, float* stats_out, int n, int h, int w, int cout, void* stream);

int ldmk_upconv_gather(const float* x, int c, int n, int h, int w, float* a, void* stream);
int ldmk_upconv_gather_ps(const float* x, int c, int n, int h, int w, void* a_ps, void* stream);
int ldmk_upconv_gather_ps_h2(const float* x, int c, int n, int h, int w, void* a_ps, int* range_flag, void* stream);
int ldmk_upconv_scatter(const float* planes, const float* bias, float* out, float* stats_out, int n, int h, int w, int cout,
                        void* stream);

int ldmk_gn_chunks(int hw);
int ldmk_gn_partial(const float* x, int c, int n, int hw, float* partial, void* stream);
int ldmk_gn_finalize(const float* partial0, int c0, const float* partial1, int c1, int n, int hw, int groups,
                     float eps, const float* gamma, const float* beta, float* coef, void* stream);
int ldmk_gn_coef(const float* x0, int c0, const float* x1, int c1, int n, int hw, int groups, float eps,
                 const float* gamma, const float* beta, float* partial, float* coef, void* stream);
int ldmk_ln_stats(const float* x, int rows, int c, float eps, float* stats, void* stream);
int ldmk_ln_stats_guard(const float* x, int rows, int c, float eps, float* stats, float guard, int* flag, void* stream);
int ldmk_ln_stats_split(const float* x, int rows, int C, float eps, float* stats, void* split, int ld_split, void* stream);
int ldmk_gn_apply(const float* x0, int c0, const float* x1, int c1, const float* coef, float* y, int n, int hw,
                  int silu, void* stream);
int ldmk_resample2(const float* x, float* y, int n, int h, int w, int c, int up, void* stream);
int ldmk_gn_coef_film(float* coef, const float* emb, int ld, int n, int c, void* stream);

enum { LDMK_POST_NONE = 0, LDMK_POST_GROUPNORM = 1, LDMK_POST_LAYERNORM = 2 };
typedef struct ldmk_post_args {
  const float* src;
  int nslab;
  long long slab_stride;
  int M, N;
  int rows_per_sample;
  float alpha;
  const float* bias;
  const float* batch_vec;
  int batch_vec_ld;
  const float* residual;
  int ldr;
  int geglu;
  float* raw_out;
  int ld_raw;
  int norm;
  const float* x1;
  int c1;
  int groups;
// ... 202 lines not shown
```

Baseline: 1266 sample-steps/s.

## Fuse upsampling-conv phase gather, GEMM and scatter into one pre-split kernel

Adds a phase-mode pre-split kernel that computes the four output-parity phases of the nearest-upsample+3x3 conv directly from the low-resolution input. It gathers the 2x2 taps in the DMA addressing and interleaves the results into NHWC output, with optional GroupNorm records. This replaces the gather, batch-4 GEMM and scatter launches and their intermediate buffers. Separately, the stride-2 downsampling convs are routed onto the conv-mode pre-split f16x2 tile with packed weights. The trade-off is extra packing launches, and the GroupNorm partial sums are partitioned differently.

After: 1279 sample-steps/s, median of 6. No clear change (+1.0%).

```diff
diff --git a/dsml_thesis_amd/csrc/igemm.hip b/dsml_thesis_amd/csrc/igemm.hip
--- a/dsml_thesis_amd/csrc/igemm.hip
+++ b/dsml_thesis_amd/csrc/igemm.hip
@@ -1234,7 +1234,8 @@
   LDMK_REQUIRE(a.M > 0 && a.N > 0 && a.K > 0, "ldmk_igemm: empty problem M=%d N=%d K=%d", a.M, a.N, a.K);
   LDMK_REQUIRE(a.c0 > 0 && a.c0 % 32 == 0 && a.c1 % 32 == 0, "ldmk_igemm: channel counts must be multiples of 32 (c0=%d c1=%d)", a.c0, a.c1);
   LDMK_REQUIRE((a.c1 == 0) == (a.a1 == nullptr), "ldmk_igemm: a1/c1 mismatch");
-  const int taps = a.a_mode == LDMK_A_CONV3X3 ? 9 : 1;
+  LDMK_REQUIRE(a.a_mode == LDMK_A_ROWS || a.a_mode == LDMK_A_CONV3X3 || a.a_mode == LDMK_A_UPCONV2X2, "ldmk_igemm: a_mode=%d", a.a_mode);
+  const int taps = a.a_mode == LDMK_A_CONV3X3 ? 9 : (a.a_mode == LDMK_A_UPCONV2X2 ? 4 : 1);
   const int skip_k = a.skip_a0 ? a.skip_c0 + a.skip_c1 : 0;
   LDMK_REQUIRE(a.K == taps * (a.c0 + a.c1) + skip_k, "ldmk_igemm: K=%d != taps*(c0+c1)+skip=%d", a.K, taps * (a.c0 + a.c1) + skip_k);
   LDMK_REQUIRE(!a.skip_a0 || (a.a_mode == LDMK_A_CONV3X3 && a.skip_c0 > 0 && a.skip_c0 % 8 == 0 && a.skip_c1 % 8 == 0 &&
@@ -1263,7 +1264,7 @@
   LDMK_REQUIRE(a.a_tf >= LDMK_TF_NONE && a.a_tf <= LDMK_TF_LAYERNORM_FOLDED, "ldmk_igemm: a_tf=%d", a.a_tf);
   if (a.epi == LDMK_EPI_GEGLU) LDMK_REQUIRE(a.N % 64 == 0 && !a.residual && !a.batch_vec, "ldmk_igemm: GEGLU needs N%%64==0 and no residual");
   if (a.stats_out)
-    LDMK_REQUIRE(a.M % 32 == 0 && a.rows_per_sample % 32 == 0 && a.epi == LDMK_EPI_NONE && a.batch <= 1,
+    LDMK_REQUIRE(a.M % 32 == 0 && a.rows_per_sample % 32 == 0 && a.epi == LDMK_EPI_NONE && (a.batch <= 1 || a.a_mode == LDMK_A_UPCONV2X2),
                  "ldmk_igemm: stats_out needs M%%32==0, rows_per_sample%%32==0, no GEGLU, no batching");
   LDMK_REQUIRE(a.tile_cfg >= 0 && a.tile_cfg <= kNumCfg + kNumRCfg + kNumSCfg + kNumWCfg + kNumPCfg, "ldmk_igemm: tile_cfg=%d outside [0,%d]",
                a.tile_cfg, kNumCfg + kNumRCfg + kNumSCfg + kNumWCfg + kNumPCfg);
@@ -1271,6 +1272,8 @@
   LDMK_REQUIRE(a.compute == LDMK_COMPUTE_F32 || a.compute == LDMK_COMPUTE_BF16 || a.compute == LDMK_COMPUTE_BF16X3 || a.compute == LDMK_COMPUTE_F16X2,
                "ldmk_igemm: compute=%d", a.compute);
   const bool ps_tile = a.tile_cfg > kNumCfg + kNumRCfg + kNumSCfg + kNumWCfg;
+  LDMK_REQUIRE(a.a_mode != LDMK_A_UPCONV2X2 || (ps_tile && a.a_ps && a.compute == LDMK_COMPUTE_F16X2),
+               "ldmk_igemm: LDMK_A_UPCONV2X2 (the upsampling phases) runs on a pinned pre-split tile in LDMK_COMPUTE_F16X2 only (a_ps, tile_cfg 23 / 24 / 26 / 27)");
   LDMK_REQUIRE(!a.a_ps1 || (ps_tile && a.a_ps), "ldmk_igemm: a_ps1 (second A source) is read by the pre-split tiles only, next to a_ps");
   if (a.compute == LDMK_COMPUTE_BF16X3 && !ps_tile) {
     LDMK_REQUIRE(a.w_split && !a.b_trans && a.w_split_ld >= a.K && a.w_split_ld % 8 == 0,
@@ -1311,6 +1314,7 @@
   plan(a, &cfg, &sk, a.splitk_ws ? a.splitk_ws_elems : 0);
   if (a.tile_cfg > 0) cfg = a.tile_cfg;
   if (g_force_cfg > 0 && (g_force_cfg <= kNumCfg || !rgemm_unsupported(a, g_force_cfg - kNumCfg - 1))) cfg = g_force_cfg;
+  LDMK_REQUIRE(a.a_mode != LDMK_A_UPCONV2X2 || cfg > kNumCfg + kNumRCfg + kNumSCfg + kNumWCfg, "ldmk_igemm: LDMK_A_UPCONV2X2 on tile_cfg=%d", cfg);
   LDMK_REQUIRE(!a.skip_a0 || cfg > kNumCfg + kNumRCfg, "ldmk_igemm: the fused skip connection runs on the slab GEMM only (tile_cfg 13..20)");
   if (cfg > kNumCfg + kNumRCfg + kNumSCfg + kNumWCfg) {
     const int pcfg = cfg - kNumCfg - kNumRCfg - kNumSCfg - kNumWCfg - 1;
diff --git a/dsml_thesis_amd/csrc/igemm_ps.hip b/dsml_thesis_amd/csrc/igemm_ps.hip
--- a/dsml_thesis_amd/csrc/igemm_ps.hip
+++ b/dsml_thesis_amd/csrc/igemm_ps.hip
@@ -957,6 +957,152 @@
   return check_launch("ldmk_igemm(ps, conv)");
 }
 
+template <int NWM, int NWN, int TM, int TN>
+__global__ __launch_bounds__(64 * NWM * NWN, 2) void igemm_psu_kernel(const ldmk_igemm_args p, const int nfast) {
+  constexpr int PL = 2, NS = 3;
+  constexpr int NW = NWM * NWN;
+  constexpr int BM = 32 * TM * NWM, BN = 32 * TN * NWN;
+  constexpr int FA = BM / 32, FB = BN / 32, U = FA + FB;
+  constexpr int UHI = (U + NW - 1) / NW, ULO = U / NW;
+  constexpr int AI = (FA + NW - 1) / NW;
+  constexpr int UB = PL * 1024;
+  constexpr int STAGE = U * UB;
+  static_assert(PL * UHI * (NS - 1) <= 63, "vmcnt");
+  extern __shared__ __attribute__((aligned(1024))) unsigned char smem_ps[];
+
+  const int tid = threadIdx.x, lane = tid & 63, wave = __builtin_amdgcn_readfirstlane(tid >> 6);
+  const int l31 = lane & 31, half = lane >> 5;
+  const int wm = wave / NWN, wn = wave - wm * NWN;
+  const int tiles_m = (p.M + BM - 1) / BM;
+  const int tiles_n = (p.N + BN - 1) / BN;
+  const int bid = xcd_remap(blockIdx.x, tiles_m * tiles_n);
+  const int m0 = nfast ? (bid / tiles_n) * BM : (bid % tiles_m) * BM;
+  const int n0 = nfast ? (bid % tiles_n) * BN : (bid / tiles_m) * BN;
+  const int bz = blockIdx.z, pa = bz >> 1, pb = bz & 1;
+
+  const int Kc = p.c0 / 16, Kb_w = p.K / 16;
+  const int Nb = p.N / 32;
+  const unsigned Mb_in = (unsigned)((p.M + 31) / 32);
+  const u32x4 rs_a = buffer_rsrc(p.a_ps, Mb_in * (unsigned)Kc * (unsigned)UB);
+  const u32x4 rs_b = buffer_rsrc(reinterpret_cast<const unsigned char*>(p.w_ps) + (long long)bz * p.w_ps_bstride, (unsigned)Nb * (unsigned)Kb_w * (unsigned)UB);
+
+  unsigned toff[AI][4];
+#pragma unroll
+  for (int i = 0; i < AI; ++i) {
+    const int u = wave + NW * i;
+    const int row = m0 + 32 * u + l31;
+    const bool rok = u < FA && row < p.M;
+    const int rr = rok ? row : 0;
+    const int n = rr / p.rows_per_sample, rem = rr - n * p.rows_per_sample;
+    const int y = rem / p.in_w, x = rem - y * p.in_w;
+#pragma unroll
+    for (int t = 0; t < 4; ++t) {
+      const int iy = y + pa + (t >> 1) - 1, ix = x + pb + (t & 1) - 1;
+      const bool ok = rok && iy >= 0 && iy < p.in_h && ix >= 0 && ix < p.in_w;
+      const unsigned q = (unsigned)((n * p.in_h + iy) * p.in_w + ix);
+      toff[i][t] = ok ? (q >> 5) * (unsigned)Kc * (unsigned)UB + ((unsigned)half * 32u + (q & 31u)) * 16u : PS_OOB;
+    }
+  }
+  unsigned ubase[UHI];
+#pragma unroll
+  for (int i = 0; i < UHI; ++i) {
+    const int u = wave + NW * i;
+    const int blk = n0 / 32 + (u - FA);
+    ubase[i] = (u >= FA && u < U && blk < Nb) ? (unsigned)blk * (unsigned)Kb_w * (unsigned)UB : PS_OOB;
+  }
+  const unsigned lane16 = lane * 16;
+  const unsigned lds0 = (unsigned)(size_t)smem_ps;
+  const bool hi_wave = wave + NW * (UHI - 1) < U;
+
+  f32x16 acc[TM][TN];
+#pragma unroll
+  for (int i = 0; i < TM; ++i)
+#pragma unroll
+    for (int j = 0; j < TN; ++j)
+#pragma unroll
+      for (int r = 0; r < 16; ++r) acc[i][j][r] = 0.f;
+
+  auto issue = [&](const unsigned (&ta)[AI], const int slab, const int buf, const unsigned sB, const bool live) {
+    const unsigned cs = (unsigned)slab * (unsigned)UB;
+    const unsigned bdst = lds0 + (unsigned)buf * STAGE;
+#pragma unroll
+    for (int i = 0; i < UHI; ++i) {
+      const int u = wave + NW * i;
+      if (u < U) {
+        if (i < AI && u < FA) {
+          const unsigned t = ta[i < AI ? i : 0];
+          ps_dma<PL>((live && t != PS_OOB) ? t + cs : PS_OOB, rs_a, bdst + (unsigned)u * (unsigned)UB);
+        } else {
+          ps_dma<PL>((live && ubase[i] != PS_OOB) ? lane16 + ubase[i] + sB * (unsigned)UB : PS_OOB, rs_b, bdst + (unsigned)u * (unsigned)UB);
+        }
+      }
+    }
+  };
+
+  {
+    unsigned t0[AI];
+#pragma unroll
+    for (int i = 0; i < AI; ++i) t0[i] = toff[i][0];
+    issue(t0, 0, 0, 0, true);
+    issue(t0, 1, 1, 1, true);
+  }
+  unsigned sB = 0;
+  int rb = 0;
+#pragma unroll
+  for (int tap = 0; tap < 4; ++tap) {
+    for (int slab = 0; slab < Kc; ++slab) {
+      if (hi_wave) wait_vm<PL * UHI * (NS - 2)>(); else wait_vm<PL * ULO * (NS - 2)>();
+      asm volatile("s_barrier" ::: "memory");
+      {
+        const bool nx = slab + 2 >= Kc;
+        unsigned ta[AI];
+#pragma unroll
+        for (int i = 0; i < AI; ++i) ta[i] = nx ? (tap < 3 ? toff[i][tap < 3 ? tap + 1 : 3] : PS_OOB) : toff[i][tap];
+        const int ib = rb + 2 >= NS ? rb + 2 - NS : rb + 2;
+        issue(ta, nx ? slab + 2 - Kc : slab + 2, ib, sB + 2, !(nx && tap == 3));
+      }
+      ++sB;
+      const unsigned char* sb = smem_ps + rb * STAGE + lane16;
+      rb = rb + 1 == NS ? 0 : rb + 1;
+      f16x8 a8[PL][TM];
+#pragma unroll
+      for (int g = 0; g < PL; ++g)
+#pragma unroll
+        for (int i = 0; i < TM; ++i) a8[g][i] = *reinterpret_cast<const f16x8*>(sb + ((wm * TM + i) * PL + g) * 1024);
+#pragma unroll
+      for (int jn = 0; jn < TN; ++jn) {
+        f16x8 b8[PL];
+#pragma unroll
+        for (int g = 0; g < PL; ++g) b8[g] = *reinterpret_cast<const f16x8*>(sb + ((FA + wn * TN + jn) * PL + g) * 1024);
+#pragma unroll
+        for (int i = 0; i < TM; ++i) {
+          acc[i][jn] = __builtin_amdgcn_mfma_f32_32x32x16_f16(a8[1][i], b8[0], acc[i][jn], 0, 0, 0);
+          acc[i][jn] = __builtin_amdgcn_mfma_f32_32x32x16_f16(a8[0][i], b8[1], acc[i][jn], 0, 0, 0);
+          acc[i][jn] = __builtin_amdgcn_mfma_f32_32x32x16_f16(a8[0][i], b8[0], acc[i][jn], 0, 0, 0);
+        }
+      }
+    }
+  }
+  wait_vm<0>();
+  col_phase<TM, TN>(p, acc, m0 + wm * 32 * TM, n0 + wn * 32 * TN, bz, l31, half);
+}
+
+template <int NWM, int NWN, int TM, int TN>
+static int psu_launch(const ldmk_igemm_args& a, hipStream_t st) {
+  constexpr int BM = 32 * TM * NWM, BN = 32 * TN * NWN;
+  constexpr size_t lds = (size_t)3 * (BM / 32 + BN / 32) * 2048;
+  static_assert(lds <= 160 * 1024, "LDS ring exceeds 160 KiB");
+  static bool attr = false;
+  if (!attr) {
+    (void)hipFuncSetAttribute(reinterpret_cast<const void*>(igemm_psu_kernel<NWM, NWN, TM, TN>), hipFuncAttributeMaxDynamicSharedMemorySize, (int)lds);
+    attr = true;
+  }
+  const int tiles = ((a.M + BM - 1) / BM) * ((a.N + BN - 1) / BN);
+  const int nfast = switch_value(SW_PS_NFAST) && (a.N + BN - 1) / BN > 1 && (a.M + BM - 1) / BM >= 8 ? 1 : 0;
+  hipLaunchKernelGGL((igemm_psu_kernel<NWM, NWN, TM, TN>), dim3(tiles, 1, 4), dim3(64 * NWM * NWN), lds, st, a, nfast);
+  return check_launch("ldmk_igemm(ps, upsampling phases)");
+}
+
 const char* igemm_ps_unsupported(const ldmk_igemm_args& a, int pcfg, int splitk) {
   if (a.compute != LDMK_COMPUTE_BF16X3 && a.compute != LDMK_COMPUTE_F16X2) return "the pre-split tiles run the bf16x3 and the f16x2 arithmetic (compute)";
   const int pl = a.compute == LDMK_COMPUTE_F16X2 ? 2 : 3;
@@ -972,8 +1118,26 @@
     if ((a.c0 / 32) % splitk) return "conv mode: splitk must divide C_in / 32 (K is split on 32-channel chunk boundaries)";
     const long long smp = ((long long)a.M + a.rows_per_sample - 1) / a.rows_per_sample;
     if (((smp * a.in_h * a.in_w + 31) / 32) * (a.c0 / 16) * 2048 >= (1LL << 31)) return "conv mode: input of 2 GiB or more";
+  } else if (a.a_mode == LDMK_A_UPCONV2X2) {
+    if (pl != 2) return "phase mode: the f16x2 arithmetic only (a_ps / w_ps as two fp16 planes, not the three bf16 planes)";
+    if (pcfg != 0 && pcfg != 1 && pcfg != 3 && pcfg != 4) return "phase mode: tile_cfg 23 / 24 / 26 / 27";
+    if (a.batch != 4) return "phase mode: batch = 4, one entry per output parity";
+    if (splitk != 1) return "phase mode: no split-K";
+    if (a.a_ps1) return "phase mode: one A source (no a_ps1)";
+    if (a.out_ps) return "phase mode: no out_ps (the interleaving epilogue stores fp32 NHWC)";
+    if (a.epi != LDMK_EPI_NONE) return "phase mode: no GEGLU";
+    if (a.residual) return "phase mode: no residual";
+    if (a.batch_vec) return "phase mode: no per-sample vector";
+    if (a.attn_kv_out) return "phase mode: no attn_kv_out";
+    if (a.c1 || a.a1 || a.a_tf != LDMK_TF_NONE || a.raw_slabs) return "phase mode: one raw source (ldmk_pack_ps_h2), no prologue, no raw slabs";
+    if (a.c0 % 32) return "phase mode: C_in must be a multiple of 32";
+    if (a.in_h <= 0 || a.in_w <= 0 || a.rows_per_sample != a.in_h * a.in_w) return "phase mode: rows_per_sample = in_h x in_w of the low-resolution input";
+    if (a.stats_out && (a.in_h * a.in_w) % 32) return "phase mode: GroupNorm records need in_h x in_w to be a multiple of 32";
+    if (!a.out) return "phase mode: no output";
+    if (4LL * a.M * a.ldc >= (1LL << 31)) return "phase mode: output of 2^31 elements or more (32-bit epilogue offsets)";
+    if ((long long)((a.M + 31) / 32) * (a.c0 / 16) * 2048 >= (1LL << 31)) return "phase mode: input of 2 GiB or more";
   } else if (a.a_mode != LDMK_A_ROWS) {
-    return "rows mode or 3x3 convolution";
+    return "rows mode, 3x3 convolution or upsampling phases";
   }
   if (a.b_trans || a.upsample || a.skip_a0 || (a.splitk_counters && !(ps_probe_bits() & 8))) return "b_trans / upsample / fused skip / in-launch combine";
   if (a.a_tf != LDMK_TF_NONE && a.a_tf != LDMK_TF_LAYERNORM_FOLDED) return "no staging prologue: a_ps is what gets multiplied";
@@ -1014,6 +1178,14 @@
       case 1: return tr ? psc_launch<4, 2, 2, 5, true>(a, splitk, ws, st) : psc_launch<4, 2, 2, 5, false>(a, splitk, ws, st);
       case 3: return tr ? psc_launch<4, 2, 1, 5, true>(a, splitk, ws, st) : psc_launch<4, 2, 1, 5, false>(a, splitk, ws, st);
       default: return tr ? psc_launch<4, 1, 1, 5, true>(a, splitk, ws, st) : psc_launch<4, 1, 1, 5, false>(a, splitk, ws, st);
+    }
+  }
+  if (a.a_mode == LDMK_A_UPCONV2X2) {
+    switch (pcfg) {
+      case 0: return psu_launch<8, 1, 1, 5>(a, st);
+      case 1: return psu_launch<4, 2, 2, 5>(a, st);
+      case 3: return psu_launch<4, 2, 1, 5>(a, st);
+      default: return psu_launch<4, 1, 1, 5>(a, st);
     }
   }
   if (a.compute == LDMK_COMPUTE_F16X2 && a.attn_kv_out)
diff --git a/dsml_thesis_amd/csrc/ldmk_epilogue.h b/dsml_thesis_amd/csrc/ldmk_epilogue.h
--- a/dsml_thesis_amd/csrc/ldmk_epilogue.h
+++ b/dsml_thesis_amd/csrc/ldmk_epilogue.h
@@ -197,6 +197,52 @@
   }
 }
 
+template <int TM, int TN>
+__device__ __forceinline__ void col_phase(const ldmk_igemm_args& p, const f32x16 (&acc)[TM][TN], const int rowbase, const int colbase,
+                                          const int phase, const int l31, const int half) {
+  float* __restrict__ outp = p.out;
+  const float alpha = p.alpha;
+  const int hw = p.rows_per_sample, W = p.in_w;
+  const int pa = phase >> 1, pb = phase & 1;
+  float bv[TN];
+#pragma unroll
+  for (int j = 0; j < TN; ++j) {
+    const int col = colbase + j * 32 + l31;
+    bv[j] = (p.bias && col < p.N) ? p.bias[col] : 0.f;
+  }
+#pragma unroll
+  for (int i = 0; i < TM; ++i) {
+    const int u0 = rowbase + i * 32;
+    if (u0 >= p.M) continue;
+    const int row = min(u0 + l31, p.M - 1);
+    const int n = row / hw, rem = row - n * hw;
+    const int y = rem / W, x = rem - y * W;
+    const unsigned opix = (unsigned)((n * 2 * p.in_h + 2 * y + pa) * (2 * W) + 2 * x + pb) * (unsigned)p.ldc;
+    unsigned ro[16];
+#pragma unroll
+    for (int r = 0; r < 16; ++r) ro[r] = (unsigned)__shfl((int)opix, 4 * half + (r & 3) + 8 * (r >> 2), 64);
+    const int r0 = u0 + 4 * half;
+    const int ns = u0 / hw;
+    const int chunk = ns * (hw >> 3) + phase * (hw >> 5) + ((u0 - ns * hw) >> 5);
+#pragma unroll
+    for (int j = 0; j < TN; ++j) {
+      const int col = colbase + j * 32 + l31;
+      if (col >= p.N) continue;
+      float vals[16];
+#pragma unroll
+      for (int r = 0; r < 16; ++r) {
+        float v = 0.f;
+        if (r0 + (r & 3) + 8 * (r >> 2) < p.M) {
+          v = col_finish(acc[i][j][r] * alpha, bv[j]);
+          outp[ro[r] + (unsigned)col] = v;
+        }
+        vals[r] = v;
+      }
+      if (p.stats_out) gn_tile_record(vals, p.stats_out, chunk, p.N, col, l31, half);
+    }
+  }
+}
+
 __device__ __forceinline__ int col_lean_form(const ldmk_igemm_args& p, const int splitk, const bool off, const int row_end, const int col_end) {
   if (off || splitk != 1 || row_end > p.M || col_end > p.N) return 0;
   if (p.batch_vec && p.rows_per_sample % 32 != 0) return 0;
diff --git a/dsml_thesis_amd/engine.py b/dsml_thesis_amd/engine.py
--- a/dsml_thesis_amd/engine.py
+++ b/dsml_thesis_amd/engine.py
@@ -498,6 +498,18 @@
         if self.pin is not None and self.pin[0] != self.pin[1]:
             m = max(1, M * self.pin[0] // self.pin[1])
         return ps_plan(f"{N},{K},{L.A_CONV3X3},0,0,1" + ("" if stride == 1 else f",s{stride}u0"), m, h2=True, max_ratio=2.0)
+
+    def ps_query_up(self, pix, cout, c):
+        if not ps_enabled() or self.h2_flag is None or switches.get("LDMK_PSC", "1") == "0":
+            return None
+        forced = switches.get("LDMK_PSC_FORCE")
+        if forced:
+            return int(forced.split(",")[0]), 1
+        m = pix
+        if self.pin is not None and self.pin[0] != self.pin[1]:
+            m = max(1, pix * self.pin[0] // self.pin[1])
+        plan = ps_plan(f"{cout},{4 * c},{L.A_ROWS},0,0,4,s1u1", m, h2=True, max_ratio=2.0)
+        return None if plan is None else (plan[0], 1)
 
     def gn_conv(self, x0, x1, h, w, gamma, beta, eps, wp, u, bias, batch_vec=None, bv_ld=0, residual=None, out=None,
                 stats=False, wf=None, u_ps=None, wp_ps=None, film=None):
@@ -579,6 +591,26 @@
             return self.conv(x, None, wp, bias, h, w, upsample=True, stats=stats)
         cout = w4.shape[2]
         pix = n * h * w
+        plan_u = (self.ps_query_up(pix, cout, c)
+                  if (w4_ps is not None and pg.h2_flag is not None and c % 32 == 0 and cout % 32 == 0 and (h * w) % 32 == 0) else None)
+        if plan_u is not None:
+            hf = pg.h2_flag
+            x_ps = pg.alloc_ps(pix, 4 * c)
+            pg.add("ldmk_pack_ps_h2", p_(x), pix, c, c, 1, 1, pix * c, ops.F16X2_A_EXP, p_(hf), p_(x_ps))
+            out = pg.alloc(n, 2 * h, 2 * w, cout)
+            a = ops.make_igemm_args(pix, cout, 4 * c, None, c, w4, out, cout, h * w, bias=bias, batch=4, w_bstride=4 * c * cout,
+                                    a_ps=x_ps, w_ps=w4_ps, range_flag=hf)
+            a.a_mode, a.in_h, a.in_w, a.out_h, a.out_w, a.a_ps_bstride = L.A_UPCONV2X2, h, w, 2 * h, 2 * w, 0
+            a._winograd = True
+            a._algo_flops = 2.0 * (4 * pix) * cout * (9 * c)
+            out2d = out.view(-1, cout)
+            if stats:
+                self.drop_stats(out2d)
+                part = self.stats_buffer(4 * pix, cout)
+                a.stats_out = part.data_ptr()
+                self.attach_stats(out2d, part)
+            self._igemm_on_raw_ps(a, plan_u, x_ps)
+            return out
         Pm = pg.alloc(4, pix, cout)
         out = pg.alloc(n, 2 * h, 2 * w, cout)
         plan = self.ps_query(pix, cout, 4 * c, batch=4) if (w4_ps is not None and c % 16 == 0) else None
@@ -613,6 +645,29 @@
         pg.release(A, Pm)
         return out
 
+    def down_conv(self, x, h, w, wp, bias, wp_ps=None):
+        pg, n, ops, p_ = self.pg, self.n, self.ops, self.ptr
+        c, cout = x.shape[-1], wp.shape[1]
+        oh, ow = (h - 1) // 2 + 1, (w - 1) // 2 + 1
+        plan = (self.ps_query_conv(n * oh * ow, cout, 9 * c, stride=2)
+                if (wp_ps is not None and c % 32 == 0 and cout % 32 == 0) else None)
+        if plan is None:
+            return self.conv(x, None, wp, bias, h, w, stride=2, stats=True)
+        hf = self.h2_flag
+        x_ps = pg.alloc_ps(n * h * w, c)
+        pg.add("ldmk_pack_ps_h2", p_(x), n * h * w, c, c, 1, 1, n * h * w * c, ops.F16X2_A_EXP, p_(hf), p_(x_ps))
+        out = pg.alloc(n, oh, ow, cout)
+        a = ops.make_igemm_args(n * oh * ow, cout, 9 * c, None, c, wp, out, cout, oh * ow, conv=(h, w, oh, ow, 2, 1, 0), bias=bias,
+                                a_ps=x_ps, w_ps=wp_ps, range_flag=hf)
+        a._algo_flops = 2.0 * (n * oh * ow) * cout * (9 * c)
+        self._maybe_stats(a, out.view(-1, cout), oh * ow, True)
+        self._igemm_on_raw_ps(a, plan, x_ps)
+        return out
+
+    def _igemm_on_raw_ps(self, a, plan, x_ps):
+        self.pg.igemm_ps(a, *plan)
+        self.pg.release(x_ps)
+
     def _maybe_stats(self, a, out2d, rows_per_sample, stats):
         if stats and a.M % 32 == 0 and rows_per_sample % 32 == 0:
             self.drop_stats(out2d)
diff --git a/dsml_thesis_amd/lib.py b/dsml_thesis_amd/lib.py
--- a/dsml_thesis_amd/lib.py
+++ b/dsml_thesis_amd/lib.py
@@ -6,7 +6,7 @@
 _HERE = os.path.dirname(os.path.abspath(__file__))
 LIB_PATH = switches.get("LDMK_LIBRARY") or os.path.join(_HERE, "libldmk.so")
 
-A_ROWS, A_CONV3X3 = 0, 1
+A_ROWS, A_CONV3X3, A_UPCONV2X2 = 0, 1, 2
 TF_NONE, TF_AFFINE, TF_AFFINE_SILU, TF_LAYERNORM, TF_LAYERNORM_FOLDED = 0, 1, 2, 3, 4
 EPI_NONE, EPI_GEGLU = 0, 1
 COMPUTE_F32, COMPUTE_BF16, COMPUTE_BF16X3, COMPUTE_F16X2 = 0, 1, 2, 3
diff --git a/dsml_thesis_amd/ops.py b/dsml_thesis_amd/ops.py
--- a/dsml_thesis_amd/ops.py
+++ b/dsml_thesis_amd/ops.py
@@ -125,6 +125,24 @@
     if stats_out is not None:
         a.stats_out = stats_out.data_ptr()
         a._keep = a._keep + (stats_out,)
+    igemm(a)
+    return out
+
+
+def upsample_conv3x3_ps(x_ps, n, h, w_, cin, wp4, wp4_ps, range_flag, bias=None, out=None, tile_cfg=27, stats_out=None, **fields):
+    cout = wp4.shape[2]
+    pix = n * h * w_
+    if out is None:
+        out = torch.empty(n, 2 * h, 2 * w_, cout, device=wp4.device, dtype=torch.float32)
+    a = make_igemm_args(pix, cout, 4 * cin, None, cin, wp4, out, cout, h * w_, bias=bias, batch=4, w_bstride=4 * cin * cout,
+                        tile_cfg=tile_cfg, splitk=1, a_ps=x_ps, w_ps=wp4_ps, range_flag=range_flag)
+    a.a_mode, a.in_h, a.in_w, a.out_h, a.out_w, a.a_ps_bstride = L.A_UPCONV2X2, h, w_, 2 * h, 2 * w_, 0
+    if stats_out is not None:
+        a.stats_out = stats_out.data_ptr()
+        a._keep = a._keep + (stats_out,)
+    for k, v in fields.items():
+        setattr(a, k, _ptr(v) if isinstance(v, torch.Tensor) else v)
+        a._keep = a._keep + (v,)
     igemm(a)
     return out
 
diff --git a/dsml_thesis_amd/switches.py b/dsml_thesis_amd/switches.py
--- a/dsml_thesis_amd/switches.py
+++ b/dsml_thesis_amd/switches.py
@@ -13,10 +13,12 @@
     "LDMK_PS": ("1", "route", "0: no pre-split (PS layout, LDS-DMA) GEMM tiles: every GEMM back on the LDS-tiled plan of its shape (that plan's "
                 "tile and K split), no conv-mode tile, no folded proj_out -- other bits, same tolerance (tile for tile, at equal split-K, "
                 "a pre-split kernel gives the LDS-tiled kernel's bits: tests/test_ps_gpu.py)", "tolerance"),
-    "LDMK_PSC": ("1", "route", "0: no conv-mode pre-split tile for 3x3 convolutions: the listed shapes return to their other route (Winograd for "
-                 "the wide ones, the in-register split on that route's plan) -- other bits, same tolerance (at equal split-K the tile gives "
-                 "the LDS-tiled F16X2 convolution's bits: tests/test_ps_conv_gpu.py)", "tolerance"),
-    "LDMK_PSC_FORCE": (None, "route", "'cfg,splitk': force the conv-mode pre-split tile for every eligible convolution (A/B runs)", None),
+    "LDMK_PSC": ("1", "route", "0: no conv-mode pre-split tile for 3x3 convolutions and no phase mode of it for the upsampling convolutions: the "
+                 "listed shapes return to their other route (Winograd for the wide ones, the in-register split on that route's plan; "
+                 "gather + batch-4 GEMM + scatter for the upsampling phases) -- other bits, same tolerance (at equal split-K the tile gives "
+                 "the LDS-tiled F16X2 convolution's bits: tests/test_ps_conv_gpu.py; the phase mode gives the three-launch route's bits, "
+                 "only its GroupNorm records partition the pixels differently: tests/test_upconv_psc_gpu.py)", "tolerance"),
+    "LDMK_PSC_FORCE": (None, "route", "'cfg,splitk': force the conv-mode pre-split tile for every eligible convolution, and the phase mode on tile cfg (no K split) for every eligible upsampling convolution (A/B runs)", None),
     "LDMK_POUT_PS": ("0", "route", "1: SpatialTransformer.proj_out on a pre-split tile instead of the row GEMM (measured slower; another arithmetic: other bits, same tolerance)", "tolerance"),
     "LDMK_FOLD_POUT": ("1", "route", "0: the last block's ff.net.2 and proj_out stay two GEMMs instead of one pre-split GEMM on two A "
                        "sources with the composed weight (other bits, same tolerance)", "tolerance"),
diff --git a/dsml_thesis_amd/unet.py b/dsml_thesis_amd/unet.py
--- a/dsml_thesis_amd/unet.py
+++ b/dsml_thesis_amd/unet.py
@@ -237,6 +237,8 @@
                 elif tail in ("c1#wg", "c2#wg", "w#up") and P[k].shape[1] % 32 == 0 and P[k].shape[2] % 32 == 0:
                     P[k + "#p2"] = ops.pack_wps(P[k], batch=P[k].shape[0], h2=True)
                 elif tail in ("c1", "c2") and P[k].dim() == 2 and P[k].shape[0] % (9 * 32) == 0 and P[k].shape[1] % 32 == 0:
+                    P[k + "#pc2"] = ops.pack_wps(P[k], h2=True)
+                elif tail == "w" and k + "#up" not in P and P[k].dim() == 2 and P[k].shape[0] % (9 * 32) == 0 and P[k].shape[1] % 32 == 0:
                     P[k + "#pc2"] = ops.pack_wps(P[k], h2=True)
 
 
@@ -801,7 +803,7 @@
                     out = emit_attention_block(nb_, P, sd, p, m, cur0, h, w)
                 elif m.kind == "down":
                     with nb_.site(p + "op"):
-                        out = conv(cur0, None, P[p + "w"], sd[p + "op.bias"], h, w, stride=2, stats=True)
+                        out = nb_.down_conv(cur0, h, w, P[p + "w"], sd[p + "op.bias"], wp_ps=P.get(p + "w#pc2"))
                     h, w = (h - 1) // 2 + 1, (w - 1) // 2 + 1
                 elif m.kind == "up":
                     with nb_.site(p + "conv"):
diff --git a/include/ldmk.h b/include/ldmk.h
--- a/include/ldmk.h
+++ b/include/ldmk.h
@@ -16,7 +16,8 @@
 int ldmk_switch_value(const char* name);
 int ldmk_switch_override(const char* name, int value);
 
-enum { LDMK_A_ROWS = 0, LDMK_A_CONV3X3 = 1 };
+enum { LDMK_A_ROWS = 0, LDMK_A_CONV3X3 = 1,
+       LDMK_A_UPCONV2X2 = 2 };
 enum { LDMK_TF_NONE = 0, LDMK_TF_AFFINE = 1, LDMK_TF_AFFINE_SILU = 2, LDMK_TF_LAYERNORM = 3,
        LDMK_TF_LAYERNORM_FOLDED = 4 };
 enum { LDMK_EPI_NONE = 0, LDMK_EPI_GEGLU = 1 };
```
